# srvk/eesen

Hardware: AMD Instinct MI355X
Metric: CTC training frames/sec (whole node), 4x512 BiLSTM (higher is better)
Workload: dtype f32

## Files before the change

eesen_amd/build.py:

```python
from __future__ import annotations

import os
import shutil
import subprocess
import sys
from concurrent.futures import ThreadPoolExecutor

_DIR = os.path.dirname(os.path.abspath(__file__))
CSRC = os.path.join(_DIR, "csrc")
LIBDIR = os.path.join(_DIR, "lib")
LIB = os.path.join(LIBDIR, "libeesen_hip.so")
SOURCES = ["gemm.hip", "lstm.hip", "lstm_persistent.hip", "rec_plan.cpp", "ctc.hip", "ctc_decode.hip", "ce.hip", "optim.hip", "feeder.hip", "net.cpp", "ctc_host.cpp", "ce_host.cpp", "nnet_format.cpp", "lm.cpp", "lex.cpp", "capi.cpp", "comm.cpp"]
HEADERS = ["common.h", "guard.h", "kernels.h", "rec_kernels.h", "net.h", "lm.h", "lex.h", "handles.h", "tuning.h", os.path.join("..", "..", "include", "eesen_hip.h")]
FLAGS = (os.environ.get("EESEN_BUILD_DEFS", "").split()) + ["--offload-arch=gfx950", "-O3", "-std=c++17", "-fPIC", "-fno-gpu-rdc", "-Wall", "-Wno-unused-function"]


BINDIR = os.path.join(os.path.dirname(os.path.abspath(__file__)), "bin")
TOOLS = {"train-ctc-parallel": "train_ctc_parallel.cc", "train-ce-parallel": "train_ce_parallel.cc", "net-output-extract": "net_output_extract.cc", "ctc-align": "ctc_align.cc", "ctc-decode": "ctc_decode.cc"}


def csrc_digest() -> str:
    import hashlib
    h = hashlib.sha1()
    files = []
    for d in (CSRC, os.path.join(CSRC, "tools"), os.path.join(_DIR, "..", "include")):
        files += [os.path.join(d, f) for f in sorted(os.listdir(d)) if f.endswith((".hip", ".cpp", ".h", ".cc", ".map"))]
    for f in files:
        h.update(os.path.basename(f).encode() + b"\0")
        h.update(open(f, "rb").read())
    return h.hexdigest()[:16]


def hipcc() -> str:
    for c in (os.environ.get("HIPCC"), shutil.which("hipcc"), "/opt/rocm/bin/hipcc"):
        if c and os.path.exists(c):
            return c
    raise RuntimeError("hipcc not found")


def _stale(target: str, deps) -> bool:
    if not os.path.exists(target):
        return True
    t = os.path.getmtime(target)
    return any(os.path.getmtime(d) > t for d in deps)


def build(force: bool = False, verbose: bool = False) -> str:
    os.makedirs(LIBDIR, exist_ok=True)
    cc = hipcc()
    hdrs = [os.path.join(CSRC, h) for h in HEADERS] + [os.path.abspath(__file__)]
    jobs = []
    objs = []
    for s in SOURCES:
        src = os.path.join(CSRC, s)
        obj = os.path.join(LIBDIR, s.replace(".", "_") + ".o")
        objs.append(obj)
        if force or _stale(obj, [src] + hdrs):
            cmd = [cc] + FLAGS + (["-x", "hip"] if s.endswith(".cpp") else []) + ["-c", src, "-o", obj]
            jobs.append(cmd)

    def run(cmd):
        if verbose:
            print(" ".join(cmd), file=sys.stderr)
        r = subprocess.run(cmd, capture_output=True, text=True)
        if r.returncode != 0:
            raise RuntimeError("hipcc failed:\n" + " ".join(cmd) + "\n" + r.stdout + r.stderr)
        return r.stderr

    with ThreadPoolExecutor(max_workers=8) as ex:
        for warn in ex.map(run, jobs):
            if verbose and warn:
                print(warn, file=sys.stderr)
    if jobs or force or _stale(LIB, objs + [os.path.join(CSRC, "exports.map")]):
        run([cc, "--offload-arch=gfx950", "-shared", "-fPIC", "-o", LIB] + objs +
            ["-ldl", "-Wl,-Bsymbolic", "-Wl,--version-script=" + os.path.join(CSRC, "exports.map")])
    os.makedirs(BINDIR, exist_ok=True)
    cxx = shutil.which("g++") or "g++"
    for name, src in TOOLS.items():
        exe = os.path.join(BINDIR, name)
        srcp = os.path.join(CSRC, "tools", src)
        if force or _stale(exe, [srcp, LIB, os.path.join(CSRC, "tools", "kaldi_tables.h"), os.path.join(CSRC, "tools", "feat_pipeline.h"), os.path.join(CSRC, "tools", "parse_options.h"), os.path.join(CSRC, "tools", "class_prior.h"),
                                 os.path.join(CSRC, "..", "..", "include", "eesen_hip.h"), os.path.join(CSRC, "..", "..", "include", "eesen_hip_info.h")]):
            run([cxx, "-O2", "-std=c++17", "-Wall", srcp, "-o", exe, "-L" + LIBDIR, "-leesen_hip", "-Wl,-rpath," + LIBDIR,
                 "-Wl,-rpath,$ORIGIN/../lib", "-Wl,--allow-shlib-undefined"])
    return LIB


if __name__ == "__main__":
    print(build(force="--force" in sys.argv, verbose=True))
```

eesen_amd/csrc/kernels.h:

```cpp
#pragma once
#include "common.h"

namespace eesen {

struct GemmBound {
  const float* p = nullptr;
  int per_index = 0;
};
void gemm_f32(hipStream_t st, bool a_kc, bool b_kc, int M, int N, int K, float alpha, const float* A, int lda,
              const float* B, int ldb, float beta, float* C, int ldc, const float* bias, float* ws,
              size_t ws_floats, int extra_lds_bytes = 0,
              bool bf16_operands = false,
              GemmBound bound_a = {}, GemmBound bound_b = {});

constexpr int kDefaultGemmMode = 2;
int gemm_mode();
void set_gemm_mode(int mode);
void amax_abs(hipStream_t st, const float* P, long rows, int cols, int ld, float* out);
void amax_abs_accumulate(hipStream_t st, const float* P, long rows, int cols, int ld, float* out);
constexpr int kAmaxBlocks = 512;
void amax_rows_cols(hipStream_t st, const float* P, long rows, int cols, int ld, float* out_rows, float* out_cols, float* ws);

#ifndef EESEN_SHARDS
#define EESEN_SHARDS 8
#endif
constexpr int kShards = EESEN_SHARDS, kShardStride = 32;
constexpr int kCtlHalf = 2048 * kShards;

struct GemmGate {
  const unsigned* cnt;
  unsigned* err;
  int ndir, nz, nblk;
  int T, S;
  int spin_limit;
};
void gemm_f32_nt_gated(hipStream_t st, int M, int N, int K, const float* A, int lda, const float* B, int ldb, float* C,
                       int ldc, const float* bias, const GemmGate& gate, GemmBound bound_a = {}, GemmBound bound_b = {});

struct LstmLayerDev {
  int T, S, H, ndir;
  float* G;
  float* C;
  float* Y;
  float* X = nullptr;
  const float* Wm;
  const float* WmT;
  const float* peep;
  const int* lens;
  const float* rmask = nullptr;
  int drop_mode = 0;
  int s_begin = 0, s_count = 0;
  float* PX = nullptr;
  size_t px_floats = 0;
  int poll_delay = 0;
  int poll_raw = 0;
  unsigned* milestone = nullptr;
  int milestone_step = 0;
  int xcd_map = 1, fwd_mux = 1, bwd_q4 = 1, bwd_ksplit = 1, bwd_mux = 1;
  int fwd_t16_small = 1;
  int fwd_narrow2 = 1;
  int bwd_q4_st8 = 1;
  int fwd_bf16 = 0;
  int fwd_split = 0;
  int fwd_f16 = 0;
  const float* wm_amax = nullptr;
  int bwd_f16 = 0;
  unsigned char* DGH = nullptr;
  float* EX = nullptr;
};
float handoff_flight_ns();
void set_gpu_share(int n);
int gpu_share_value();
void wait_for_word(hipStream_t st, const unsigned* word, unsigned target, unsigned* err, double limit_s = 2.0);
void lstm_fwd_step(hipStream_t st, const LstmLayerDev& L, int step);
void lstm_bwd_step(hipStream_t st, const LstmLayerDev& L, int step, const float* dY, int lddy, float* DG, float* DCF);
void dropout_mask(hipStream_t st, float* out, long rows, int cols, int ld, float p, unsigned long long seed, bool per_column);
void activation_rows(hipStream_t st, bool tanh_, const float* x, int ldx, float* y, int ldy, long rows, int cols);
void activation_diff_rows(hipStream_t st, bool tanh_, const float* y, int ldy, float* d, int ldd, long rows, int cols);
void mul_elements(hipStream_t st, const float* a, int lda, const float* m, int ldm, float* out, int ldo, long rows, int cols);
enum { kRecNone = 0, kRecFwdBf = 1, kRecFwdMux = 2, kRecFwdF32 = 3, kRecBwdQ4 = 4, kRecBwdKsplit = 5, kRecBwdKsplitMux = 6, kRecBwdGeneric = 7 };
struct RecPlan {
  int kind = kRecNone;
  const char* kernel = "";
  int seq_tile = 0;
  int units = 0;
  int windows = 0;
  int grid[3] = {0, 0, 0};
  int wgs = 0;
  int wgs_per_cu = 0;
  int vgprs = 0, lds = 0;
  int free_vgprs = -1;
  int seq_tiles = 1;
  bool one_window = false;
  bool leaves_room = false;
  bool bf16 = false;
  bool light = false;
  size_t need_px = 0, need_ex = 0;
  bool need_dgh = false;
  size_t ctl_words = 0;
  int chunk = 0;
  const void* fn = nullptr;
};
RecPlan lstm_fwd_plan(const LstmLayerDev& L);
RecPlan lstm_bwd_plan(const LstmLayerDev& L);
void lstm_fwd_launch(hipStream_t st, const RecPlan& plan, const LstmLayerDev& L, unsigned* cnt, unsigned* err, int spin_limit,
                     unsigned long long* trace = nullptr, hipEvent_t after_reset = nullptr);
void lstm_bwd_launch(hipStream_t st, const RecPlan& plan, const LstmLayerDev& L, const float* dY, int lddy, float* DG, unsigned* cnt,
                     unsigned* err, int spin_limit, unsigned long long* trace = nullptr);
void lstm_bias_peep_grads(hipStream_t st, const LstmLayerDev& L, const float* DG, float* bias_grad, float* peep_grad,
                          float* ws, size_t ws_floats);
size_t lstm_bias_peep_ws_floats(int T, int S, int H, int ndir);

void col_sums(hipStream_t st, const float* M, int rows, int cols, int ld, float* out, float* ws, size_t ws_floats);
size_t col_sums_ws_floats(int rows, int cols);

void softmax_rows(hipStream_t st, const float* x, int ldx, float* y, int ldy, int rows, int K);
void log_rows(hipStream_t st, const float* in, int ldi, float* out, int ldo, int rows, int K);
void ctc_alpha_beta(hipStream_t st, const float* logp, int ld, int T, int S, int Lpad, const int* labx, const int* lens,
                    const int* lablens, float* alpha, float* beta, float* pzx, int waves = 0);
int ctc_sweep_waves(int Lpad, int waves = 0);
void ctc_best_path(hipStream_t st, const float* scores, int ld, int T, int S, int Lpad, const int* labx, const int* lens,
                   const int* lablens, float* delta, int waves = 0, int lattices = 0, int lat0 = 0, int lpu = 1);
void ctc_traceback(hipStream_t st, const float* delta, int T, int S, int Lpad, const int* labx, const int* lens, const int* lablens,
                   int* ali, int* pos, float* score);
void ctc_stamp(hipStream_t st, const int* pos, int T, int NL, int G, const int* lens, int* lstart, int* lend);
void ctc_hyp_lattices(hipStream_t st, const int* hyp, const int* hyp_len, const int* lens, int T, int NL, int N, int Lpad, int* labx,
                      int* lablens, int* lat_lens);
void ctc_row_topc(hipStream_t st, const float* scores, int ld, int rows, int K, int S, const int* lens, int Cc, int* cid, float* csc,
                  float* sblank);
struct LmTables;
struct LexTables;
void ctc_prefix_beam(hipStream_t st, const float* scores, int ld, int T, int S, const int* lens, int B, int Cc, const int* cid,
                     const float* csc, const float* sblank, const LmTables* lm, const LexTables* lex, float alpha, float beta, bool use_eos,
                     int* tparent, int* tlabel, int* fnode, int* flen, float* fscore, float* flm, int* count);
void ctc_hyp(hipStream_t st, const int* tparent, const int* tlabel, const int* fnode, const int* flen, const float* fscore, const float* flm,
             const int* count, int T, int S, int B, int N, int* hyp, int* hyp_len, float* score, float* lm_out);
struct WordLexTables;
void ctc_word_beam(hipStream_t st, const float* scores, int ld, int T, int S, const int* lens, int B, int Cc, const int* cid,
                   const float* csc, const float* sblank, const LmTables* lm, const WordLexTables& lex, float alpha, float beta, bool use_eos,
                   int* tparent, int* tlabel, int* tword, int* fnode, int* flen, float* fscore, float* flm, int* fword, int* fnw, int* count);
void ctc_word_hyp(hipStream_t st, const int* tparent, const int* tlabel, const int* tword, const int* fnode, const int* flen, const float* fscore,
                  const float* flm, const int* fword, const int* fnw, const int* count, int T, int S, int B, int N, int* hyp, int* hyp_len,
                  float* score, float* lm_out, int* words, int* ends, int* word_len);
void ctc_error_diff(hipStream_t st, const float* probs, int ld, int T, int S, int K, int Lpad, int Lmax, const int* lens,
                    const int* lablens, const int* labx, const float* alpha, const float* beta,
                    const float* pzx, float* diff, int ldd);
void log_sub_prior(hipStream_t st, float* m, int ld, int rows, int K, bool apply_log, const float* log_prior, float prior_scale);
void row_argmax(hipStream_t st, const float* m, int ld, int rows, int K, int* ids);

struct CeSums {
  double obj;
  long long correct;
};
int ce_eval_blocks(int rows);
void ce_eval(hipStream_t st, const float* y, int ld, int rows, int K, int S, const int* lens, const int* tgt, float* diff,
             int ldd, CeSums* part, CeSums* out);

void sgd_update(hipStream_t st, float* param, float* corr, const float* fresh, long n, float mmt, float lr_coef,
                float max_grad, const unsigned* skip = nullptr, const float* live = nullptr);
void zero_if_set(hipStream_t st, float* p, long n, const unsigned* word);
void adaptive_update(hipStream_t st, float* param, float* corr, const float* fresh, float* accu, long n, float mmt, float lr,
                     float max_grad, float eps, float rho, float one_minus_rho, bool rmsprop, const unsigned* skip = nullptr,
                     const float* live = nullptr);
void tensor_moments(hipStream_t st, const float* base, long rows, int cols, long ld, double* out6, double* ws,
                    int nb = 0, int hf = 0, int hi = 0);
void transpose2d(hipStream_t st, const float* src, int rows, int cols, float* dst);
void copy2d(hipStream_t st, const float* src, int lds, float* dst, int ldd, int rows, int cols);

}
```

eesen_amd/csrc/lstm_persistent.hip:

```cpp
#include "rec_kernels.h"

namespace eesen {
namespace {

typedef float f32x4 __attribute__((ext_vector_type(4)));
constexpr int NW = 8;
constexpr int kSc1 = 16;

#define EESEN_RCP(x) __builtin_amdgcn_rcpf(x)
__device__ __forceinline__ float sigmoidf_(float x) { return EESEN_RCP(1.f + __expf(-x)); }
__device__ __forceinline__ float tanhf_(float x) { return 1.f - 2.f * EESEN_RCP(1.f + __expf(2.f * x)); }

__device__ __forceinline__ __amdgpu_buffer_rsrc_t make_rsrc(const float* base) {
  return __builtin_amdgcn_make_buffer_rsrc(const_cast<float*>(base), 0, 0x7fffffff, 0x00020000);
}
__device__ __forceinline__ float ld1(__amdgpu_buffer_rsrc_t r, unsigned byte_off) {
  return __builtin_bit_cast(float, __builtin_amdgcn_raw_buffer_load_b32(r, byte_off, 0, 0));
}
constexpr int EESEN_POLL_WAVE = 7;
constexpr int EESEN_POLL_SLEEP = 1;
__device__ __forceinline__ void ld8_sc1(__amdgpu_buffer_rsrc_t r, unsigned byte_off, int k, int kmax, bool ok, float (&v)[8]) {
  constexpr int pol = 0;
  constexpr unsigned kOob = 0x80000000u;
  const unsigned oa = (ok && k < kmax) ? byte_off : kOob;
  const unsigned ob = (ok && k + 4 < kmax) ? byte_off + 16 : kOob;
  const f32x4 a = __builtin_amdgcn_raw_buffer_load_b128(r, oa, 0, pol);
  const f32x4 b = __builtin_amdgcn_raw_buffer_load_b128(r, ob, 0, pol);
  v[0] = a[0]; v[1] = a[1]; v[2] = a[2]; v[3] = a[3];
  v[4] = b[0]; v[5] = b[1]; v[6] = b[2]; v[7] = b[3];
}
__device__ __forceinline__ float ror8(float x) {
  return __builtin_bit_cast(float, __builtin_amdgcn_mov_dpp(__builtin_bit_cast(int, x), 0x128, 0xf, 0xf, true));
}
__device__ __forceinline__ void ld8_plain(const float* __restrict__ row, int k, int kmax, bool ok, float (&v)[8]) {
  float4 a = make_float4(0.f, 0.f, 0.f, 0.f), b = a;
  if (ok && k < kmax) a = *reinterpret_cast<const float4*>(row + k);
  if (ok && k + 4 < kmax) b = *reinterpret_cast<const float4*>(row + k + 4);
  v[0] = a.x; v[1] = a.y; v[2] = a.z; v[3] = a.w;
  v[4] = b.x; v[5] = b.y; v[6] = b.z; v[7] = b.w;
}

struct Role {
  int nblk, ndir, nz, xcd;
  __device__ __forceinline__ int combo(int b) const { return xcd ? b % (ndir * nz) : b / nblk; }
  __device__ __forceinline__ int unit_group(int b) const { return xcd ? b / (ndir * nz) : b % nblk; }
  __device__ __forceinline__ int dir(int b) const { return combo(b) % ndir; }
  __device__ __forceinline__ int seq_group(int b) const { return combo(b) / ndir; }
};

__device__ __forceinline__ void sleep_ticks(int ticks) {
  if (ticks <= 0) return;
  const unsigned long long t0 = wall_clock64();
  while ((long long)(wall_clock64() - t0) < (long long)ticks) __builtin_amdgcn_s_sleep(1);
}
__device__ __forceinline__ bool wait_counters(unsigned* cnt, unsigned nblk, unsigned step, unsigned* err, int spin_limit, int lane, int delay) {
  const unsigned mine = lane < kShards ? ((nblk - lane + kShards - 1) / kShards) * step : 0u;
  sleep_ticks(delay);
  for (int spins = 0; spins < spin_limit; ++spins) {
    bool ok = true;
    if (lane < kShards) ok = __hip_atomic_load(cnt + lane * kShardStride, __ATOMIC_RELAXED, __HIP_MEMORY_SCOPE_AGENT) >= mine;
    if (__all(ok)) return true;
    if ((spins & 1023) == 1023 && __hip_atomic_load(err, __ATOMIC_RELAXED, __HIP_MEMORY_SCOPE_AGENT) != 0) return false;
    __builtin_amdgcn_s_sleep(EESEN_POLL_SLEEP);
  }
  if (lane == 0) __hip_atomic_store(err, 1u, __ATOMIC_RELAXED, __HIP_MEMORY_SCOPE_AGENT);
  return false;
}

__global__ __launch_bounds__(64) void handoff_pingpong_kernel(unsigned* flags, unsigned long long* out, int rounds) {
  if (threadIdx.x != 0) return;
  unsigned* mine = flags + (blockIdx.x == 0 ? 0 : 32);
  unsigned* theirs = flags + (blockIdx.x == 0 ? 32 : 0);
  unsigned* dead = flags + 16;
  const unsigned long long t0 = wall_clock64();
  bool ok = true;
  for (int i = 1; i <= rounds && ok; ++i) {
    if (blockIdx.x == 0) __hip_atomic_store(mine, (unsigned)i, __ATOMIC_RELAXED, __HIP_MEMORY_SCOPE_AGENT);
    ok = false;
    for (int spins = 0; spins < (1 << 20); ++spins) {
      if (__hip_atomic_load(theirs, __ATOMIC_RELAXED, __HIP_MEMORY_SCOPE_AGENT) >= (unsigned)i) { ok = true; break; }
      if ((spins & 255) == 255 && __hip_atomic_load(dead, __ATOMIC_RELAXED, __HIP_MEMORY_SCOPE_AGENT) != 0) break;
    }
    if (!ok) { __hip_atomic_store(dead, 1u, __ATOMIC_RELAXED, __HIP_MEMORY_SCOPE_AGENT); break; }
    if (blockIdx.x != 0) __hip_atomic_store(mine, (unsigned)i, __ATOMIC_RELAXED, __HIP_MEMORY_SCOPE_AGENT);
  }
  if (blockIdx.x == 0) out[0] = ok ? wall_clock64() - t0 : 0ull;
}

__global__ __launch_bounds__(64) void wait_for_word_kernel(const unsigned* word, unsigned target, unsigned* err, unsigned long long limit_ticks) {
  if (threadIdx.x != 0) return;
  const unsigned long long t0 = wall_clock64();
  for (unsigned spins = 0;; ++spins) {
    if (__hip_atomic_load(word, __ATOMIC_RELAXED, __HIP_MEMORY_SCOPE_AGENT) >= target) return;
    if ((spins & 7) == 7) {
      if (__hip_atomic_load(err, __ATOMIC_RELAXED, __HIP_MEMORY_SCOPE_AGENT) != 0) return;
      if (wall_clock64() - t0 > limit_ticks) break;
    }
    __builtin_amdgcn_s_sleep(127);
    __builtin_amdgcn_s_sleep(127);
  }
  __hip_atomic_store(err, 2u, __ATOMIC_RELAXED, __HIP_MEMORY_SCOPE_AGENT);
}

__device__ __forceinline__ void report_milestone(unsigned* ms, unsigned ngroups) {
  if (__hip_atomic_fetch_add(ms, 1u, __ATOMIC_RELAXED, __HIP_MEMORY_SCOPE_AGENT) + 1u == ngroups)
    __hip_atomic_store(ms + 1, 1u, __ATOMIC_RELAXED, __HIP_MEMORY_SCOPE_AGENT);
}

#define EESEN_STAMP(i) do { if (trace && tid == 0 && blockIdx.x == 0 && step < 127) \
    trace[step * 5 + (i)] = __builtin_amdgcn_s_memtime(); } while (0)

template <int CPW, int MT, int NT, bool DROP, bool XCHG = false>
__global__ __launch_bounds__(NW * 64) void lstm_fwd_persistent_kernel(LstmLayerDev L, unsigned* cnt, unsigned* err,
                                                                      int spin_limit, unsigned long long* trace, Role R) {
  constexpr int ST = 16 * MT, UB = 4 * NT, RW = 16 * NT + 4;
  __shared__ __attribute__((aligned(16))) float red[NW][ST][RW];
  __shared__ int s_go;
  __builtin_amdgcn_s_setprio(3);
  const int tid = threadIdx.x, lane = tid & 63, wave = tid >> 6;
  const int H = L.H, S = L.S, T = L.T;
  const int ldY = L.ndir * H, ldG = L.ndir * 4 * H;
  const int bx = R.unit_group(blockIdx.x), dir = R.dir(blockIdx.x), bz = R.seq_group(blockIdx.x);
  const int u0 = bx * UB, s0 = L.s_begin + bz * ST;
  const int s_end = L.s_begin + (L.s_count ? L.s_count : S);
  unsigned* my_cnt = cnt + (size_t)(dir * R.nz + bz) * kShards * kShardStride;
  const unsigned nblk = R.nblk;

  const int li = lane & 15, kq = lane >> 4;
  float b[NT][CPW][8];
#pragma unroll
  for (int n = 0; n < NT; ++n) {
    const float* Wr = L.Wm + ((size_t)dir * 4 * H + (size_t)u0 * 4 + n * 16 + li) * H;
#pragma unroll
    for (int c = 0; c < CPW; ++c) ld8_plain(Wr, (wave + c * NW) * 32 + kq * 8, H, true, b[n][c]);
  }
  const int es = tid / UB, eu = tid % UB;
  const int s_e = s0 + es;
  const bool e_ok = tid < ST * UB && s_e < s_end;
  float p_i = 0.f, p_f = 0.f, p_o = 0.f, cprev = 0.f;
  int len = 0;
  if (e_ok) {
    const float* pp = L.peep + (size_t)dir * 3 * H + u0 + eu;
    p_i = pp[0]; p_f = pp[H]; p_o = pp[2 * H];
    len = L.lens[s_e];
  }
  const size_t gcol = (size_t)dir * 4 * H + (u0 + eu) * 4;
  float4 gx = make_float4(0.f, 0.f, 0.f, 0.f);
  if (e_ok) gx = *reinterpret_cast<const float4*>(L.G + (size_t)((dir == 0 ? 0 : T - 1) * S + s_e) * ldG + gcol);

  const __amdgpu_buffer_rsrc_t rY = make_rsrc(XCHG ? L.X : L.Y);
  const int nch = (H + 31) / 32;
  const unsigned xblk = (unsigned)nch * 512u * 4u;
  const int zt = (L.s_begin / ST) + bz;
  const int nzall = (S + ST - 1) / ST;
  for (int step = 0; step < T; ++step) {
    const int t = dir == 0 ? step : T - 1 - step;
    const int tp = dir == 0 ? t - 1 : t + 1;
    f32x4 acc[MT][NT];
#pragma unroll
    for (int m = 0; m < MT; ++m)
#pragma unroll
      for (int n = 0; n < NT; ++n) acc[m][n] = f32x4{0.f, 0.f, 0.f, 0.f};
    EESEN_STAMP(0);
    if (step > 0) {
      if (wave == EESEN_POLL_WAVE) {
        const bool go = wait_counters(my_cnt, nblk, (unsigned)step, err, spin_limit, lane, L.poll_delay);
        if (lane == 0) s_go = go ? 1 : 0;
      }
      __syncthreads();
      if (!s_go) return;
      EESEN_STAMP(1);
      if (L.milestone && step == L.milestone_step + 1 && bx == 0 && tid == 0)
        report_milestone(L.milestone, (unsigned)(R.ndir * R.nz));
      const unsigned ybase = (unsigned)(((size_t)(tp + 1) * S * ldY + dir * H) * 4);
      float a[MT][CPW][8];
      if constexpr (XCHG) {
        const unsigned xb = ((unsigned)(tp * L.ndir + dir) * (unsigned)nzall + (unsigned)zt) * xblk;
        constexpr unsigned kOob = 0x80000000u;
        const bool rok = s0 + li < s_end;
#pragma unroll
        for (int c = 0; c < CPW; ++c) {
          const int ch = wave + c * NW;
          const unsigned o0 = xb + (unsigned)((ch * 2 * 4 + kq) * 64 + li * 4) * 4u;
          const bool ok = rok && ch < nch;
          const f32x4 lo = __builtin_amdgcn_raw_buffer_load_b128(rY, ok ? o0 : kOob, 0, 0);
          const f32x4 hi = __builtin_amdgcn_raw_buffer_load_b128(rY, ok ? o0 + 4u * 64u * 4u : kOob, 0, 0);
          a[0][c][0] = lo[0]; a[0][c][1] = lo[1]; a[0][c][2] = lo[2]; a[0][c][3] = lo[3];
          a[0][c][4] = hi[0]; a[0][c][5] = hi[1]; a[0][c][6] = hi[2]; a[0][c][7] = hi[3];
        }
      } else {
#pragma unroll
      for (int c = 0; c < CPW; ++c) {
        const int k = (wave + c * NW) * 32 + kq * 8;
#pragma unroll
        for (int m = 0; m < MT; ++m) {
          const int sa = s0 + m * 16 + li;
          ld8_sc1(rY, ybase + (unsigned)(((size_t)sa * ldY + k) * 4), k, H, sa < s_end, a[m][c]);
        }
      }
      }
      __builtin_amdgcn_sched_barrier(0);
#pragma unroll
      for (int c = 0; c < CPW; ++c)
#pragma unroll
        for (int j = 0; j < 8; ++j)
#pragma unroll
          for (int m = 0; m < MT; ++m)
#pragma unroll
            for (int n = 0; n < NT; ++n) acc[m][n] = __builtin_amdgcn_mfma_f32_16x16x4f32(a[m][c][j], b[n][c][j], acc[m][n], 0, 0, 0);
    }
#pragma unroll
    for (int m = 0; m < MT; ++m)
#pragma unroll
      for (int n = 0; n < NT; ++n)
#pragma unroll
        for (int r = 0; r < 4; ++r) red[wave][m * 16 + 4 * kq + r][n * 16 + li] = acc[m][n][r];
    __syncthreads();
    EESEN_STAMP(2);
    if (e_ok) {
      float4 pre = gx;
#pragma unroll
      for (int w = 0; w < NW; ++w) {
        const float4 v = *reinterpret_cast<const float4*>(&red[w][es][eu * 4]);
        pre.x += v.x; pre.y += v.y; pre.z += v.z; pre.w += v.w;
      }
      float g = tanhf_(pre.x);
      float i = sigmoidf_(pre.y + p_i * cprev);
      float f = sigmoidf_(pre.z + p_f * cprev);
      float c = g * i + cprev * f;
      if (DROP) {
        const float mk = L.rmask[(size_t)((t + 1) * S + s_e) * ldY + dir * H + u0 + eu];
        c = L.drop_mode == 1 ? mk * (g * i) + cprev * f : mk * (g * i + cprev * f);
      }
      float h = tanhf_(c);
      float o = sigmoidf_(pre.w + p_o * c);
      float m = h * o;
      if (t >= len) { g = i = f = o = c = m = 0.f; }
      *reinterpret_cast<float4*>(L.G + (size_t)(t * S + s_e) * ldG + gcol) = make_float4(g, i, f, o);
      const size_t o1 = (size_t)((t + 1) * S + s_e) * ldY + dir * H + u0 + eu;
      L.C[o1] = c;
      __hip_atomic_store(L.Y + o1, m, __ATOMIC_RELAXED, __HIP_MEMORY_SCOPE_AGENT);
      if constexpr (XCHG) {
        const int k = u0 + eu;
        const size_t xo = ((size_t)(t * L.ndir + dir) * nzall + zt) * ((size_t)nch * 512) +
                          (size_t)(((k >> 5) * 2 + ((k & 7) >> 2)) * 4 + ((k & 31) >> 3)) * 64 + es * 4 + (k & 3);
        __hip_atomic_store(L.X + xo, m, __ATOMIC_RELAXED, __HIP_MEMORY_SCOPE_AGENT);
      }
      cprev = c;
    }
    EESEN_STAMP(3);
    {
      if (tid < ST * UB) asm volatile("s_waitcnt vmcnt(0)" ::: "memory");
      __syncthreads();
      EESEN_STAMP(4);
      if (tid == 0) __hip_atomic_fetch_add(my_cnt + (bx & (kShards - 1)) * kShardStride, 1u, __ATOMIC_RELAXED, __HIP_MEMORY_SCOPE_AGENT);
      if (e_ok && step + 1 < T)
        gx = *reinterpret_cast<const float4*>(L.G + (size_t)((dir == 0 ? t + 1 : t - 1) * S + s_e) * ldG + gcol);
    }
  }
}

typedef __bf16 bf16x8_t __attribute__((ext_vector_type(8)));
typedef _Float16 f16x8_t __attribute__((ext_vector_type(8)));
typedef _Float16 f16x2_t __attribute__((ext_vector_type(2)));
typedef float f32x2_t __attribute__((ext_vector_type(2)));
__device__ __forceinline__ void half_scale(const float* amax, float& scale, float& inv) {
  const int e = (int)((__float_as_uint(*amax) >> 23) & 0xffu);
  const int s = min(max(127 + 14 + 127 - e, 1), 253);
  scale = __uint_as_float((unsigned)s << 23);
  inv = __uint_as_float((unsigned)(254 - s) << 23);
}
__device__ __forceinline__ void half_scale(float amax, float& scale, float& inv) { half_scale(&amax, scale, inv); }
__device__ __forceinline__ unsigned rne_f16(float x) { return (unsigned)__builtin_bit_cast(unsigned short, (_Float16)x); }
__device__ __forceinline__ float f16_bits_to_f32(unsigned h) { return (float)__builtin_bit_cast(_Float16, (unsigned short)h); }
__device__ __forceinline__ unsigned rne_bf16(float x) {
  const unsigned b = __float_as_uint(x);
  return (b + 0x7fffu + ((b >> 16) & 1u)) >> 16;
}
__device__ __forceinline__ unsigned quad_xor1(unsigned v) { return (unsigned)__builtin_amdgcn_mov_dpp((int)v, 0xB1, 0xf, 0xf, true); }
__device__ __forceinline__ unsigned quad_xor2(unsigned v) { return (unsigned)__builtin_amdgcn_mov_dpp((int)v, 0x4E, 0xf, 0xf, true); }
template <int CPW, int NT, int AP, int WP, bool F16 = false>
__global__ __launch_bounds__(NW * 64) void lstm_fwd_persistent_bf_kernel(LstmLayerDev L, unsigned* cnt, unsigned* err,
                                                                         int spin_limit, unsigned long long* trace, Role R) {
  constexpr int ST = 16, UB = 4 * NT, RW = 16 * NT + 4, SMAX = (AP > WP ? AP : WP) - 1;
  constexpr float kMScale = 16384.f;
  __shared__ __attribute__((aligned(16))) float red[NW][ST][RW];
  __shared__ int s_go;
  __builtin_amdgcn_s_setprio(3);
  const int tid = threadIdx.x, lane = tid & 63, wave = tid >> 6;
  const int H = L.H, S = L.S, T = L.T;
  if (T < 0) {
    if (tid == 0) {
      __hip_atomic_fetch_add(cnt, 1u, __ATOMIC_RELAXED, __HIP_MEMORY_SCOPE_AGENT);
      const unsigned long long t0 = wall_clock64();
      bool all = false;
      while (!(all = __hip_atomic_load(cnt, __ATOMIC_RELAXED, __HIP_MEMORY_SCOPE_AGENT) >= gridDim.x) && wall_clock64() - t0 < 500000ull)
        __builtin_amdgcn_s_sleep(8);
      if (!all) __hip_atomic_store(err, 1u, __ATOMIC_RELAXED, __HIP_MEMORY_SCOPE_AGENT);
    }
    return;
  }
  const int ldY = L.ndir * H, ldG = L.ndir * 4 * H;
  const int bx = R.unit_group(blockIdx.x), dir = R.dir(blockIdx.x), bz = R.seq_group(blockIdx.x);
  const int u0 = bx * UB, s0 = L.s_begin + bz * ST;
  const int s_end = L.s_begin + (L.s_count ? L.s_count : S);
  unsigned* my_cnt = cnt + (size_t)(dir * R.nz + bz) * kShards * kShardStride;
  const unsigned nblk = R.nblk;
  const int li = lane & 15, kq = lane >> 4;
  const int nch = H / 32;
  float wscale = 1.f, unscale = 1.f;
  if constexpr (F16) { half_scale(L.wm_amax, wscale, unscale); unscale *= 1.f / kMScale; }
  f32x4 b[WP][NT][CPW];
#pragma unroll
  for (int n = 0; n < NT; ++n) {
    const float* Wr = L.Wm + ((size_t)dir * 4 * H + (size_t)u0 * 4 + n * 16 + li) * H;
#pragma unroll
    for (int c = 0; c < CPW; ++c) {
      float w[8];
      ld8_plain(Wr, (wave + c * NW) * 32 + kq * 8, H, true, w);
      if constexpr (F16) {
#pragma unroll
        for (int j = 0; j < 8; ++j) w[j] *= wscale;
      }
#pragma unroll
      for (int pl = 0; pl < WP; ++pl) {
        f32x4 pk;
#pragma unroll
        for (int j = 0; j < 4; ++j) {
          if constexpr (F16) {
            const unsigned h0 = rne_f16(w[2 * j]), h1 = rne_f16(w[2 * j + 1]);
            pk[j] = __uint_as_float(h0 | (h1 << 16));
            w[2 * j] -= f16_bits_to_f32(h0);
            w[2 * j + 1] -= f16_bits_to_f32(h1);
          } else {
            const unsigned h0 = rne_bf16(w[2 * j]), h1 = rne_bf16(w[2 * j + 1]);
            pk[j] = __uint_as_float(h0 | (h1 << 16));
            w[2 * j] -= __uint_as_float(h0 << 16);
            w[2 * j + 1] -= __uint_as_float(h1 << 16);
          }
        }
        b[pl][n][c] = pk;
      }
    }
  }
  const int es = tid / UB, eu = tid % UB;
  const int s_e = s0 + es;
  const bool e_act = tid < ST * UB;
  const bool e_ok = e_act && s_e < s_end;
  float p_i = 0.f, p_f = 0.f, p_o = 0.f, cprev = 0.f;
  int len = 0;
  if (e_ok) {
    const float* pp = L.peep + (size_t)dir * 3 * H + u0 + eu;
    p_i = pp[0]; p_f = pp[H]; p_o = pp[2 * H];
    len = L.lens[s_e];
  }
  const size_t gcol = (size_t)dir * 4 * H + (u0 + eu) * 4;
  float4 gx = make_float4(0.f, 0.f, 0.f, 0.f);
  if (e_ok) gx = *reinterpret_cast<const float4*>(L.G + (size_t)((dir == 0 ? 0 : T - 1) * S + s_e) * ldG + gcol);
  const __amdgpu_buffer_rsrc_t rX = make_rsrc(L.X);
  const unsigned xpl = (unsigned)nch * 1024u;
  const unsigned xblk = xpl * AP;
  const int zt = (L.s_begin / ST) + bz;
  const int nzall = (S + ST - 1) / ST;
  unsigned char* const xbytes = reinterpret_cast<unsigned char*>(L.X);
  for (int step = 0; step < T; ++step) {
    const int t = dir == 0 ? step : T - 1 - step;
    const int tp = dir == 0 ? t - 1 : t + 1;
    f32x4 acc[NT];
#pragma unroll
    for (int n = 0; n < NT; ++n) acc[n] = f32x4{0.f, 0.f, 0.f, 0.f};
    EESEN_STAMP(0);
    if (step > 0) {
      if (wave == EESEN_POLL_WAVE) {
        const bool go = wait_counters(my_cnt, nblk, (unsigned)step, err, spin_limit, lane, L.poll_delay);
        if (lane == 0) s_go = go ? 1 : 0;
      }
      __syncthreads();
      if (!s_go) return;
      EESEN_STAMP(1);
      if (L.milestone && step == L.milestone_step + 1 && bx == 0 && tid == 0)
        report_milestone(L.milestone, (unsigned)(R.ndir * R.nz));
      const unsigned xb = ((unsigned)(tp * L.ndir + dir) * (unsigned)nzall + (unsigned)zt) * xblk;
      constexpr unsigned kOob = 0x80000000u;
      const bool rok = s0 + li < s_end;
      f32x4 a[AP][CPW];
#pragma unroll
      for (int pl = 0; pl < AP; ++pl)
#pragma unroll
        for (int c = 0; c < CPW; ++c) {
          const int ch = wave + c * NW;
          a[pl][c] = __builtin_amdgcn_raw_buffer_load_b128(rX, (rok && ch < nch) ? xb + (unsigned)pl * xpl + (unsigned)(((ch * 4 + kq) * 16 + li) * 16) : kOob, 0, 0);
        }
      __builtin_amdgcn_sched_barrier(0);
#pragma unroll
      for (int sum = SMAX; sum >= 0; --sum)
#pragma unroll
        for (int i = 0; i < AP; ++i) {
          const int j = sum - i;
          if (j < 0 || j >= WP) continue;
#pragma unroll
          for (int c = 0; c < CPW; ++c)
#pragma unroll
            for (int n = 0; n < NT; ++n) {
              const f32x4& bb = b[j < WP && j >= 0 ? j : 0][n][c];
              if constexpr (F16) acc[n] = __builtin_amdgcn_mfma_f32_16x16x32_f16(__builtin_bit_cast(f16x8_t, a[i][c]), __builtin_bit_cast(f16x8_t, bb), acc[n], 0, 0, 0);
              else acc[n] = __builtin_amdgcn_mfma_f32_16x16x32_bf16(__builtin_bit_cast(bf16x8_t, a[i][c]), __builtin_bit_cast(bf16x8_t, bb), acc[n], 0, 0, 0);
            }
        }
    }
#pragma unroll
    for (int n = 0; n < NT; ++n)
#pragma unroll
      for (int r = 0; r < 4; ++r) red[wave][4 * kq + r][n * 16 + li] = F16 ? acc[n][r] * unscale : acc[n][r];
    __syncthreads();
    EESEN_STAMP(2);
    if (e_act) {
      float4 pv[NW];
#pragma unroll
      for (int w = 0; w < NW; ++w) pv[w] = *reinterpret_cast<const float4*>(&red[w][es][eu * 4]);
      __builtin_amdgcn_sched_barrier(0);
      float4 pre = gx;
#pragma unroll
      for (int w = 0; w < NW; ++w) { pre.x += pv[w].x; pre.y += pv[w].y; pre.z += pv[w].z; pre.w += pv[w].w; }
      float g = tanhf_(pre.x);
      float i = sigmoidf_(pre.y + p_i * cprev);
      float f = sigmoidf_(pre.z + p_f * cprev);
      float c = g * i + cprev * f;
      float h = tanhf_(c);
      float o = sigmoidf_(pre.w + p_o * c);
      float m = h * o;
      if (t >= len || !e_ok) { g = i = f = o = c = m = 0.f; }
      if (e_ok) {
        *reinterpret_cast<float4*>(L.G + (size_t)(t * S + s_e) * ldG + gcol) = make_float4(g, i, f, o);
        const size_t o1 = (size_t)((t + 1) * S + s_e) * ldY + dir * H + u0 + eu;
        L.C[o1] = c;
        __hip_atomic_store(L.Y + o1, m, __ATOMIC_RELAXED, __HIP_MEMORY_SCOPE_AGENT);
        cprev = c;
      }
      const int k = u0 + eu;
      const size_t xo = ((size_t)(t * L.ndir + dir) * nzall + zt) * (size_t)xblk +
                        (size_t)((((k >> 5) * 4 + ((k & 31) >> 3)) * 16 + es) * 16 + (k & 7) * 2);
      float rem = F16 ? m * kMScale : m;
#pragma unroll
      for (int pl = 0; pl < AP; ++pl) {
        const unsigned hb = F16 ? rne_f16(rem) : rne_bf16(rem);
        rem -= F16 ? f16_bits_to_f32(hb) : __uint_as_float(hb << 16);
        const unsigned pk = hb | (quad_xor1(hb) << 16);
        const unsigned pk2 = quad_xor2(pk);
        if (e_ok && (eu & 3) == 0)
          __hip_atomic_store(reinterpret_cast<unsigned long long*>(xbytes + xo + (size_t)pl * xpl), (unsigned long long)pk | ((unsigned long long)pk2 << 32),
                             __ATOMIC_RELAXED, __HIP_MEMORY_SCOPE_AGENT);
      }
    }
    EESEN_STAMP(3);
    {
      if (e_act) asm volatile("s_waitcnt vmcnt(0)" ::: "memory");
      __syncthreads();
      EESEN_STAMP(4);
      if (tid == 0) __hip_atomic_fetch_add(my_cnt + (bx & (kShards - 1)) * kShardStride, 1u, __ATOMIC_RELAXED, __HIP_MEMORY_SCOPE_AGENT);
      if (e_ok && step + 1 < T)
        gx = *reinterpret_cast<const float4*>(L.G + (size_t)((dir == 0 ? t + 1 : t - 1) * S + s_e) * ldG + gcol);
    }
  }
}

template <int CPW, int NT, bool XCHG>
__global__ __launch_bounds__(NW * 64) void lstm_fwd_persistent_mux_kernel(LstmLayerDev L, unsigned* cnt, unsigned* err,
                                                                          int spin_limit, Role R) {
  constexpr int ST = 16, UB = 4 * NT, RW = 16 * NT + 4, Q = 2;
  __shared__ __attribute__((aligned(16))) float red[NW][ST][RW];
  __shared__ int s_go;
  __builtin_amdgcn_s_setprio(3);
  const int tid = threadIdx.x, lane = tid & 63, wave = tid >> 6;
  const int H = L.H, S = L.S, T = L.T;
  const int ldY = L.ndir * H, ldG = L.ndir * 4 * H;
  const int bx = R.unit_group(blockIdx.x), dir = R.dir(blockIdx.x), bg = R.seq_group(blockIdx.x);
  const int u0 = bx * UB;
  const int nzall = (S + ST - 1) / ST;
  const unsigned nblk = R.nblk;
  const int li = lane & 15, kq = lane >> 4;
  float b[NT][CPW][8];
#pragma unroll
  for (int n = 0; n < NT; ++n) {
    const float* Wr = L.Wm + ((size_t)dir * 4 * H + (size_t)u0 * 4 + n * 16 + li) * H;
#pragma unroll
    for (int c = 0; c < CPW; ++c) ld8_plain(Wr, (wave + c * NW) * 32 + kq * 8, H, true, b[n][c]);
  }
  const int es = tid / UB, eu = tid % UB;
  float p_i = 0.f, p_f = 0.f, p_o = 0.f;
  if (tid < ST * UB) {
    const float* pp = L.peep + (size_t)dir * 3 * H + u0 + eu;
    p_i = pp[0]; p_f = pp[H]; p_o = pp[2 * H];
  }
  const size_t gcol = (size_t)dir * 4 * H + (u0 + eu) * 4;
  int zt[Q], s_e[Q], len[Q];
  bool e_ok[Q];
  float cprev[Q];
  float4 gx[Q];
  unsigned* my_cnt[Q];
#pragma unroll
  for (int q = 0; q < Q; ++q) {
    zt[q] = bg * Q + q;
    s_e[q] = zt[q] * ST + es;
    e_ok[q] = tid < ST * UB && zt[q] < nzall && s_e[q] < S;
    len[q] = e_ok[q] ? L.lens[s_e[q]] : 0;
    cprev[q] = 0.f;
    gx[q] = make_float4(0.f, 0.f, 0.f, 0.f);
    if (e_ok[q]) gx[q] = *reinterpret_cast<const float4*>(L.G + (size_t)((dir == 0 ? 0 : T - 1) * S + s_e[q]) * ldG + gcol);
    my_cnt[q] = cnt + (size_t)(dir * nzall + zt[q]) * kShards * kShardStride;
  }
  const __amdgpu_buffer_rsrc_t rY = make_rsrc(XCHG ? L.X : L.Y);
  const int nch = (H + 31) / 32;
  const unsigned xblk = (unsigned)nch * 512u * 4u;
  bool polled = false;
  for (int step = 0; step < T; ++step) {
    const int t = dir == 0 ? step : T - 1 - step;
    const int tp = dir == 0 ? t - 1 : t + 1;
#pragma unroll
    for (int q = 0; q < Q; ++q) {
      if (zt[q] >= nzall) continue;
      f32x4 acc[NT];
#pragma unroll
      for (int n = 0; n < NT; ++n) acc[n] = f32x4{0.f, 0.f, 0.f, 0.f};
      if (step > 0) {
        if (!polled) {
          if (wave == EESEN_POLL_WAVE) {
            const bool go = wait_counters(my_cnt[q], nblk, (unsigned)step, err, spin_limit, lane, 0);
            if (lane == 0) s_go = go ? 1 : 0;
          }
          __syncthreads();
          if (!s_go) return;
        }
        if (L.milestone && step == L.milestone_step + 1 && bx == 0 && tid == 0)
          report_milestone(L.milestone, (unsigned)(L.ndir * nzall));
        float a[CPW][8];
        const int s0 = zt[q] * ST;
        if constexpr (XCHG) {
          const unsigned xb = ((unsigned)(tp * L.ndir + dir) * (unsigned)nzall + (unsigned)zt[q]) * xblk;
          constexpr unsigned kOob = 0x80000000u;
          const bool rok = s0 + li < S;
#pragma unroll
          for (int c = 0; c < CPW; ++c) {
            const int ch = wave + c * NW;
            const unsigned o0 = xb + (unsigned)((ch * 2 * 4 + kq) * 64 + li * 4) * 4u;
            const bool ok = rok && ch < nch;
            const f32x4 lo = __builtin_amdgcn_raw_buffer_load_b128(rY, ok ? o0 : kOob, 0, 0);
            const f32x4 hi = __builtin_amdgcn_raw_buffer_load_b128(rY, ok ? o0 + 4u * 64u * 4u : kOob, 0, 0);
            a[c][0] = lo[0]; a[c][1] = lo[1]; a[c][2] = lo[2]; a[c][3] = lo[3];
            a[c][4] = hi[0]; a[c][5] = hi[1]; a[c][6] = hi[2]; a[c][7] = hi[3];
          }
        } else {
          const unsigned ybase = (unsigned)(((size_t)(tp + 1) * S * ldY + dir * H) * 4);
#pragma unroll
          for (int c = 0; c < CPW; ++c) {
            const int k = (wave + c * NW) * 32 + kq * 8;
            const int sa = s0 + li;
            ld8_sc1(rY, ybase + (unsigned)(((size_t)sa * ldY + k) * 4), k, H, sa < S, a[c]);
          }
        }
        __builtin_amdgcn_sched_barrier(0);
#pragma unroll
        for (int c = 0; c < CPW; ++c)
#pragma unroll
          for (int j = 0; j < 8; ++j)
#pragma unroll
            for (int n = 0; n < NT; ++n) acc[n] = __builtin_amdgcn_mfma_f32_16x16x4f32(a[c][j], b[n][c][j], acc[n], 0, 0, 0);
      }
#pragma unroll
      for (int n = 0; n < NT; ++n)
#pragma unroll
        for (int r = 0; r < 4; ++r) red[wave][4 * kq + r][n * 16 + li] = acc[n][r];
      __syncthreads();
      if (e_ok[q]) {
        float4 pre = gx[q];
#pragma unroll
        for (int w = 0; w < NW; ++w) {
          const float4 v = *reinterpret_cast<const float4*>(&red[w][es][eu * 4]);
          pre.x += v.x; pre.y += v.y; pre.z += v.z; pre.w += v.w;
        }
        float g = tanhf_(pre.x);
        float i = sigmoidf_(pre.y + p_i * cprev[q]);
        float f = sigmoidf_(pre.z + p_f * cprev[q]);
        float c = g * i + cprev[q] * f;
        float h = tanhf_(c);
        float o = sigmoidf_(pre.w + p_o * c);
        float m = h * o;
        if (t >= len[q]) { g = i = f = o = c = m = 0.f; }
        *reinterpret_cast<float4*>(L.G + (size_t)(t * S + s_e[q]) * ldG + gcol) = make_float4(g, i, f, o);
        const size_t o1 = (size_t)((t + 1) * S + s_e[q]) * ldY + dir * H + u0 + eu;
        L.C[o1] = c;
        __hip_atomic_store(L.Y + o1, m, __ATOMIC_RELAXED, __HIP_MEMORY_SCOPE_AGENT);
        if constexpr (XCHG) {
          const int k = u0 + eu;
          const size_t xo = ((size_t)(t * L.ndir + dir) * nzall + zt[q]) * ((size_t)nch * 512) +
                            (size_t)(((k >> 5) * 2 + ((k & 7) >> 2)) * 4 + ((k & 31) >> 3)) * 64 + es * 4 + (k & 3);
          __hip_atomic_store(L.X + xo, m, __ATOMIC_RELAXED, __HIP_MEMORY_SCOPE_AGENT);
        }
        cprev[q] = c;
      }
      polled = false;
      {
        const int nq = q + 1 < Q && zt[Q - 1] < nzall ? q + 1 : 0;
        const int nstep = nq > q ? step : step + 1;
        if (nstep > 0 && nstep < T && !(nq == q)) {
          if (wave == EESEN_POLL_WAVE) {
            const bool go = wait_counters(my_cnt[nq], nblk, (unsigned)nstep, err, spin_limit, lane, 0);
            if (lane == 0) s_go = go ? 1 : 0;
          }
          polled = true;
        }
      }
      if (tid < ST * UB) asm volatile("s_waitcnt vmcnt(0)" ::: "memory");
      __syncthreads();
      if (polled && !s_go) return;
      if (tid == 0) __hip_atomic_fetch_add(my_cnt[q] + (bx & (kShards - 1)) * kShardStride, 1u, __ATOMIC_RELAXED, __HIP_MEMORY_SCOPE_AGENT);
      if (e_ok[q] && step + 1 < T)
        gx[q] = *reinterpret_cast<const float4*>(L.G + (size_t)((dir == 0 ? t + 1 : t - 1) * S + s_e[q]) * ldG + gcol);
    }
  }
}

template <int CPW, int ST, bool DROP>
__global__ __launch_bounds__(NW * 64) void lstm_bwd_persistent_kernel(LstmLayerDev L, const float* __restrict__ dY,
                                                                      int lddy, float* __restrict__ DG, unsigned* cnt,
                                                                      unsigned* err, int spin_limit, unsigned long long* trace,
                                                                      Role R, int chunk) {
  constexpr bool X44 = ST == 8 && CPW <= 8;
  constexpr int LDSB = X44 && CPW == 8 ? 2 : 0, REGB = X44 ? CPW - LDSB : 1;
  __shared__ __attribute__((aligned(16))) float4 bl[LDSB ? LDSB : 1][4][LDSB ? NW * 64 : 1];
  __shared__ float red[NW][16][17];
  __shared__ int s_go;
  __builtin_amdgcn_s_setprio(3);
  const int tid = threadIdx.x, lane = tid & 63, wave = tid >> 6;
  const int H = L.H, S = L.S, T = L.T;
  const int ldY = L.ndir * H, ldG = L.ndir * 4 * H, K4 = 4 * H;
  const int bx = R.unit_group(blockIdx.x), dir = R.dir(blockIdx.x), bz = R.seq_group(blockIdx.x);
  const int u0 = bx * 16, s0 = L.s_begin + bz * ST;
  const int s_end = L.s_begin + (L.s_count ? L.s_count : S);
  unsigned* my_cnt = cnt + (size_t)(dir * R.nz + bz) * kShards * kShardStride;
  const unsigned nblk = R.nblk;

  const int li = lane & 15, kq = lane >> 4;
  const int sa = s0 + li, ub = u0 + li;
  const int g4 = lane >> 4, rb4 = g4 >> 1, ks4 = g4 & 1, cb4 = (lane >> 2) & 3, x4 = lane & 3;
  float bw[REGB][4][4];
  if constexpr (X44) {
    const int ub4 = u0 + cb4 * 4 + x4;
    const float* Br = L.WmT + ((size_t)dir * H + min(ub4, H - 1)) * K4;
#pragma unroll
    for (int c = 0; c < CPW; ++c) {
      const int k0 = (wave + c * NW) * 32 + ks4 * 16;
#pragma unroll
      for (int q = 0; q < 4; ++q) {
        float4 v = make_float4(0.f, 0.f, 0.f, 0.f);
        if (ub4 < H && k0 + q * 4 < K4) v = *reinterpret_cast<const float4*>(Br + k0 + q * 4);
        if (c < REGB) { bw[c][0][q] = v.x; bw[c][1][q] = v.y; bw[c][2][q] = v.z; bw[c][3][q] = v.w; }
        else bl[c - REGB][q][tid] = v;
      }
    }
  }
  float b[X44 ? 1 : CPW][8];
  if constexpr (!X44) {
    const float* Br = L.WmT + ((size_t)dir * H + ub) * K4;
#pragma unroll
    for (int c = 0; c < CPW; ++c) {
      const int k0 = (wave + c * NW) * 32;
      if constexpr (ST == 8) {
        float lo[8], hi[8];
        ld8_plain(Br, k0 + kq * 4, K4, ub < H, lo);
        ld8_plain(Br, k0 + 16 + kq * 4, K4, ub < H, hi);
#pragma unroll
        for (int j = 0; j < 4; ++j) { b[c][j] = lo[j]; b[c][4 + j] = hi[j]; }
      } else {
        ld8_plain(Br, k0 + kq * 8, K4, ub < H, b[c]);
      }
    }
  }
  const int es = tid >> 4, eu = tid & 15;
  const int s_e = s0 + es, u_e = u0 + eu;
  const bool e_ok = tid < ST * 16 && s_e < s_end && u_e < H;
  float p_i = 0.f, p_f = 0.f, p_o = 0.f;
  int len = 0;
  if (e_ok) {
    const float* pp = L.peep + (size_t)dir * 3 * H + u_e;
    p_i = pp[0]; p_f = pp[H]; p_o = pp[2 * H];
    len = L.lens[s_e];
  }
  float dcf = 0.f, dn_i = 0.f, dn_f = 0.f;
  const size_t gcol = (size_t)dir * K4 + u_e * 4;
  const size_t ycol = (size_t)dir * H + u_e;
  float4 gt = make_float4(0.f, 0.f, 0.f, 0.f);
  float dy = 0.f, c_t = 0.f, c_p = 0.f;
  {
    const int t0 = dir == 0 ? T - 1 : 0, tp0 = dir == 0 ? t0 - 1 : t0 + 1;
    if (e_ok) {
      gt = *reinterpret_cast<const float4*>(L.G + (size_t)(t0 * S + s_e) * ldG + gcol);
      dy = dY[(size_t)(t0 * S + s_e) * lddy + ycol];
      c_t = L.C[(size_t)((t0 + 1) * S + s_e) * ldY + ycol];
      c_p = L.C[(size_t)((tp0 + 1) * S + s_e) * ldY + ycol];
    }
  }
  __amdgpu_buffer_rsrc_t rDG = make_rsrc(DG);
  int tbS = 0;

  for (int step = 0; step < T; ++step) {
    const int t = dir == 0 ? T - 1 - step : step;
    const int tn = dir == 0 ? t + 1 : t - 1;
    if (chunk < T && step % chunk == 0) {
      const int tb = dir == 0 ? max(0, T - step - chunk) : max(0, step - 1);
      tbS = tb * S;
      rDG = make_rsrc(DG + (size_t)tbS * ldG);
    }
    f32x4 acc0 = {0.f, 0.f, 0.f, 0.f}, acc1 = {0.f, 0.f, 0.f, 0.f};
    EESEN_STAMP(0);
    if (step > 0) {
      if (wave == EESEN_POLL_WAVE) {
        const bool go = wait_counters(my_cnt, nblk, (unsigned)step, err, spin_limit, lane, L.poll_delay);
        if (lane == 0) s_go = go ? 1 : 0;
      }
      __syncthreads();
      if (!s_go) return;
      EESEN_STAMP(1);
      const int tnb = tn * S - tbS;
      const size_t arow = ((size_t)(tnb + sa) * ldG + (size_t)dir * K4) * 4;
      if constexpr (X44) {
        const unsigned arow4 = (unsigned)(((size_t)(tnb + s0 + rb4 * 4 + x4) * ldG + (size_t)dir * K4) * 4);
        const bool rok = s0 + rb4 * 4 + x4 < s_end;
        constexpr int INF = CPW < 4 ? CPW : 4;
        auto fetch = [&](int c) {
          const int k = (wave + c * NW) * 32 + (ks4 * 4 + cb4) * 4;
          return __builtin_amdgcn_raw_buffer_load_b128(rDG, (rok && k < K4) ? arow4 + (unsigned)k * 4u : 0x80000000u, 0,
                                                       0);
        };
        f32x4 a4[INF];
#pragma unroll
        for (int c = 0; c < INF; ++c) a4[c] = fetch(c);
        __builtin_amdgcn_sched_barrier(0);
        f32x4 ac[2] = {{0.f, 0.f, 0.f, 0.f}, {0.f, 0.f, 0.f, 0.f}};
#pragma unroll
        for (int c = 0; c < CPW; ++c) {
          const f32x4 cur = a4[c % INF];
#pragma unroll
          for (int h = 0; h < 2; ++h) {
            float w0[4], w1[4];
            if (c < REGB) {
#pragma unroll
              for (int r = 0; r < 4; ++r) { w0[r] = bw[c < REGB ? c : 0][r][2 * h]; w1[r] = bw[c < REGB ? c : 0][r][2 * h + 1]; }
            } else {
              int lt = tid;
              asm volatile("" : "+v"(lt));
              const float4 v0 = bl[c < REGB ? 0 : c - REGB][2 * h][lt], v1 = bl[c < REGB ? 0 : c - REGB][2 * h + 1][lt];
              w0[0] = v0.x; w0[1] = v0.y; w0[2] = v0.z; w0[3] = v0.w;
              w1[0] = v1.x; w1[1] = v1.y; w1[2] = v1.z; w1[3] = v1.w;
            }
#pragma unroll
            for (int r = 0; r < 4; ++r) {
              if (h == 0) {
                ac[0] = __builtin_amdgcn_mfma_f32_4x4x1f32(cur[r], w0[r], ac[0], 2, 0, 0);
                ac[1] = __builtin_amdgcn_mfma_f32_4x4x1f32(cur[r], w1[r], ac[1], 2, 1, 0);
              } else {
                ac[0] = __builtin_amdgcn_mfma_f32_4x4x1f32(cur[r], w0[r], ac[0], 2, 2, 0);
                ac[1] = __builtin_amdgcn_mfma_f32_4x4x1f32(cur[r], w1[r], ac[1], 2, 3, 0);
              }
            }
          }
          if (c + INF < CPW) {
// ... 677 lines not shown
#pragma unroll
        for (int d = 0; d < 2; ++d) tmp[d] = __builtin_amdgcn_mfma_f32_16x16x32_f16(__builtin_bit_cast(f16x8_t, ah2[d]), __builtin_bit_cast(f16x8_t, bl[3][c + d]), tmp[d], 0, 0, 0);
#pragma unroll
        for (int d = 0; d < 2; ++d) tmp[d] = __builtin_amdgcn_mfma_f32_16x16x32_f16(__builtin_bit_cast(f16x8_t, ah2[d]), __builtin_bit_cast(f16x8_t, bh[3][c + d]), tmp[d], 0, 0, 0);
#pragma unroll
        for (int d = 0; d < 2; ++d) {
#pragma unroll
          for (int r = 0; r < 4; ++r) acc[3][r] = fmaf(tmp[d][r], ex_inv(iv[c + d], r), acc[3][r]);
        }
        if (c == 0) {
          __builtin_amdgcn_sched_barrier(0);
          if (e_ok) px_load<KU>(px, ku, es * 16 + eu, sw);
          __builtin_amdgcn_sched_barrier(0);
        }
      }
#pragma unroll
      for (int r = 0; r < 4; ++r) red2[wave][4 * kq + r][li] = acc[3][r] * winv;
      EESEN_STAMP(2);
      __syncthreads();
      if (e_ok) {
        float rv[NW];
#pragma unroll
        for (int w = 0; w < NW; ++w) rv[w] = red2[w][es][eu];
#pragma unroll
        for (int w = 0; w < NW; ++w) dm_in += rv[w];
        if (!px_take<KU>(px, ku, es * 16 + eu, (unsigned)step, err, spin_limit, sw, dm_in)) {
          __hip_atomic_store(err, 1u, __ATOMIC_RELAXED, __HIP_MEMORY_SCOPE_AGENT);
          s_fail = 1;
        }
      }
      EESEN_STAMP(3);
    }
    if (e_act) {
      const float dm = dy + dm_in;
      const float g_ = gt.x, i = gt.y, f = gt.z, o = gt.w;
      const float h = tanhf_(c_t);
      const float dh = (1.f - h * h) * (dm * o);
      float dob = o * (1.f - o) * (dm * h);
      const float dc = dh + park[3][tid] + park[4][tid] * park[0][tid] + park[5][tid] * park[1][tid] + dob * park[2][tid];
      float df = f * (1.f - f) * (dc * c_p);
      float di = i * (1.f - i) * (dc * g_);
      float dg = (1.f - g_ * g_) * (dc * i);
      float carry = dc * f;
      if (t >= len || !e_ok) { dg = di = df = dob = 0.f; carry = 0.f; }
      float sc, inv;
      unsigned ex4;
      {
        const float rm = dpp_row_max16(fmaxf(fmaxf(fabsf(dg), fabsf(di)), fmaxf(fabsf(df), fabsf(dob))));
        half_scale(rm, sc, inv);
        const int ei = (int)(__float_as_uint(inv) >> 23);
        ex4 = (unsigned)__builtin_amdgcn_readlane(ei, 0) | ((unsigned)__builtin_amdgcn_readlane(ei, 16) << 8) |
              ((unsigned)__builtin_amdgcn_readlane(ei, 32) << 16) | ((unsigned)__builtin_amdgcn_readlane(ei, 48) << 24);
      }
#if !defined(EESEN_PROBE_KH) || !(EESEN_PROBE_KH & 4)
      if (lane == 0 && s0 + 4 * wave < s_end) {
        const f32x4 iv4 = {__uint_as_float(ex4), __uint_as_float(ex4), __uint_as_float(ex4), __uint_as_float(ex4)};
        __builtin_amdgcn_raw_buffer_store_b128(iv4, rEX, (unsigned)((((size_t)(t * L.ndir + dir) * NZ + zt) * NP + uc0 / 16) * 64 + wave * 16), 0, kSc1);
      }
#endif
      if (e_ok) {
        const f32x4 out = {dg, di, df, dob};
        const unsigned o32 = (unsigned)(((size_t)(t * S - tbS + s_e) * ldG + gcol) * 4);
        const f32x2_t x01 = {dg * sc, di * sc}, x23 = {df * sc, dob * sc};
        const f16x2_t h01 = __builtin_convertvector(x01, f16x2_t), h23 = __builtin_convertvector(x23, f16x2_t);
        const f32x2_t r01 = {x01[0] - (float)h01[0], x01[1] - (float)h01[1]}, r23 = {x23[0] - (float)h23[0], x23[1] - (float)h23[1]};
        const f16x2_t l01 = __builtin_convertvector(r01, f16x2_t), l23 = __builtin_convertvector(r23, f16x2_t);
        const f32x4 pp = {__builtin_bit_cast(float, h01), __builtin_bit_cast(float, h23), __builtin_bit_cast(float, l01), __builtin_bit_cast(float, l23)};
#if !defined(EESEN_PROBE_KH) || !(EESEN_PROBE_KH & 1)
        __builtin_amdgcn_raw_buffer_store_b128(pp, rDH, o32, 0, kSc1);
#endif
        __builtin_amdgcn_raw_buffer_store_b128(out, rDG, o32, 0, kSc1);
        park[3][tid] = carry; park[4][tid] = di; park[5][tid] = df;
      }
    }
    if (step + 1 < T) {
      if (tid < ST * 16) asm volatile("s_waitcnt vmcnt(1)" ::: "memory");
      __syncthreads();
      if (s_fail) return;
      EESEN_STAMP(4);
      if (tid == 0) __hip_atomic_fetch_add(pub_cnt, 1u, __ATOMIC_RELAXED, __HIP_MEMORY_SCOPE_AGENT);
      if (e_ok) {
        const int t2 = dir == 0 ? t - 1 : t + 1, tp2 = dir == 0 ? t2 - 1 : t2 + 1;
        gt = *reinterpret_cast<const float4*>(L.G + (size_t)(t2 * S + s_e) * ldG + gcol);
        dy = dY[(size_t)(t2 * S + s_e) * lddy + ycol];
        c_t = c_p;
        c_p = L.C[(size_t)((tp2 + 1) * S + s_e) * ldY + ycol];
      }
    }
  }
}

template <int CPW>
__global__ __launch_bounds__(NW * 64) void lstm_bwd_persistent_ksplit_mux_kernel(LstmLayerDev L, const float* __restrict__ dY, int lddy,
                                                                                 float* __restrict__ DG, unsigned long long* __restrict__ PX, unsigned* cnt,
                                                                                 unsigned* err, int spin_limit, Role R, int chunk) {
  constexpr int KU = 4, ST = 16, UW = 64, NT = 4, Q = 2;
  __shared__ float red[NW][ST][UW + 1];
  __shared__ float own[Q][ST][17];
  __shared__ int s_go, s_fail;
  __builtin_amdgcn_s_setprio(3);
  const int tid = threadIdx.x, lane = tid & 63, wave = tid >> 6;
  const int H = L.H, S = L.S, T = L.T;
  const int ldY = L.ndir * H, ldG = L.ndir * 4 * H, K4 = 4 * H, KQ = K4 / KU;
  const int bx = R.unit_group(blockIdx.x), dir = R.dir(blockIdx.x), bg = R.seq_group(blockIdx.x);
  const int uu = bx / KU, ku = bx % KU;
  const int um0 = uu * UW, uc0 = um0 + ku * 16;
  const int nzall = (S + ST - 1) / ST, ngroups = L.ndir * nzall, nub = H / UW;
  const unsigned nprod = (unsigned)(H / KU / 16);
  const int li = lane & 15, kq = lane >> 4;
  float b[NT][CPW][8];
#pragma unroll
  for (int n = 0; n < NT; ++n) {
    const float* Br = L.WmT + ((size_t)dir * H + um0 + n * 16 + li) * K4 + (size_t)ku * KQ;
#pragma unroll
    for (int c = 0; c < CPW; ++c) ld8_plain(Br, (wave + c * NW) * 32 + kq * 8, KQ, true, b[n][c]);
  }
  const int es = tid >> 4, eu = tid & 15;
  const int u_e = uc0 + eu;
  float p_i = 0.f, p_f = 0.f, p_o = 0.f;
  if (tid < ST * 16) {
    const float* pp = L.peep + (size_t)dir * 3 * H + u_e;
    p_i = pp[0]; p_f = pp[H]; p_o = pp[2 * H];
  }
  const size_t gcol = (size_t)dir * K4 + u_e * 4;
  const size_t ycol = (size_t)dir * H + u_e;
  int zt[Q], s0[Q], s_e[Q], len[Q], g[Q];
  bool live[Q], e_ok[Q];
  float dcf[Q], dn_i[Q], dn_f[Q], dy[Q], c_t[Q], c_p[Q], dm_in[Q];
  float4 gt[Q];
  unsigned *wait_cnt[Q], *pub_cnt[Q];
#pragma unroll
  for (int q = 0; q < Q; ++q) {
    zt[q] = bg * Q + q;
    live[q] = zt[q] < nzall;
    s0[q] = zt[q] * ST;
    s_e[q] = s0[q] + es;
    e_ok[q] = live[q] && tid < ST * 16 && s_e[q] < S;
    g[q] = dir * nzall + (live[q] ? zt[q] : 0);
    wait_cnt[q] = cnt + (size_t)(g[q] * KU + ku) * kShards * kShardStride;
    pub_cnt[q] = cnt + (size_t)(g[q] * KU + uc0 / (H / KU)) * kShards * kShardStride + (size_t)(((uc0 / 16) % (int)nprod) & (kShards - 1)) * kShardStride;
    len[q] = e_ok[q] ? L.lens[s_e[q]] : 0;
    dcf[q] = dn_i[q] = dn_f[q] = dy[q] = c_t[q] = c_p[q] = dm_in[q] = 0.f;
    gt[q] = make_float4(0.f, 0.f, 0.f, 0.f);
    const int t0 = dir == 0 ? T - 1 : 0, tp0 = dir == 0 ? t0 - 1 : t0 + 1;
    if (e_ok[q]) {
      gt[q] = *reinterpret_cast<const float4*>(L.G + (size_t)(t0 * S + s_e[q]) * ldG + gcol);
      dy[q] = dY[(size_t)(t0 * S + s_e[q]) * lddy + ycol];
      c_t[q] = L.C[(size_t)((t0 + 1) * S + s_e[q]) * ldY + ycol];
      c_p[q] = L.C[(size_t)((tp0 + 1) * S + s_e[q]) * ldY + ycol];
    }
  }
  if (tid == 0) s_fail = 0;
  __amdgpu_buffer_rsrc_t rDG = make_rsrc(DG);
  int tbS = 0;

  for (int step = 0; step < T; ++step) {
    const int t = dir == 0 ? T - 1 - step : step;
    const int tn = dir == 0 ? t + 1 : t - 1;
    if (chunk < T && step % chunk == 0) {
      const int tb = dir == 0 ? max(0, T - step - chunk) : max(0, step - 1);
      tbS = tb * S;
      rDG = make_rsrc(DG + (size_t)tbS * ldG);
    }
    unsigned long long sw[Q][KU] = {};
    if (step > 0) {
#pragma unroll
      for (int q = 0; q < Q; ++q) {
        if (!live[q]) continue;
        if (wave == EESEN_POLL_WAVE) {
          const bool go = wait_counters(wait_cnt[q], nprod, (unsigned)step, err, spin_limit, lane, 0);
          if (lane == 0) s_go = go ? 1 : 0;
        }
        __syncthreads();
        if (!s_go) return;
        f32x4 acc[NT];
#pragma unroll
        for (int n = 0; n < NT; ++n) acc[n] = f32x4{0.f, 0.f, 0.f, 0.f};
        const int sa = s0[q] + li;
        const size_t arow = ((size_t)(tn * S - tbS + sa) * ldG + (size_t)dir * K4 + (size_t)ku * KQ) * 4;
        float a[CPW][8];
#pragma unroll
        for (int c = 0; c < CPW; ++c) {
          const int k = (wave + c * NW) * 32 + kq * 8;
          ld8_sc1(rDG, (unsigned)(arow + (size_t)k * 4), k, KQ, sa < S, a[c]);
        }
        __builtin_amdgcn_sched_barrier(0);
#pragma unroll
        for (int c = 0; c < CPW / 2; ++c)
#pragma unroll
          for (int j = 0; j < 8; ++j)
#pragma unroll
            for (int n = 0; n < NT; ++n) acc[n] = __builtin_amdgcn_mfma_f32_16x16x4f32(a[c][j], b[n][c][j], acc[n], 0, 0, 0);
        __builtin_amdgcn_sched_barrier(0);
        if (q == 1 && e_ok[0])
          px_load<KU>(PX + ((size_t)((size_t)(step & 1) * ngroups + g[0]) * nub + uu) * (KU * KU * 256), ku, es * 16 + eu, sw[0]);
        __builtin_amdgcn_sched_barrier(0);
#pragma unroll
        for (int c = CPW / 2; c < CPW; ++c)
#pragma unroll
          for (int j = 0; j < 8; ++j)
#pragma unroll
            for (int n = 0; n < NT; ++n) acc[n] = __builtin_amdgcn_mfma_f32_16x16x4f32(a[c][j], b[n][c][j], acc[n], 0, 0, 0);
#pragma unroll
        for (int n = 0; n < NT; ++n)
#pragma unroll
          for (int r = 0; r < 4; ++r) red[wave][4 * kq + r][n * 16 + li] = acc[n][r];
        __syncthreads();
        unsigned long long* px = PX + ((size_t)((size_t)(step & 1) * ngroups + g[q]) * nub + uu) * (KU * KU * 256);
#pragma unroll
        for (int h = 0; h < 2; ++h) {
          const int o = tid + h * (NW * 64), sq = o >> 6, uc = o & 63, dst = uc >> 4;
          float v = 0.f;
#pragma unroll
          for (int w = 0; w < NW; ++w) v += red[w][sq][uc];
          if (dst == ku) own[q][sq][uc & 15] = v;
          else px_put(px + (size_t)(dst * KU + ku) * 256 + sq * 16 + (uc & 15), v, (unsigned)step);
        }
        __syncthreads();
      }
    }
    if (step > 0) {
      if (live[1] && e_ok[1]) px_load<KU>(PX + ((size_t)((size_t)(step & 1) * ngroups + g[1]) * nub + uu) * (KU * KU * 256), ku, es * 16 + eu, sw[1]);
      if (!live[1] && e_ok[0]) px_load<KU>(PX + ((size_t)((size_t)(step & 1) * ngroups + g[0]) * nub + uu) * (KU * KU * 256), ku, es * 16 + eu, sw[0]);
    }
#pragma unroll
    for (int q = 0; q < Q; ++q) {
      if (!live[q]) continue;
      float dm = dy[q];
      if (step > 0) {
        if (e_ok[q]) {
          const unsigned long long* px = PX + ((size_t)((size_t)(step & 1) * ngroups + g[q]) * nub + uu) * (KU * KU * 256);
          dm += own[q][es][eu];
          if (!px_take<KU>(px, ku, es * 16 + eu, (unsigned)step, err, spin_limit, sw[q], dm)) {
            __hip_atomic_store(err, 1u, __ATOMIC_RELAXED, __HIP_MEMORY_SCOPE_AGENT);
            s_fail = 1;
          }
        }
      }
      if (e_ok[q]) {
        const float g_ = gt[q].x, i = gt[q].y, f = gt[q].z, o = gt[q].w;
        const float h = tanhf_(c_t[q]);
        const float dh = (1.f - h * h) * (dm * o);
        float dob = o * (1.f - o) * (dm * h);
        const float dc = dh + dcf[q] + dn_i[q] * p_i + dn_f[q] * p_f + dob * p_o;
        float df = f * (1.f - f) * (dc * c_p[q]);
        float di = i * (1.f - i) * (dc * g_);
        float dg = (1.f - g_ * g_) * (dc * i);
        float carry = dc * f;
        if (t >= len[q]) { dg = di = df = dob = 0.f; carry = 0.f; }
        const f32x4 out = {dg, di, df, dob};
        __builtin_amdgcn_raw_buffer_store_b128(out, rDG, (unsigned)(((size_t)(t * S - tbS + s_e[q]) * ldG + gcol) * 4), 0, kSc1);
        dcf[q] = carry; dn_i[q] = di; dn_f[q] = df;
      }
      if (step + 1 < T) {
        if (tid < ST * 16) asm volatile("s_waitcnt vmcnt(0)" ::: "memory");
        __syncthreads();
        if (s_fail) return;
        if (tid == 0) __hip_atomic_fetch_add(pub_cnt[q], 1u, __ATOMIC_RELAXED, __HIP_MEMORY_SCOPE_AGENT);
        if (e_ok[q]) {
          const int t2 = dir == 0 ? t - 1 : t + 1, tp2 = dir == 0 ? t2 - 1 : t2 + 1;
          gt[q] = *reinterpret_cast<const float4*>(L.G + (size_t)(t2 * S + s_e[q]) * ldG + gcol);
          dy[q] = dY[(size_t)(t2 * S + s_e[q]) * lddy + ycol];
          c_t[q] = c_p[q];
          c_p[q] = L.C[(size_t)((tp2 + 1) * S + s_e[q]) * ldY + ycol];
        }
      }
    }
  }
}

static_assert(NW == kRecWaves && sizeof(Role) == sizeof(RecRole), "rec_kernels.h states the workgroup size and the role argument");

#define EESEN_ROW(family, kind, kernel, ...) {family, kind, {__VA_ARGS__}, reinterpret_cast<const void*>(&kernel<__VA_ARGS__>), #kernel "<" #__VA_ARGS__ ">"}
#define EESEN_FWD_F32(...) EESEN_ROW(kFwdF32, kRecFwdF32, lstm_fwd_persistent_kernel, __VA_ARGS__)
#define EESEN_FWD_BF(...) EESEN_ROW(kFwdBf, kRecFwdBf, lstm_fwd_persistent_bf_kernel, __VA_ARGS__)
#define EESEN_BWD_GEN(...) EESEN_ROW(kBwdGeneric, kRecBwdGeneric, lstm_bwd_persistent_kernel, __VA_ARGS__)
#define EESEN_BWD_Q4(...) EESEN_ROW(kBwdQ4, kRecBwdQ4, lstm_bwd_persistent_q4_kernel, __VA_ARGS__)
const RecKernel kRecKernels[] = {
    EESEN_FWD_F32(1,1,4,true,false), EESEN_FWD_F32(1,1,4,false,false), EESEN_FWD_F32(1,1,4,false,true),
    EESEN_FWD_F32(2,1,4,true,false), EESEN_FWD_F32(2,1,4,false,false), EESEN_FWD_F32(2,1,4,false,true),
    EESEN_FWD_F32(4,1,4,true,false), EESEN_FWD_F32(4,1,4,false,false), EESEN_FWD_F32(4,1,4,false,true),
    EESEN_FWD_F32(1,1,2,true,false), EESEN_FWD_F32(1,1,2,false,false), EESEN_FWD_F32(1,1,2,false,true),
    EESEN_FWD_F32(2,1,2,true,false), EESEN_FWD_F32(2,1,2,false,false), EESEN_FWD_F32(2,1,2,false,true),
    EESEN_FWD_F32(1,2,1,true,false), EESEN_FWD_F32(1,2,1,false,false),
    EESEN_FWD_F32(2,2,1,true,false), EESEN_FWD_F32(2,2,1,false,false),
    EESEN_FWD_F32(4,2,1,true,false), EESEN_FWD_F32(4,2,1,false,false),
    EESEN_FWD_BF(1,2,2,2,true), EESEN_FWD_BF(2,2,2,2,true),
    EESEN_FWD_BF(1,4,2,2,true), EESEN_FWD_BF(2,4,2,2,true), EESEN_FWD_BF(3,4,2,2,true), EESEN_FWD_BF(4,4,2,2,true),
    EESEN_FWD_BF(1,2,3,3,false), EESEN_FWD_BF(2,2,3,3,false),
    EESEN_FWD_BF(1,4,1,2,false), EESEN_FWD_BF(2,4,1,2,false), EESEN_FWD_BF(3,4,1,2,false), EESEN_FWD_BF(4,4,1,2,false),
    EESEN_ROW(kFwdMux, kRecFwdMux, lstm_fwd_persistent_mux_kernel, 4,4,true), EESEN_ROW(kFwdMux, kRecFwdMux, lstm_fwd_persistent_mux_kernel, 4,4,false),
    EESEN_BWD_GEN(1,8,true), EESEN_BWD_GEN(1,8,false), EESEN_BWD_GEN(1,16,true), EESEN_BWD_GEN(1,16,false),
    EESEN_BWD_GEN(2,8,true), EESEN_BWD_GEN(2,8,false), EESEN_BWD_GEN(2,16,true), EESEN_BWD_GEN(2,16,false),
    EESEN_BWD_GEN(4,8,true), EESEN_BWD_GEN(4,8,false), EESEN_BWD_GEN(4,16,true), EESEN_BWD_GEN(4,16,false),
    EESEN_BWD_GEN(8,8,true), EESEN_BWD_GEN(8,8,false), EESEN_BWD_GEN(8,16,true), EESEN_BWD_GEN(8,16,false),
    EESEN_BWD_GEN(16,8,true), EESEN_BWD_GEN(16,8,false), EESEN_BWD_GEN(16,16,true), EESEN_BWD_GEN(16,16,false),
    EESEN_BWD_Q4(2,4), EESEN_BWD_Q4(2,8), EESEN_BWD_Q4(4,4), EESEN_BWD_Q4(4,8), EESEN_BWD_Q4(6,4), EESEN_BWD_Q4(6,8), EESEN_BWD_Q4(8,4), EESEN_BWD_Q4(8,8),
    EESEN_ROW(kBwdKsplit, kRecBwdKsplit, lstm_bwd_persistent_ksplit_kernel, 2), EESEN_ROW(kBwdKsplit, kRecBwdKsplit, lstm_bwd_persistent_ksplit_kernel, 3),
    EESEN_ROW(kBwdKsplit, kRecBwdKsplit, lstm_bwd_persistent_ksplit_kernel, 4),
    EESEN_ROW(kBwdKsplitH, kRecBwdKsplit, lstm_bwd_persistent_ksplit_h_kernel, 2), EESEN_ROW(kBwdKsplitH, kRecBwdKsplit, lstm_bwd_persistent_ksplit_h_kernel, 4),
    EESEN_ROW(kBwdKsplitMux, kRecBwdKsplitMux, lstm_bwd_persistent_ksplit_mux_kernel, 2), EESEN_ROW(kBwdKsplitMux, kRecBwdKsplitMux, lstm_bwd_persistent_ksplit_mux_kernel, 3),
    EESEN_ROW(kBwdKsplitMux, kRecBwdKsplitMux, lstm_bwd_persistent_ksplit_mux_kernel, 4),
};
#undef EESEN_BWD_Q4
#undef EESEN_BWD_GEN
#undef EESEN_FWD_BF
#undef EESEN_FWD_F32
#undef EESEN_ROW

}

const RecKernel* rec_kernel(int family, int a0, int a1, int a2, int a3, int a4) {
  const int want[5] = {a0, a1, a2, a3, a4};
  for (const RecKernel& k : kRecKernels)
    if (k.family == family && std::equal(want, want + 5, k.arg)) return &k;
  return nullptr;
}
const void* handoff_pingpong_fn() { return reinterpret_cast<const void*>(&handoff_pingpong_kernel); }
const void* wait_for_word_fn() { return reinterpret_cast<const void*>(&wait_for_word_kernel); }

}
```

eesen_amd/csrc/net.cpp:

```cpp
#include "net.h"

#include <algorithm>
#include <cmath>
#include <cstdio>
#include <cstring>

namespace eesen {


int PhaseTimer::begin(hipStream_t st, int phase) {
  if (!on_) return -1;
  if (used_ == spans_.size()) spans_.emplace_back();
  spans_[used_].phase = phase;
  spans_[used_].a.record(st);
  return (int)used_++;
}
void PhaseTimer::end(hipStream_t st, int idx) {
  if (!on_ || idx < 0) return;
  spans_[idx].b.record(st);
}
void PhaseTimer::collect(float* out, int nphase) {
  for (int i = 0; i < nphase; ++i) out[i] = 0.f;
  for (size_t i = 0; i < used_; ++i) {
    spans_[i].b.wait();
    float ms = 0.f;
    EESEN_HIP_CHECK(hipEventElapsedTime(&ms, spans_[i].a, spans_[i].b));
    if (spans_[i].phase >= 0 && spans_[i].phase < nphase) out[spans_[i].phase] += ms * 1e-3f;
  }
  if (accumulate_) used_ = 0;
}

int PhaseTimer::spans(int* phases, float* secs, int cap) {
  for (size_t i = 0; i < used_ && (int)i < cap; ++i) {
    spans_[i].b.wait();
    float ms = 0.f;
    EESEN_HIP_CHECK(hipEventElapsedTime(&ms, spans_[i].a, spans_[i].b));
    if (phases) phases[i] = spans_[i].phase;
    if (secs) secs[i] = ms * 1e-3f;
  }
  return (int)used_;
}

long Layer::file_params() const {
  if (is_lstm()) return (long)ndir * ((long)4 * Hf * din_f + (long)4 * Hf * Hf + 4 * Hf + 3 * Hf);
  if (kind == EESEN_LAYER_AFFINE) return (long)dout_f * din_f + dout_f;
  return 0;
}

const char* Layer::marker() const {
  switch (kind) {
    case EESEN_LAYER_BILSTM_PARALLEL: return nonparallel ? "<BiLstm>" : "<BiLstmParallel>";
    case EESEN_LAYER_LSTM_PARALLEL: return nonparallel ? "<Lstm>" : "<LstmParallel>";
    case EESEN_LAYER_AFFINE: return "<AffineTransform>";
    case EESEN_LAYER_SOFTMAX: return "<Softmax>";
    case EESEN_LAYER_SIGMOID: return "<Sigmoid>";
    case EESEN_LAYER_TANH: return "<Tanh>";
  }
  return "<Unknown>";
}

template <class F>
static void for_each_param(const Layer& L, F f) {
  long fi = 0;
  if (L.is_lstm()) {
    const int H = L.H, Hf = L.Hf, D = L.din_f, D4 = pad4(L.din);
    for (int dir = 0; dir < L.ndir; ++dir) {
      for (int r = 0; r < 4 * Hf; ++r) {
        const int q = r / Hf, u = r % Hf;
        for (int d = 0; d < D; ++d) f(fi++, L.off_wx + ((size_t)dir * 4 * H + u * 4 + q) * D4 + L.in_col(d));
      }
      for (int r = 0; r < 4 * Hf; ++r) {
        const int q = r / Hf, u = r % Hf;
        for (int k = 0; k < Hf; ++k) f(fi++, L.off_wm + ((size_t)dir * 4 * H + u * 4 + q) * H + k);
      }
      for (int r = 0; r < 4 * Hf; ++r) f(fi++, L.off_bias + (size_t)dir * 4 * H + (r % Hf) * 4 + r / Hf);
      for (int g = 0; g < 3; ++g)
        for (int u = 0; u < Hf; ++u) f(fi++, L.off_peep + ((size_t)dir * 3 + g) * H + u);
    }
  } else if (L.kind == EESEN_LAYER_AFFINE) {
    const int D4 = pad4(L.din);
    for (int r = 0; r < L.dout; ++r)
      for (int d = 0; d < L.din_f; ++d) f(fi++, L.off_w + (size_t)r * D4 + L.in_col(d));
    for (int r = 0; r < L.dout; ++r) f(fi++, L.off_b + r);
  }
}

Net::Net(int dev, void* stream) : device(dev) {
  require_device(dev);
  st = reinterpret_cast<hipStream_t>(stream);
  int lo = 0, hi = 0;
  EESEN_HIP_CHECK(hipDeviceGetStreamPriorityRange(&lo, &hi));
  EESEN_HIP_CHECK(hipStreamCreateWithPriority(&st2.s, hipStreamNonBlocking, lo));
  tn = Tuning::from_env();
  persistent = tn.persistent;
  gate_fwd = tn.gate_fwd >= 0 ? tn.gate_fwd != 0 : gemm_mode() == 0;
  overlap = tn.overlap >= 0 ? tn.overlap != 0 : persistent != 0;
  spin_limit = tn.spin_limit;
  if (tn.trace) {
    trace.reserve(1280);
    EESEN_HIP_CHECK(hipMemset(trace.p, 0, 1280 * sizeof(unsigned long long)));
  }
  ctl.reserve(kCtlWords);
  EESEN_HIP_CHECK(hipMemset(ctl.p, 0, kCtlWords * sizeof(unsigned)));
  {
    constexpr float kFwdNs = 400.f, kBwdNs = 280.f, kBwdSideNs = 420.f, kRefFlightNs = 400.f;
    flight_ns = handoff_flight_ns();
    const float fscale = flight_ns >= 300.f && flight_ns <= 700.f ? 1.f : flight_ns / kRefFlightNs;
    auto ticks = [&](float ns) { return std::min(300, std::max(0, (int)std::lround(fscale * ns / 10.f))); };
    delay_fwd = ticks(kFwdNs); delay_bwd = ticks(kBwdNs); delay_bwd_side = ticks(kBwdSideNs);
    if (const char* e = tn.poll_ns) {
      int a = -1, b2 = -1;
      if (sscanf(e, "%d,%d", &a, &b2) == 2) { delay_fwd = a / 10; delay_bwd = delay_bwd_side = b2 / 10; poll_raw = 1; }
    }
    if (tn.print_flight)
      fprintf(stderr, "eesen_hip: increment flight %.0f ns; first-poll delays forward %d0, backward %d0 (beside side-stream GEMMs %d0) ns\n", flight_ns, delay_fwd, delay_bwd, delay_bwd_side);
  }
}

Net::~Net() {
  (void)hipSetDevice(device);
  (void)hipStreamSynchronize(st);
  for (StatGuard* g : guards) {
    (void)hipStreamSynchronize(g->st);
    g->word = nullptr;
    g->net = nullptr;
  }
  if (trace.p) {
    std::vector<unsigned long long> h(1280);
    if (hipMemcpy(h.data(), trace.p, h.size() * 8, hipMemcpyDeviceToHost) == hipSuccess)
      for (int pass = 0; pass < 2; ++pass) {
        double seg[5] = {0, 0, 0, 0, 0};
        int n = 0;
        for (int s = 8; s < 120; ++s) {
          const unsigned long long* a = h.data() + pass * 640 + s * 5;
          if (!a[0] || !a[5]) continue;
          seg[0] += (double)(a[1] - a[0]); seg[1] += (double)(a[2] - a[1]); seg[2] += (double)(a[3] - a[2]);
          seg[3] += (double)(a[4] - a[3]); seg[4] += (double)(a[5] - a[4]);
          ++n;
        }
        if (n) fprintf(stderr, "EESEN_TRACE %s: wait %.0f | A-load+MFMA+reduce %.0f | epilogue %.0f | drain+barrier %.0f | publish->next %.0f ticks/step (%d steps)\n",
                       pass ? "bwd" : "fwd", seg[0] / n, seg[1] / n, seg[2] / n, seg[3] / n, seg[4] / n, n);
      }
  }
  if (st2) (void)hipStreamSynchronize(st2);
}

void StatGuard::hook(Net* n, int device, hipStream_t stream, const char* entry_point) {
  if (n && !(n->device == device && n->st == stream))
    throw Error(EESEN_ERR_INVALID, std::string(entry_point) + ": the loss object and the Net must live on the same device and stream");
  unhook();
  if (!n || !n->ctl.p) return;
  word = n->ctl.p + kCtlWords - 1;
  net = n;
  st = stream;
  n->guards.push_back(this);
}

void StatGuard::unhook() {
  if (net) net->guards.erase(std::remove(net->guards.begin(), net->guards.end(), this), net->guards.end());
  word = nullptr;
  net = nullptr;
}

void StatGuard::note_dropped(const char* what) {
  if (dropped++ == 0 || dropped % 100 == 0)
    fprintf(stderr, "WARNING (eesen_hip) %s statistics of a minibatch computed from a timed-out forward pass were dropped (%ld so far)\n", what, dropped);
}

void Net::sync() {
  EESEN_HIP_CHECK(hipSetDevice(device));
  EESEN_HIP_CHECK(hipStreamSynchronize(st));
  wait_buckets_host();
  comm_check_alive(comm);
  check_device_error(true);
}

void Net::check_device_error(bool consumer) {
  if (!ctl.p) return;
  unsigned e = 0;
  EESEN_HIP_CHECK(hipMemcpy(&e, ctl.p + kCtlWords - 1, sizeof(unsigned), hipMemcpyDeviceToHost));
  if (!e) { steps_since_clean = 0; return; }
  EESEN_HIP_CHECK(hipStreamSynchronize(st));
  EESEN_HIP_CHECK(hipMemset(ctl.p + kCtlWords - 1, 0, sizeof(unsigned)));
  const bool only_waiter = e == 2 && tn.fwd_mid;
  if (only_waiter) tn.fwd_mid = 0;
  else { persistent = 0; gate_fwd = false; overlap = false; }
  ++recoveries;
  const int lost = std::max(1, steps_since_clean);
  steps_since_clean = 0;
  const bool rerun = consumer && propagated && input.p && rows > 0;
  const char* what = comm ? "contributed a ZERO gradient to the data-parallel sum (the ranks' models stay identical)" : "were NOT applied";
  if (only_waiter)
    fprintf(stderr, "WARNING (eesen_hip) the side stream's wait for a forward-recurrence milestone gave up (kernels serialised by a tool?): "
                    "%d minibatch(es) in flight %s%s; continuing without the early input GEMM (EESEN_FWD_MID=0)\n", lost, what,
            rerun ? " and the last forward pass is re-run" : "");
  else
    fprintf(stderr, "WARNING (eesen_hip) a persistent recurrence kernel gave up waiting for a peer workgroup (GPU shared or preempted?): "
                    "%d minibatch(es) in flight %s%s; continuing with the one-launch-per-step kernels\n", lost, what,
            rerun ? " and the last forward pass is re-run" : "");
  if (rerun) {
    forward_pass();
    EESEN_HIP_CHECK(hipStreamSynchronize(st));
  }
}

void Net::arm_device_error_poll() {
  if (!ctl.p) return;
  if (!err_pin.p) *static_cast<unsigned*>(err_pin.reserve(sizeof(unsigned))) = 0;
  EESEN_HIP_CHECK(hipMemcpyAsync(err_pin.p, ctl.p + kCtlWords - 1, sizeof(unsigned), hipMemcpyDeviceToHost, st));
  err_pin.used(st);
  err_armed = true;
}

void Net::poll_device_error() {
  if (!err_armed || !err_pin.ev.query()) return;
  err_armed = false;
  if (*err_pin.as<unsigned>()) check_device_error(false);
  else steps_since_clean = 0;
}

void Net::add_layer(int kind, int din, int dout, float coef, float max_grad) {
  EESEN_REQUIRE(!finalized, EESEN_ERR_STATE, "net already finalized");
  EESEN_REQUIRE(din > 0 && dout > 0, EESEN_ERR_INVALID, "layer dimensions must be positive");
  const Layer* prev = layers.empty() ? nullptr : &layers.back();
  if (prev)
    EESEN_REQUIRE(prev->dout_f == din, EESEN_ERR_INVALID, "Dimensionality mismatch between consecutive layers");
  Layer L;
  L.kind = kind; L.coef = coef; L.max_grad = max_grad;
  L.din_f = din; L.dout_f = dout;
  L.din = prev ? prev->dout : din;
  if (prev) { L.in_nb = prev->out_nb; L.in_hf = prev->out_hf; L.in_hi = prev->out_hi; }
  L.dout = dout;
  const char* sees_pad = "directly on an LSTM layer whose cell count per direction is not a multiple of 4 is not supported: it would see the "
                         "zero cells the library pads such a layer with";
  switch (kind) {
    case EESEN_LAYER_BILSTM_PARALLEL:
      EESEN_REQUIRE(dout % 2 == 0, EESEN_ERR_INVALID, "<CellDim> of a BiLstm layer must be even");
      L.ndir = 2; L.Hf = dout / 2;
      break;
    case EESEN_LAYER_LSTM_PARALLEL:
      L.ndir = 1; L.Hf = dout;
      break;
    case EESEN_LAYER_AFFINE:
      break;
    case EESEN_LAYER_SOFTMAX:
      EESEN_REQUIRE(din == dout, EESEN_ERR_INVALID, "Softmax needs InputDim == OutputDim");
      if (L.in_nb) throw Error(EESEN_ERR_INVALID, std::string("a <Softmax> ") + sees_pad);
      break;
    case EESEN_LAYER_SIGMOID:
    case EESEN_LAYER_TANH:
      EESEN_REQUIRE(din == dout, EESEN_ERR_INVALID, "an activation layer needs InputDim == OutputDim");
      if (L.in_nb && kind == EESEN_LAYER_SIGMOID) throw Error(EESEN_ERR_INVALID, std::string("a <Sigmoid> ") + sees_pad + " (sigmoid(0) = 1/2)");
      L.dout = L.din;
      L.out_nb = L.in_nb; L.out_hf = L.in_hf; L.out_hi = L.in_hi;
      break;
    default:
      throw Error(EESEN_ERR_INVALID, "unsupported layer kind " + std::to_string(kind));
  }
  if (L.is_lstm()) {
    L.H = pad4(L.Hf);
    L.dout = L.ndir * L.H;
    if (L.H != L.Hf) { L.out_nb = L.ndir; L.out_hf = L.Hf; L.out_hi = L.H; }
  }
  layers.push_back(std::move(L));
}

void Net::finalize() {
  EESEN_REQUIRE(!finalized, EESEN_ERR_STATE, "net already finalized");
  EESEN_REQUIRE(!layers.empty(), EESEN_ERR_INVALID, "empty net");
  EESEN_HIP_CHECK(hipSetDevice(device));
  size_t off = 0;
  for (Layer& L : layers) {
    L.p_off = off;
    size_t n = 0;
    if (L.is_lstm()) {
      const size_t H = L.H, D4 = pad4(L.din), nd = L.ndir;
      L.off_wx = n;   n += nd * 4 * H * D4;
      L.off_bias = n; n += nd * 4 * H;
      L.off_wm = n;   n += nd * 4 * H * H;
      L.off_peep = n; n += nd * 3 * H;
      L.WmT.reserve(nd * H * 4 * H);
    } else if (L.kind == EESEN_LAYER_AFFINE) {
      L.off_w = n; n += (size_t)L.dout * pad4(L.din);
      L.off_b = n; n += pad4(L.dout);
    }
    L.p_n = (n + 3) & ~(size_t)3;
    off += L.p_n;
  }
  P = off;
  if (P) {
    params.reserve(P); corr.reserve(P); fresh.reserve(P + kLiveWords);
    EESEN_HIP_CHECK(hipMemsetAsync(params.p, 0, P * sizeof(float), st));
    EESEN_HIP_CHECK(hipMemsetAsync(corr.p, 0, P * sizeof(float), st));
    EESEN_HIP_CHECK(hipMemsetAsync(fresh.p, 0, (P + kLiveWords) * sizeof(float), st));
  }
  if (tn.overlap < 0)
    for (const Layer& L : layers)
      if (L.is_lstm() && L.H > 512) overlap = false;
  amax.reserve(1 + layers.size());
  EESEN_HIP_CHECK(hipMemsetAsync(amax.p, 0, amax.cap * sizeof(float), st));
  EESEN_HIP_CHECK(hipMemsetD32Async(reinterpret_cast<hipDeviceptr_t>(amax.p), 0x3f800000, 1, st));
  finalized = true;
  refresh_derived();
  sync();
}

void Net::measure(const float* Pm, long nrows, int cols, int ld, DevBuf<float>& out_rows, DevBuf<float>& out_cols) {
  out_rows.reserve((size_t)nrows);
  out_cols.reserve((size_t)cols);
  amax_ws.reserve((size_t)kAmaxBlocks * std::min(16384, (cols + 3) & ~3));
  amax_rows_cols(st, Pm, nrows, cols, ld, out_rows.p, out_cols.p, amax_ws.p);
}
bool Net::x_is_bounded(int li) const {
  if (li == 0) return false;
  const Layer& Pv = layers[li - 1];
  return (Pv.is_lstm() && !Pv.cur_fwd_drop) || Pv.is_activation() || Pv.kind == EESEN_LAYER_SOFTMAX;
}
void Net::ensure_weight_amax() {
  const bool mode2 = gemm_mode() == 2;
  const bool need_w = mode2 && !wamax_valid;
  if (wm_valid && !need_w) return;
  if (!wm_valid) EESEN_HIP_CHECK(hipMemsetAsync(am_wm(0), 0, layers.size() * sizeof(float), st));
  for (size_t li = 0; li < layers.size(); ++li) {
    Layer& L = layers[li];
    if (L.is_lstm()) {
      if (need_w) measure(params.p + L.p_off + L.off_wx, (long)L.ndir * 4 * L.H, pad4(L.din), pad4(L.din), L.bw.rows, L.bw.cols);
      if (!wm_valid) amax_abs_accumulate(st, params.p + L.p_off + L.off_wm, (long)L.ndir * 4 * L.H, L.H, L.H, am_wm((int)li));
    } else if (L.kind == EESEN_LAYER_AFFINE && need_w) measure(params.p + L.p_off + L.off_w, L.dout, pad4(L.din), pad4(L.din), L.bw.rows, L.bw.cols);
  }
  wm_valid = true;
  if (mode2) wamax_valid = true;
}

long Net::num_params() const {
  long n = 0;
  for (const Layer& L : layers) n += L.file_params();
  return n;
}

void Net::init_accu() {
  if (accu_init) return;
  accu.reserve(P);
  EESEN_HIP_CHECK(hipMemsetAsync(accu.p, 0, P * sizeof(float), st));
  accu_init = true;
}

void Net::refresh_derived() {
  wamax_valid = wm_valid = false;
  for (Layer& L : layers)
    if (L.is_lstm())
      for (int dir = 0; dir < L.ndir; ++dir)
        transpose2d(st, params.p + L.p_off + L.off_wm + (size_t)dir * 4 * L.H * L.H, 4 * L.H, L.H,
                    L.WmT.p + (size_t)dir * L.H * 4 * L.H);
}

int Net::tensor_moments(int which, int layer, double* out6_host, int cap_tensors) {
  EESEN_REQUIRE(finalized, EESEN_ERR_STATE, "net not finalized");
  EESEN_REQUIRE(layer >= 0 && layer < (int)layers.size(), EESEN_ERR_INVALID, "layer index out of range");
  EESEN_REQUIRE(which >= 0 && which <= 2, EESEN_ERR_INVALID, "which: 0 parameters, 1 momentum buffers, 2 accumulators");
  const Layer& L = layers[layer];
  struct Region { size_t off; long rows; int cols; long ld; int nb, hf, hi; };
  std::vector<Region> reg;
  if (L.is_lstm()) {
    const int H = L.H, Hf = L.Hf, D4 = pad4(L.din);
    for (int dir = 0; dir < L.ndir; ++dir) {
      reg.push_back({L.off_wx + (size_t)dir * 4 * H * D4, 4L * Hf, L.din_f, D4, L.in_nb, L.in_hf, L.in_hi});
      reg.push_back({L.off_wm + (size_t)dir * 4 * H * H, 4L * Hf, Hf, H, 0, 0, 0});
      reg.push_back({L.off_bias + (size_t)dir * 4 * H, 1, 4 * Hf, 4L * H, 0, 0, 0});
      for (int g = 0; g < 3; ++g) reg.push_back({L.off_peep + ((size_t)dir * 3 + g) * H, 1, Hf, H, 0, 0, 0});
    }
  } else if (L.kind == EESEN_LAYER_AFFINE) {
    reg.push_back({L.off_w, L.dout, L.din_f, pad4(L.din), L.in_nb, L.in_hf, L.in_hi});
    reg.push_back({L.off_b, 1, L.dout, L.dout, 0, 0, 0});
  }
  const int n = (int)reg.size();
  if (!out6_host || n == 0) return n;
  EESEN_REQUIRE(cap_tensors >= n, EESEN_ERR_INVALID, "moments buffer too small");
  EESEN_HIP_CHECK(hipSetDevice(device));
  if (which == 2) init_accu();
  sync();
  const float* base = (which == 0 ? params.p : which == 1 ? corr.p : accu.p) + L.p_off;
  DevBuf<double> d;
  d.reserve((size_t)n * 6 + 8);
  for (int i = 0; i < n; ++i)
    eesen::tensor_moments(st, base + reg[i].off, reg[i].rows, reg[i].cols, reg[i].ld, d.p + (size_t)i * 6, d.p + (size_t)n * 6, reg[i].nb, reg[i].hf, reg[i].hi);
  EESEN_HIP_CHECK(hipStreamSynchronize(st));
  EESEN_HIP_CHECK(hipMemcpy(out6_host, d.p, (size_t)n * 6 * sizeof(double), hipMemcpyDeviceToHost));
  return n;
}

static void upload_flat(Net& net, DevBuf<float>& dst, const float* host, long n) {
  EESEN_REQUIRE(net.finalized, EESEN_ERR_STATE, "net not finalized");
  EESEN_REQUIRE(n == net.num_params(), EESEN_ERR_INVALID, "parameter count mismatch");
  EESEN_HIP_CHECK(hipSetDevice(net.device));
  std::vector<float> h(net.P, 0.f);
  long base = 0;
  for (const Layer& L : net.layers) {
    for_each_param(L, [&](long fi, size_t io) { h[L.p_off + io] = host[base + fi]; });
    base += L.file_params();
  }
  net.sync();
  if (net.P) EESEN_HIP_CHECK(hipMemcpy(dst.p, h.data(), net.P * sizeof(float), hipMemcpyHostToDevice));
}

void Net::set_params(const float* host, long n) {
  upload_flat(*this, params, host, n);
  refresh_derived();
  sync();
}

void Net::set_accu(const float* host, long n) {
  init_accu();
  upload_flat(*this, accu, host, n);
}

void Net::get_flat(const DevBuf<float>& buf, float* host, long n) {
  EESEN_REQUIRE(finalized, EESEN_ERR_STATE, "net not finalized");
  EESEN_REQUIRE(n == num_params(), EESEN_ERR_INVALID, "parameter count mismatch");
  sync();
  std::vector<float> h(P);
  if (P) EESEN_HIP_CHECK(hipMemcpy(h.data(), buf.p, P * sizeof(float), hipMemcpyDeviceToHost));
  long base = 0;
  for (const Layer& L : layers) {
    for_each_param(L, [&](long fi, size_t io) { host[base + fi] = h[L.p_off + io]; });
    base += L.file_params();
  }
}

void Net::set_seq_lengths(const int* l, int s) {
  EESEN_REQUIRE(s > 0, EESEN_ERR_INVALID, "need at least one sequence");
  EESEN_HIP_CHECK(hipSetDevice(device));
  lens.assign(l, l + s);
  for (int v : lens) EESEN_REQUIRE(v >= 0, EESEN_ERR_INVALID, "negative sequence length");
  poll_device_error();
  lens_d.reserve(s);
  int* pinned = static_cast<int*>(lens_pin.reserve(s * sizeof(int), std::max<size_t>(64, (size_t)s * 2) * sizeof(int)));
  std::copy(lens.begin(), lens.end(), pinned);
  EESEN_HIP_CHECK(hipMemcpyAsync(lens_d.p, pinned, s * sizeof(int), hipMemcpyHostToDevice, st));
  lens_pin.used(st);
  S = s;
  propagated = false;
}

static LstmLayerDev lstm_view(const Net& net, const Layer& L, int T) {
  LstmLayerDev d;
  d.T = T; d.S = net.S; d.H = L.H; d.ndir = L.ndir;
  d.G = L.G.p; d.C = L.C.p; d.Y = L.Y.p;
  d.X = L.X.p;
  d.Wm = net.params.p + L.p_off + L.off_wm;
  d.WmT = L.WmT.p;
  d.peep = net.params.p + L.p_off + L.off_peep;
  d.lens = net.lens_d.p;
  d.rmask = L.cur_drop_mode ? L.rmask.p : nullptr;
  d.drop_mode = L.cur_drop_mode;
  d.fwd_bf16 = net.fwd_bf16_rec ? 1 : 0;
  d.fwd_split = net.tn.fwd_split;
  d.fwd_f16 = net.tn.fwd_f16 && net.tn.fwd_split;
  d.bwd_f16 = net.tn.bwd_f16 && net.tn.fwd_split;
  d.wm_amax = net.amax.p ? const_cast<Net&>(net).am_wm((int)(&L - net.layers.data())) : nullptr;
  d.xcd_map = net.tn.xcd_map; d.fwd_mux = net.tn.fwd_mux; d.bwd_q4 = net.tn.bwd_q4; d.bwd_q4_st8 = net.tn.bwd_q4_st8; d.fwd_narrow2 = net.tn.fwd_narrow2; d.fwd_t16_small = net.tn.fwd_t16_small; d.bwd_ksplit = net.tn.bwd_ksplit; d.bwd_mux = net.tn.bwd_mux;
  return d;
}

void Net::set_layer_dropout(int layer, const float* nine) {
  EESEN_REQUIRE(layer >= 0 && layer < (int)layers.size(), EESEN_ERR_INVALID, "layer index out of range");
  Layer& L = layers[layer];
  bool any = false;
  for (int k = 0; k < 9; ++k) any |= nine[k] != 0.f;
  EESEN_REQUIRE(!any || L.kind == EESEN_LAYER_BILSTM_PARALLEL, EESEN_ERR_INVALID, "dropout options exist on BiLstm layers only");
  EESEN_REQUIRE(nine[0] >= 0.f && nine[0] < 1.f && nine[7] >= 0.f && nine[7] < 1.f, EESEN_ERR_INVALID, "dropout factor outside [0, 1)");
  for (int k = 0; k < 9; ++k) L.drop[k] = (k == 0 || k == 7) ? nine[k] : (nine[k] != 0.f ? 1.f : 0.f);
}

void Net::get_layer_dropout(int layer, float* nine) const {
  EESEN_REQUIRE(layer >= 0 && layer < (int)layers.size(), EESEN_ERR_INVALID, "layer index out of range");
  for (int k = 0; k < 9; ++k) nine[k] = layers[layer].drop[k];
}

static void widen_mask(const Layer& L, const float* src, long n, std::vector<float>& dst, const char* what) {
  dst.clear();
  if (!src) return;
  const long wf = (long)L.ndir * L.Hf, wi = (long)L.ndir * L.H;
  EESEN_REQUIRE(n > 0 && n % wf == 0, EESEN_ERR_INVALID, std::string(what) + ": the float count is not a multiple of the layer's ndir * H columns");
  if (wf == wi) { dst.assign(src, src + n); return; }
  const long rows = n / wf;
  dst.assign((size_t)rows * wi, 0.f);
  for (long r = 0; r < rows; ++r)
    for (int d = 0; d < L.ndir; ++d)
      std::copy(src + r * wf + (long)d * L.Hf, src + r * wf + (long)(d + 1) * L.Hf, dst.begin() + r * wi + (long)d * L.H);
}

void Net::set_dropout_masks(int layer, const float* fwd, long fwd_n, const float* rec, int rec_rows, long rec_n, int coin) {
  EESEN_REQUIRE(layer >= 0 && layer < (int)layers.size() && layers[layer].is_lstm(), EESEN_ERR_INVALID, "not an LSTM layer");
  Layer& L = layers[layer];
  if (rec) EESEN_REQUIRE(rec_rows > 0 && rec_n == (long)rec_rows * L.ndir * L.Hf, EESEN_ERR_INVALID, "recurrent mask: rec_floats must be rec_rows x ndir * H");
  widen_mask(L, fwd, fwd ? fwd_n : 0, L.inj_fmask, "forward mask");
  widen_mask(L, rec, rec ? rec_n : 0, L.inj_rmask, "recurrent mask");
  L.inj_rmask_rows = rec ? rec_rows : 0;
  L.inj_coin = coin;
}

void Net::get_dropout_masks(int layer, float* fwd_host, float* rec_host, int* info4) {
  EESEN_REQUIRE(layer >= 0 && layer < (int)layers.size() && layers[layer].is_lstm(), EESEN_ERR_INVALID, "not an LSTM layer");
  EESEN_REQUIRE(propagated, EESEN_ERR_STATE, "no Propagate yet");
  Layer& L = layers[layer];
  EESEN_HIP_CHECK(hipSetDevice(device));
  sync();
  const size_t ldY = (size_t)L.ndir * L.H, wf = (size_t)L.ndir * L.Hf;
  auto fetch = [&](float* host, const float* dev, size_t nrows) {
    if (wf == ldY) { EESEN_HIP_CHECK(hipMemcpy(host, dev, nrows * ldY * sizeof(float), hipMemcpyDeviceToHost)); return; }
    std::vector<float> tmp(nrows * ldY);
    EESEN_HIP_CHECK(hipMemcpy(tmp.data(), dev, tmp.size() * sizeof(float), hipMemcpyDeviceToHost));
    for (size_t r = 0; r < nrows; ++r)
      for (int d = 0; d < L.ndir; ++d)
        std::copy(tmp.begin() + r * ldY + (size_t)d * L.H, tmp.begin() + r * ldY + (size_t)d * L.H + L.Hf, host + r * wf + (size_t)d * L.Hf);
  };
  if (fwd_host && L.cur_fwd_drop) fetch(fwd_host, L.fmask.p, (size_t)rows);
  if (rec_host && L.cur_drop_mode) fetch(rec_host, L.rmask.p, (size_t)(T + 2) * S);
  if (info4) { info4[0] = L.cur_fwd_drop; info4[1] = L.cur_drop_mode; info4[2] = L.cur_twiddle_coin; info4[3] = (int)wf; }
}

static void prepare_dropout(Net& net, Layer& L) {
  L.cur_fwd_drop = false; L.cur_drop_mode = 0; L.cur_twiddle_coin = false;
  const bool want = net.in_train && L.has_dropout();
  if (!want) { L.inj_fmask.clear(); L.inj_rmask.clear(); L.inj_rmask_rows = 0; L.inj_coin = -1; return; }
  const float fwd_p = L.drop[0], rec_p = L.drop[7];
  const bool fw_seq = L.drop[2] != 0.f, rec_step = L.drop[3] != 0.f, rec_seq = L.drop[4] != 0.f;
  const bool rnndrop = L.drop[5] != 0.f, nml = L.drop[6] != 0.f, twiddle = L.drop[8] != 0.f;
  const int T = net.T, S = net.S, ldY = L.ndir * L.H;
  bool coin = false;
  if (twiddle) {
    if (L.inj_coin >= 0) coin = L.inj_coin != 0;
    else {
      unsigned long long z = net.drop_seed + (++net.drop_counter) * 0x9E3779B97F4A7C15ull;
      z = (z ^ (z >> 30)) * 0xBF58476D1CE4E5B9ull; z = (z ^ (z >> 27)) * 0x94D049BB133111EBull; z ^= z >> 31;
      coin = (z >> 63) != 0;
    }
  }
  L.cur_twiddle_coin = coin;
  const bool rec = (rnndrop || nml) && (!twiddle || !coin);
  const bool fwd = fwd_p > 0.f && (!twiddle || coin);
  if (rec) {
    EESEN_REQUIRE(rec_step != rec_seq, EESEN_ERR_INVALID,
                  "recurrent dropout needs exactly one of RecurrentTimeStepDropout / RecurrentSequenceDropout (bilstm-layer.h:102-113)");
    EESEN_REQUIRE(!(rnndrop && nml), EESEN_ERR_INVALID, "RNNDrop and NoMemLossDropout are mutually exclusive");
    const long mrows = (long)(T + 2) * S;
    L.rmask.reserve((size_t)mrows * ldY);
    if (!L.inj_rmask.empty()) {
      EESEN_REQUIRE((L.inj_rmask_rows == mrows || L.inj_rmask_rows == S) && (long)L.inj_rmask.size() == (long)L.inj_rmask_rows * ldY,
                    EESEN_ERR_INVALID, "injected recurrent mask has the wrong shape");
      const size_t chunk = (size_t)L.inj_rmask_rows * ldY;
      for (long r0 = 0; r0 < mrows; r0 += L.inj_rmask_rows)
        EESEN_HIP_CHECK(hipMemcpyAsync(L.rmask.p + (size_t)r0 * ldY, L.inj_rmask.data(), chunk * sizeof(float), hipMemcpyHostToDevice, net.st));
      EESEN_HIP_CHECK(hipStreamSynchronize(net.st));
    } else {
      dropout_mask(net.st, L.rmask.p, mrows, ldY, ldY, rec_p, net.drop_seed + (++net.drop_counter) * 0x632BE59BD9B4E019ull, rec_seq);
    }
    L.cur_drop_mode = rnndrop ? 2 : 1;
  }
  if (fwd) {
    L.fmask.reserve((size_t)net.rows * ldY);
    L.Yd.reserve((size_t)net.rows * ldY);
    if (!L.inj_fmask.empty()) {
      EESEN_REQUIRE((long)L.inj_fmask.size() == (long)net.rows * ldY, EESEN_ERR_INVALID, "injected forward mask has the wrong shape");
      EESEN_HIP_CHECK(hipMemcpyAsync(L.fmask.p, L.inj_fmask.data(), L.inj_fmask.size() * sizeof(float), hipMemcpyHostToDevice, net.st));
      EESEN_HIP_CHECK(hipStreamSynchronize(net.st));
    } else {
      dropout_mask(net.st, L.fmask.p, net.rows, ldY, ldY, fwd_p, net.drop_seed + (++net.drop_counter) * 0x632BE59BD9B4E019ull, fw_seq);
    }
    L.cur_fwd_drop = true;
  }
  L.inj_fmask.clear(); L.inj_rmask.clear(); L.inj_rmask_rows = 0; L.inj_coin = -1;
}

void Net::propagate(const float* in, int nrows, int ld, bool is_device) {
  EESEN_REQUIRE(finalized, EESEN_ERR_STATE, "net not finalized");
  EESEN_REQUIRE(S > 0, EESEN_ERR_STATE, "SetSeqLengths must precede Propagate");
  EESEN_REQUIRE(nrows > 0 && nrows % S == 0, EESEN_ERR_INVALID, "row count must be a positive multiple of the sequence count");
  const int D = layers[0].din, D4 = pad4(D);
  EESEN_REQUIRE(ld >= D, EESEN_ERR_INVALID, "input leading dimension smaller than InputDim");
  EESEN_HIP_CHECK(hipSetDevice(device));
  rows = nrows;
  T = rows / S;
  for (int v : lens) EESEN_REQUIRE(v <= T, EESEN_ERR_INVALID, "sequence length exceeds the number of frames");
  timer.reset();

  if (input.reserve((size_t)rows * D4) || D4 != D) EESEN_HIP_CHECK(hipMemsetAsync(input.p, 0, (size_t)rows * D4 * sizeof(float), st));
  if (is_device) {
    EESEN_HIP_CHECK(hipMemcpy2DAsync(input.p, (size_t)D4 * sizeof(float), in, (size_t)ld * sizeof(float), (size_t)D * sizeof(float), rows,
                                     hipMemcpyDeviceToDevice, st));
  } else {
    PinBuf& hs = in_stage[in_stage_idx++ & 1];
    const size_t bytes = (size_t)rows * D * sizeof(float);
    float* staged = static_cast<float*>(hs.reserve(bytes, bytes + bytes / 4));
    for (int r = 0; r < rows; ++r) std::memcpy(staged + (size_t)r * D, in + (size_t)r * ld, (size_t)D * sizeof(float));
    EESEN_HIP_CHECK(hipMemcpy2DAsync(input.p, (size_t)D4 * sizeof(float), staged, (size_t)D * sizeof(float), (size_t)D * sizeof(float), rows,
                                     hipMemcpyHostToDevice, st));
    hs.used(st);
  }
  forward_pass();
}

void Net::forward_pass() {
  const float* x = input.p;
  int ldx = pad4(layers[0].din);
  ++steps_since_clean;
  info_fwd_persistent = info_lstm_layers = info_fwd_bf16 = 0;
  bool g_gated = false;
  int gated_rows = 0;
  int mid_r0 = 0, mid_r1 = 0;
  const bool half = gemm_mode() == 2;
  ensure_weight_amax();
  amx_valid = half;
  for (Layer& L : layers) {
    const int li_ = (int)(&L - layers.data());
    GemmBound x_amax, w_amax;
    if (half && L.trainable()) {
      if (x_is_bounded(li_)) x_amax = bound_one();
      else { measure(x, rows, L.din, ldx, L.bx.rows, L.bx.cols); x_amax = GemmBound{L.bx.rows.p, 1}; }
      w_amax = GemmBound{L.bw.rows.p, 1};
    }
    if (L.is_lstm()) {
      const int H = L.H, nd = L.ndir, ldY = nd * H, ldG = nd * 4 * H;
      L.G.reserve((size_t)rows * ldG);
      const size_t state = (size_t)(T + 2) * S * ldY;
      L.C.reserve(state);
      L.Y.reserve(state);
      if (persistent && H % 32 == 0) L.X.reserve((size_t)T * nd * ((S + 15) / 16) * (size_t)(H / 32) * 768);
      const size_t blk = (size_t)S * ldY * sizeof(float);
      EESEN_HIP_CHECK(hipMemsetAsync(L.C.p, 0, blk, st));
      EESEN_HIP_CHECK(hipMemsetAsync(L.Y.p, 0, blk, st));
      EESEN_HIP_CHECK(hipMemsetAsync(L.C.p + (size_t)(T + 1) * S * ldY, 0, blk, st));
      EESEN_HIP_CHECK(hipMemsetAsync(L.Y.p + (size_t)(T + 1) * S * ldY, 0, blk, st));
      prepare_dropout(*this, L);
      if (g_gated) {
        if (gated_rows < rows) {
          const int ti_ = timer.begin(st, 0);
          gemm_f32(st, true, true, rows - gated_rows, ldG, L.din, 1.f, x + (size_t)gated_rows * ldx, ldx, params.p + L.p_off + L.off_wx,
                   pad4(L.din), 0.f, L.G.p + (size_t)gated_rows * ldG, ldG, params.p + L.p_off + L.off_bias, nullptr, 0, 0, fwd_bf16, x_amax, w_amax);
          timer.end(st, ti_);
        }
        EESEN_HIP_CHECK(hipStreamWaitEvent(st, ev_gate_done, 0));
        g_gated = false;
      } else if (mid_r1 > mid_r0) {
        const int ti_ = timer.begin(st, 0);
        const int parts[2][2] = {{0, mid_r0}, {mid_r1, rows}};
        for (const auto& pr : parts)
          if (pr[1] > pr[0])
            gemm_f32(st, true, true, pr[1] - pr[0], ldG, L.din, 1.f, x + (size_t)pr[0] * ldx, ldx, params.p + L.p_off + L.off_wx, pad4(L.din),
                     0.f, L.G.p + (size_t)pr[0] * ldG, ldG, params.p + L.p_off + L.off_bias, nullptr, 0, 0, fwd_bf16, x_amax, w_amax);
        timer.end(st, ti_);
        EESEN_HIP_CHECK(hipStreamWaitEvent(st, ev_gate_done, 0));
        mid_r0 = mid_r1 = 0;
      } else {
        const int ti_ = timer.begin(st, 0);
        gemm_f32(st, true, true, rows, ldG, L.din, 1.f, x, ldx, params.p + L.p_off + L.off_wx, pad4(L.din), 0.f, L.G.p, ldG,
                 params.p + L.p_off + L.off_bias, nullptr, 0, 0, fwd_bf16, x_amax, w_amax);
        timer.end(st, ti_);
      }
      Layer* nxt = (&L - layers.data()) + 1 < (long)layers.size() ? &layers[(&L - layers.data()) + 1] : nullptr;
      LstmLayerDev v = lstm_view(*this, L, T);
      const RecPlan fp = persistent ? lstm_fwd_plan(v) : RecPlan{};
      const bool pers = fp.kind != kRecNone;
      const bool plan_gate = pers && overlap && gate_fwd && !fwd_bf16 && !L.cur_fwd_drop && fp.units <= 8 && nxt && nxt->is_lstm() && T >= 2 && rows >= 128 &&
                             fp.one_window &&
                             (nxt->ndir * 4 * nxt->H) % 128 == 0 && ldY % 16 == 0 && nd * fp.seq_tiles * kShards <= 64;
      const int mile_step = (3 * T) / 4;
      const bool plan_mid = pers && overlap && tn.fwd_mid && !plan_gate && !L.cur_fwd_drop && fp.leaves_room && nd == 2 && nxt && nxt->is_lstm() &&
                            T >= 32 && mile_step + 1 < T && fp.one_window;
      { const int ti_ = timer.begin(st, 1);
      v.poll_delay = delay_fwd;
      v.poll_raw = poll_raw;
      if (plan_mid) {
        mile.reserve(32);
        EESEN_HIP_CHECK(hipMemsetAsync(mile.p, 0, 2 * sizeof(unsigned), st));
        EESEN_HIP_CHECK(hipEventRecord(ev_gate_reset, st));
        v.milestone = mile.p;
        v.milestone_step = mile_step;
      }
      if (pers) lstm_fwd_launch(st, fp, v, ctl.p, ctl.p + kCtlWords - 1, spin_limit, trace.p, plan_gate ? ev_gate_reset.get() : nullptr);
      else
        for (int step = 0; step < T; ++step) lstm_fwd_step(st, v, step);
      info_fwd_persistent += pers ? 1 : 0;
      info_fwd_bf16 += fp.bf16 ? 1 : 0;
      ++info_lstm_layers;
      check_launch("lstm_fwd");
      timer.end(st, ti_);
      if (pers && plan_gate) {
        const int ldG2 = nxt->ndir * 4 * nxt->H;
        nxt->G.reserve((size_t)rows * ldG2);
        EESEN_HIP_CHECK(hipStreamWaitEvent(st2, ev_gate_reset, 0));
        const int tj_ = timer.begin(st2, 0);
        GemmGate gate{ctl.p, ctl.p + kCtlWords - 1, nd, fp.seq_tiles, fp.grid[0], T, S, spin_limit};
        gated_rows = rows / 128 * 128;
        gemm_f32_nt_gated(st2, gated_rows, ldG2, ldY, L.Y.p + (size_t)S * ldY, ldY, params.p + nxt->p_off + nxt->off_wx, pad4(nxt->din),
                          nxt->G.p, ldG2, params.p + nxt->p_off + nxt->off_bias, gate, half ? bound_one() : GemmBound{}, half ? GemmBound{nxt->bw.rows.p, 1} : GemmBound{});
        timer.end(st2, tj_);
        EESEN_HIP_CHECK(hipEventRecord(ev_gate_done, st2));
        g_gated = true;
      }
      if (plan_mid) {
        EESEN_HIP_CHECK(hipMemsetD32Async(reinterpret_cast<hipDeviceptr_t>(mile.p + 1), 1, 1, st));
        const int ldG2 = nxt->ndir * 4 * nxt->H;
        nxt->G.reserve((size_t)rows * ldG2);
        mid_r0 = ((T - 1 - mile_step) * S + 255) / 256 * 256;
        mid_r1 = (mile_step + 1) * S / 256 * 256;
        if (mid_r1 <= mid_r0) mid_r0 = mid_r1 = 0;
      }
      if (plan_mid && mid_r1 > mid_r0) {
        const int ldG2 = nxt->ndir * 4 * nxt->H;
        EESEN_HIP_CHECK(hipStreamWaitEvent(st2, ev_gate_reset, 0));
        wait_for_word(st2, mile.p + 1, 1u, ctl.p + kCtlWords - 1, 2.0 * std::max(1.0, T / 1000.0) * std::max(1.0, spin_limit / 400000.0));
        const int tj_ = timer.begin(st2, 0);
        gemm_f32(st2, true, true, mid_r1 - mid_r0, ldG2, nxt->din, 1.f, L.Y.p + (size_t)S * ldY + (size_t)mid_r0 * ldY, ldY,
                 params.p + nxt->p_off + nxt->off_wx, pad4(nxt->din), 0.f, nxt->G.p + (size_t)mid_r0 * ldG2, ldG2,
                 params.p + nxt->p_off + nxt->off_bias, nullptr, 0,  64, fwd_bf16,
                 half ? bound_one() : GemmBound{}, half ? GemmBound{nxt->bw.rows.p, 1} : GemmBound{});
        timer.end(st2, tj_);
        EESEN_HIP_CHECK(hipEventRecord(ev_gate_done, st2));
      } }
      if (L.cur_fwd_drop)
        mul_elements(st, L.Y.p + (size_t)S * ldY, ldY, L.fmask.p, ldY, L.Yd.p, ldY, rows, ldY);
      x = L.output(S);
      ldx = ldY;
    } else if (L.kind == EESEN_LAYER_AFFINE) {
      const int ldo = pad4(L.dout);
      if (L.out.reserve((size_t)rows * ldo)) EESEN_HIP_CHECK(hipMemsetAsync(L.out.p, 0, L.out.cap * sizeof(float), st));
      { const int ti_ = timer.begin(st, 2);
      gemm_f32(st, true, true, rows, L.dout, L.din, 1.f, x, ldx, params.p + L.p_off + L.off_w, pad4(L.din), 0.f, L.out.p, ldo,
               params.p + L.p_off + L.off_b, nullptr, 0, 0, fwd_bf16, x_amax, w_amax);
      timer.end(st, ti_); }
      x = L.out.p;
      ldx = ldo;
    } else if (L.is_activation()) {
      const int ldo = pad4(L.dout);
      if (L.out.reserve((size_t)rows * ldo)) EESEN_HIP_CHECK(hipMemsetAsync(L.out.p, 0, L.out.cap * sizeof(float), st));
      { const int ti_ = timer.begin(st, 2);
      activation_rows(st, L.kind == EESEN_LAYER_TANH, x, ldx, L.out.p, ldo, rows, L.dout);
      timer.end(st, ti_); }
      x = L.out.p;
      ldx = ldo;
    } else {
      const int ldo = pad4(L.dout);
      if (L.out.reserve((size_t)rows * ldo)) EESEN_HIP_CHECK(hipMemsetAsync(L.out.p, 0, L.out.cap * sizeof(float), st));
      { const int ti_ = timer.begin(st, 2);
      softmax_rows(st, x, ldx, L.out.p, ldo, rows, L.dout);
      timer.end(st, ti_); }
      x = L.out.p;
      ldx = ldo;
    }
  }
  out_ptr = x;
  out_cols = layers.back().dout;
  out_ld = ldx;
  if (const Layer& Lb = layers.back(); Lb.out_nb) {
    const int ldo = pad4(Lb.dout_f);
    if (out_f.reserve((size_t)rows * ldo) && ldo != Lb.dout_f) EESEN_HIP_CHECK(hipMemsetAsync(out_f.p, 0, out_f.cap * sizeof(float), st));
    for (int b = 0; b < Lb.out_nb; ++b) copy2d(st, x + (size_t)b * Lb.out_hi, ldx, out_f.p + (size_t)b * Lb.out_hf, ldo, rows, Lb.out_hf);
    out_ptr = out_f.p; out_cols = Lb.dout_f; out_ld = ldo;
  }
  propagated = true;
  if (persistent) arm_device_error_poll();
}

void Net::backpropagate(const float* out_diff, int ldd, float* in_diff, int ldi) {
  bucket_log.clear();
  deferred_buckets.clear();
  try {
    backpropagate_impl(out_diff, ldd, in_diff, ldi);
  } catch (...) {
    fail_step_buckets();
    throw;
  }
}

void Net::backpropagate_impl(const float* out_diff, int ldd, float* in_diff, int ldi) {
  EESEN_REQUIRE(propagated, EESEN_ERR_STATE, "Backpropagate needs a preceding Propagate");
  EESEN_HIP_CHECK(hipSetDevice(device));
  int maxdim = 0, max_g = 0, max_y = 0;
  size_t need_ws = 0;
  for (const Layer& L : layers) {
    maxdim = std::max(maxdim, std::max(pad4(L.din), pad4(L.dout)));
    if (L.is_lstm()) {
      max_g = std::max(max_g, L.ndir * 4 * L.H);
      max_y = std::max(max_y, L.ndir * L.H);
      need_ws = std::max(need_ws, lstm_bias_peep_ws_floats(T, S, L.H, L.ndir));
    }
    need_ws = std::max(need_ws, col_sums_ws_floats(rows, L.dout));
  }
  need_ws = std::max(need_ws, (size_t)16 << 20);
  ws.reserve(need_ws);
  ws_floats = need_ws;
  dA.reserve((size_t)rows * maxdim);
  dB.reserve((size_t)rows * maxdim);
  if (max_g) {
    DGb[0].reserve((size_t)rows * max_g);
    DGb[1].reserve((size_t)rows * max_g);
  }
  if (max_y) DCF.reserve((size_t)S * max_y);
  ws2.reserve(need_ws);
  int dg_slot = 0;
  bool side_pending[2] = {false, false};
  deferred_buckets.clear();
  const std::vector<RecPlan> bwd = bwd_plans(T);
  const bool overlap = overlap_for_minibatch(bwd);
  exchange_deferred = comm && exchange_deferred_for_minibatch(bwd);
  bucket_log.clear();
  info_bwd_persistent = 0;
  live_valid = comm != nullptr;
  if (comm) {
    comm_check_alive(comm);
    EESEN_HIP_CHECK(hipMemsetD32Async(reinterpret_cast<hipDeviceptr_t>(fresh.p + P), 0x3f800000, 1, st));
  }

  const int Kout = layers.back().dout;
  float* d = dA.p;
  int ld_d = pad4(Kout);
  float* dn = dB.p;
  const bool half = gemm_mode() == 2;
  ensure_weight_amax();
  auto x_cols = [&](int li) -> GemmBound {
    if (!half || !amx_valid) return GemmBound{};
    return x_is_bounded(li) ? bound_one() : GemmBound{layers[li].bx.cols.p, 1};
  };
  if (const Layer& Lb = layers.back(); Lb.out_nb) {
    EESEN_HIP_CHECK(hipMemsetAsync(d, 0, (size_t)rows * ld_d * sizeof(float), st));
    for (int b = 0; b < Lb.out_nb; ++b) copy2d(st, out_diff + (size_t)b * Lb.out_hf, ldd, d + (size_t)b * Lb.out_hi, ld_d, rows, Lb.out_hf);
  } else {
    if (ld_d != Kout) EESEN_HIP_CHECK(hipMemsetAsync(d, 0, (size_t)rows * ld_d * sizeof(float), st));
    copy2d(st, out_diff, ldd, d, ld_d, rows, Kout);
  }

  for (int li = (int)layers.size() - 1; li >= 0; --li) {
    Layer& L = layers[li];
    const float* x;
    int ldx;
    if (li == 0) { x = input.p; ldx = pad4(L.din); }
    else {
      const Layer& Pv = layers[li - 1];
      if (Pv.is_lstm()) { ldx = Pv.ndir * Pv.H; x = Pv.output(S); }
      else { ldx = pad4(Pv.dout); x = Pv.out.p; }
    }
    const bool want_in = li > 0 || in_diff != nullptr;
    const int ld_n = pad4(L.din);
    float* fr = fresh.p + L.p_off;
    if (L.kind == EESEN_LAYER_SOFTMAX) {
      continue;
    } else if (L.is_activation()) {
      { const int ti_ = timer.begin(st, 4);
      activation_diff_rows(st, L.kind == EESEN_LAYER_TANH, L.out.p, pad4(L.dout), d, ld_d, rows, L.dout);
      timer.end(st, ti_); }
      continue;
    } else if (L.kind == EESEN_LAYER_AFFINE) {
      { const int ti_ = timer.begin(st, 4);
      if (half) measure(d, rows, L.dout, ld_d, L.bd.rows, L.bd.cols);
      if (want_in) {
        if (ld_n != L.din) EESEN_HIP_CHECK(hipMemsetAsync(dn, 0, (size_t)rows * ld_n * sizeof(float), st));
        gemm_f32(st, true, false, rows, L.din, L.dout, 1.f, d, ld_d, params.p + L.p_off + L.off_w, pad4(L.din), 0.f, dn, ld_n,
                 nullptr, nullptr, 0, 0, false, half ? GemmBound{L.bd.rows.p, 1} : GemmBound{}, half ? GemmBound{L.bw.cols.p, 1} : GemmBound{});
      }
      gemm_f32(st, false, false, L.dout, L.din, rows, 1.f, d, ld_d, x, ldx, 0.f, fr + L.off_w, pad4(L.din), nullptr, ws.p, ws_floats, 0, false,
               half ? GemmBound{L.bd.cols.p, 1} : GemmBound{}, x_cols(li));
      col_sums(st, d, rows, L.dout, ld_d, fr + L.off_b, ws.p, ws_floats);
      timer.end(st, ti_); }
      bucket_allreduce(li, st);
    } else {
      const int H = L.H, nd = L.ndir, ldG = nd * 4 * H, ldY = nd * H;
      LstmLayerDev v = lstm_view(*this, L, T);
      v.poll_delay = overlap ? delay_bwd_side : delay_bwd;
      v.poll_raw = poll_raw;
      const RecPlan& bp = bwd[li];
      if (bp.need_px) { bwd_px.reserve(bp.need_px); v.PX = bwd_px.p; v.px_floats = bwd_px.cap; }
      if (bp.need_dgh) {
        bwd_dgh.reserve((size_t)rows * ldG);
        bwd_ex.reserve(bp.need_ex);
        v.DGH = reinterpret_cast<unsigned char*>(bwd_dgh.p);
        v.EX = bwd_ex.p;
      }
      EESEN_REQUIRE(in_train || !L.has_dropout(), EESEN_ERR_STATE, "Can't backpropagate a dropout layer in test mode (bilstm-parallel-layer.h:425)");
      if (L.cur_fwd_drop) mul_elements(st, d, ld_d, L.fmask.p, ldY, d, ld_d, rows, ldY);
      float* DGl = DGb[dg_slot].p;
      if (side_pending[dg_slot]) {
        EESEN_HIP_CHECK(hipStreamWaitEvent(st, ev_grad[dg_slot], 0));
        side_pending[dg_slot] = false;
      }
      { const int ti_ = timer.begin(st, 3);
      if (bp.kind != kRecNone) {
        lstm_bwd_launch(st, bp, v, d, ld_d, DGl, ctl.p + kCtlHalf, ctl.p + kCtlWords - 1, spin_limit, trace.p ? trace.p + 640 : nullptr);
        ++info_bwd_persistent;
      } else
        for (int step = 0; step < T; ++step) lstm_bwd_step(st, v, step, d, ld_d, DGl, DCF.p);
      check_launch("lstm_bwd");
      timer.end(st, ti_); }
      if (half) { const int ti_ = timer.begin(st, 4); measure(DGl, rows, ldG, ldG, L.bd.rows, L.bd.cols); timer.end(st, ti_); }
      EESEN_HIP_CHECK(hipEventRecord(ev_rec, st));
      if (want_in) {
        const int ti_ = timer.begin(st, 4);
        if (ld_n != L.din) EESEN_HIP_CHECK(hipMemsetAsync(dn, 0, (size_t)rows * ld_n * sizeof(float), st));
        gemm_f32(st, true, false, rows, L.din, ldG, 1.f, DGl, ldG, params.p + L.p_off + L.off_wx, pad4(L.din), 0.f, dn, ld_n,
                 nullptr, nullptr, 0, 0, false, half ? GemmBound{L.bd.rows.p, 1} : GemmBound{}, half ? GemmBound{L.bw.cols.p, 1} : GemmBound{});
        timer.end(st, ti_);
        EESEN_HIP_CHECK(hipEventRecord(ev_rec, st));
      }
      hipStream_t sg = overlap ? st2 : st;
      const int side_lds_env = (tn.side_lds_kb >= 0 ? tn.side_lds_kb : (gemm_mode() >= 1 ? 48 : 32)) * 1024;
      bool lstm_below = false;
      for (int lj = 0; lj < li; ++lj) lstm_below |= layers[lj].is_lstm();
      const int side_lds = overlap && lstm_below ? side_lds_env : 0;
      if (overlap) EESEN_HIP_CHECK(hipStreamWaitEvent(st2, ev_rec, 0));
      { const int ti_ = timer.begin(sg, 4);
      gemm_f32(sg, false, false, ldG, L.din, rows, 1.f, DGl, ldG, x, ldx, 0.f, fr + L.off_wx, pad4(L.din), nullptr, ws2.p, need_ws, side_lds, false,
               half ? GemmBound{L.bd.cols.p, 1} : GemmBound{}, x_cols(li));
      for (int dir = 0; dir < nd; ++dir)
        gemm_f32(sg, false, false, 4 * H, H, rows, 1.f, DGl + (size_t)dir * 4 * H, ldG,
                 L.Y.p + (size_t)(dir == 0 ? 0 : 2 * S) * ldY + (size_t)dir * H, ldY, 0.f,
                 fr + L.off_wm + (size_t)dir * 4 * H * H, H, nullptr, ws2.p, need_ws, side_lds, false,
                 half ? GemmBound{L.bd.cols.p + (size_t)dir * 4 * H, 1} : GemmBound{}, half ? bound_one() : GemmBound{});
      lstm_bias_peep_grads(sg, v, DGl, fr + L.off_bias, fr + L.off_peep, ws2.p, need_ws);
      timer.end(sg, ti_); }
      bucket_allreduce(li, sg);
      if (overlap) {
        EESEN_HIP_CHECK(hipEventRecord(ev_grad[dg_slot], st2));
        side_pending[dg_slot] = true;
      }
      dg_slot ^= 1;
    }
    if (want_in) {
      std::swap(d, dn);
      ld_d = ld_n;
    }
  }
  if (in_diff) copy2d(st, d, ld_d, in_diff, ldi, rows, layers[0].din);
  flush_deferred_buckets();
  for (int k = 0; k < 2; ++k)
    if (side_pending[k]) EESEN_HIP_CHECK(hipStreamWaitEvent(st, ev_grad[k], 0));
}

std::vector<RecPlan> Net::bwd_plans(int T) const {
  std::vector<RecPlan> plans(layers.size());
  for (size_t li = 0; li < layers.size(); ++li)
    if (persistent && layers[li].is_lstm()) plans[li] = lstm_bwd_plan(lstm_view(*this, layers[li], T));
  return plans;
}
bool Net::overlap_for_minibatch(const std::vector<RecPlan>& bwd) const {
  bool ov = overlap;
  if (ov && tn.overlap < 0 && persistent)
    for (size_t li = 0; li < layers.size(); ++li)
      if (const Layer& L = layers[li]; L.is_lstm() && L.H > 320 && L.H <= 512 && S > 32 && !bwd[li].light) ov = false;
  return ov;
}
bool Net::exchange_deferred_for_minibatch(const std::vector<RecPlan>& bwd) const {
  if (tn.comm_defer >= 0) return tn.comm_defer != 0;
  if (!persistent) return false;
  for (const RecPlan& bp : bwd)
    if (bp.kind != kRecNone && bp.free_vgprs < kRcclVgprsPerSimdLane) return true;
  return false;
}

std::string Net::plan_string() const {
  EESEN_REQUIRE(finalized, EESEN_ERR_STATE, "net not finalized");
  EESEN_REQUIRE(S > 0, EESEN_ERR_STATE, "call eesen_net_set_seq_lengths first: the plan depends on the minibatch shape");
  EESEN_HIP_CHECK(hipSetDevice(device));
  int T = this->T;
  if (!propagated) { T = 0; for (int v : lens) T = std::max(T, v); }
  auto one = [](const RecPlan& P) {
    char b[512];
    if (P.kind == kRecNone) { snprintf(b, sizeof(b), "{\"kernel\": \"per-step kernels (lstm.hip)\", \"persistent\": false}"); return std::string(b); }
    snprintf(b, sizeof(b), "{\"kernel\": \"%s\", \"persistent\": true, \"sequences_per_workgroup\": %d, \"units_per_workgroup\": %d, \"grid\": [%d, %d, %d], "
             "\"workgroups\": %d, \"workgroups_per_cu\": %d, \"launches\": %d, \"vgprs\": %d, \"lds_bytes\": %d, \"free_vgprs_per_simd_lane\": %d}",
             P.kernel, P.seq_tile, P.units, P.grid[0], P.grid[1], P.grid[2], P.wgs, P.wgs_per_cu, P.windows, P.vgprs, P.lds, P.free_vgprs);
    return std::string(b);
  };
  const std::vector<RecPlan> bwd = bwd_plans(T);
  std::string o = "{\"T\": " + std::to_string(T) + ", \"S\": " + std::to_string(S) + ", \"persistent\": " + (persistent ? "true" : "false") + ", \"layers\": [";
  bool first = true;
  for (size_t li = 0; li < layers.size(); ++li) {
    const Layer& L = layers[li];
    if (!L.is_lstm()) continue;
    const RecPlan fp = persistent && T >= 1 ? lstm_fwd_plan(lstm_view(*this, L, T)) : RecPlan{}, &bp = bwd[li];
    o += std::string(first ? "" : ", ") + "{\"layer\": " + std::to_string(li) + ", \"cells\": " + std::to_string(L.H) + ", \"directions\": " + std::to_string(L.ndir) +
         ", \"forward\": " + one(fp) + ", \"backward\": " + one(bp) + "}";
    first = false;
  }
  const bool ov = overlap_for_minibatch(bwd);
  o += std::string("], \"weight_gradient_gemms\": \"") + (ov ? "side stream, under the next-lower recurrence" : "main stream, serial") + "\"";
  o += std::string(", \"gemm_arithmetic\": \"") + (gemm_mode() == 2 ? "two fp16 planes, three products (fp32-class)" : gemm_mode() == 1 ? "3-way bf16 split (fp32-class)" : "f32-input MFMA") + "\"";
  o += std::string(", \"exchange\": ") + (comm ? (exchange_deferred_for_minibatch(bwd) ? "\"deferred: every bucket behind the backward pass's last recurrence\""
                                                                                      : "\"overlapped: each bucket as soon as its layer's gradients are enqueued\"") : "null");
  o += std::string(", \"exchange_rule\": \"") + (tn.comm_defer >= 0 ? "EESEN_COMM_DEFER" : "auto: deferred when a persistent backward grid leaves < 256 registers per SIMD lane") + "\"";
  o += ", \"gpu_share\": " + std::to_string(gpu_share_value()) + "}";
  return o;
}

void Net::update() {
  EESEN_REQUIRE(finalized, EESEN_ERR_STATE, "net not finalized");
  EESEN_HIP_CHECK(hipSetDevice(device));
  const unsigned* skip = persistent && !grads_sanitized ? ctl.p + kCtlWords - 1 : nullptr;
  const float* live = comm && live_valid ? fresh.p + P : nullptr;
  comm_check_alive(comm);
  { const int ti_ = timer.begin(st, 5);
  for (int li = (int)layers.size() - 1; li >= 0; --li) {
    Layer& L = layers[li];
    if (L.p_n) {
      if (comm && li < (int)bucket_pending.size() && bucket_pending[li]) {
        const int tw_ = timer.begin(st, 7);
        EESEN_HIP_CHECK(hipStreamWaitEvent(st, ev_bucket[li], 0));
        timer.end(st, tw_);
        bucket_pending[li] = 0;
      }
      if (rule == 0) {
        sgd_update(st, params.p + L.p_off, corr.p + L.p_off, fresh.p + L.p_off, (long)L.p_n, mmt, lr * L.coef, L.max_grad, skip, live);
      } else {
        init_accu();
        adaptive_update(st, params.p + L.p_off, corr.p + L.p_off, fresh.p + L.p_off, accu.p + L.p_off, (long)L.p_n, mmt, lr,
                        L.max_grad, ada_eps, rms_rho, rms_one_minus_rho, rule == 2, skip, live);
      }
    }
  }
  refresh_derived();
  timer.end(st, ti_); }
  grads_sanitized = false;
  live_valid = false;
  if (persistent) arm_device_error_poll();
}

}
```

eesen_amd/csrc/net.h:

```cpp
#pragma once
#include <string>
#include <vector>

#include "kernels.h"
#include "lex.h"
#include "lm.h"
#include "tuning.h"

namespace eesen {

inline int pad4(int x) { return (x + 3) & ~3; }
constexpr size_t kCtlWords = 2 * kCtlHalf + 32;

struct Layer {
  int kind = 0, din = 0, dout = 0;
  float coef = 1.f, max_grad = 0.f;
  size_t p_off = 0, p_n = 0;
  int H = 0, ndir = 0;
  int din_f = 0, dout_f = 0, Hf = 0;
  int in_nb = 0, in_hf = 0, in_hi = 0, out_nb = 0, out_hf = 0, out_hi = 0;
  int in_col(int d) const { return in_nb ? (d / in_hf) * in_hi + d % in_hf : d; }
  size_t off_wx = 0, off_bias = 0, off_wm = 0, off_peep = 0;
  DevBuf<float> WmT;
  DevBuf<float> G, C, Y;
  DevBuf<float> X;
  size_t off_w = 0, off_b = 0;
  DevBuf<float> out;
  struct Bounds { DevBuf<float> rows, cols; } bw, bx, bd;
  float drop[9] = {0, 0, 0, 0, 0, 0, 0, 0, 0};
  bool has_dropout() const { return drop[0] > 0.f || drop[5] != 0.f || drop[6] != 0.f; }
  DevBuf<float> fmask;
  DevBuf<float> rmask;
  DevBuf<float> Yd;
  bool cur_fwd_drop = false;
  int cur_drop_mode = 0;
  bool cur_twiddle_coin = false;
  std::vector<float> inj_fmask, inj_rmask;
  int inj_rmask_rows = 0, inj_coin = -1;
  const float* output(int S) const { return cur_fwd_drop ? Yd.p : Y.p + (size_t)S * ndir * H; }
  bool is_lstm() const { return kind == EESEN_LAYER_LSTM_PARALLEL || kind == EESEN_LAYER_BILSTM_PARALLEL; }
  bool nonparallel = false;
  bool is_activation() const { return kind == EESEN_LAYER_SIGMOID || kind == EESEN_LAYER_TANH; }
  bool trainable() const { return is_lstm() || kind == EESEN_LAYER_AFFINE; }
  long file_params() const;
  const char* marker() const;
};

class PhaseTimer {
 public:
  void enable(bool on) { on_ = on; }
  bool enabled() const { return on_; }
  void set_accumulate(bool a) { accumulate_ = a; used_ = 0; }
  void reset() { if (!accumulate_) used_ = 0; }
  int begin(hipStream_t st, int phase);
  void end(hipStream_t st, int idx);
  void collect(float* out, int nphase);
  int spans(int* phases, float* secs, int cap);
 private:
  struct Span { DevEvent a{true}, b{true}; int phase = 0; };
  std::vector<Span> spans_;
  size_t used_ = 0;
  bool on_ = false, accumulate_ = false;
};

struct Comm;
void comm_check_alive(const Comm* c);
constexpr size_t kLiveWords = 4;
constexpr int kRcclVgprsPerSimdLane = 256;

struct StatGuard {
  const unsigned* word = nullptr;
  struct Net* net = nullptr;
  long dropped = 0;
  hipStream_t st = nullptr;
  StatGuard() = default;
  StatGuard(const StatGuard&) = delete;
  StatGuard& operator=(const StatGuard&) = delete;
  ~StatGuard() { unhook(); }
  void hook(struct Net* n, int device, hipStream_t stream, const char* entry_point);
  void unhook();
  void note_dropped(const char* what);
};

struct Net {
  int device = 0;
  hipStream_t st = nullptr;
  std::vector<Layer> layers;
  bool finalized = false;
  size_t P = 0;
  DevBuf<float> params, corr, fresh;
  float lr = 0.f, mmt = 0.f;
  int rule = 0;
  float ada_eps = 1e-6f, rms_rho = 0.9f, rms_one_minus_rho = 0.1f;
  DevBuf<float> accu;
  bool accu_init = false;
  void init_accu();
  void set_accu(const float* host, long n);
  std::vector<int> lens;
  DevBuf<int> lens_d;
  int T = 0, S = 0, rows = 0;
  bool propagated = false;
  DevBuf<float> input;
  PinBuf in_stage[2];
  unsigned in_stage_idx = 0;
  const float* out_ptr = nullptr;
  int out_cols = 0, out_ld = 0;
  DevBuf<float> out_f;
  DevBuf<float> DGb[2], DCF, dA, dB, ws, ws2;
  DevBuf<float> bwd_px;
  DevBuf<float> bwd_dgh, bwd_ex;
  DevStream st2;
  DevEvent ev_rec, ev_grad[2];
  bool overlap = true;
  DevEvent ev_gate_reset, ev_gate_done;
  DevBuf<unsigned> mile;
  bool gate_fwd = true;
  bool fwd_bf16 = false;
  bool fwd_bf16_rec = false;
  int info_fwd_bf16 = 0;
  DevBuf<unsigned> ctl;
  Tuning tn;
  int persistent = 1;
  int info_fwd_persistent = 0, info_bwd_persistent = 0, info_lstm_layers = 0;
  int spin_limit = 400000;
  float flight_ns = 0.f;
  int delay_fwd = 61, delay_bwd = 43, delay_bwd_side = 64, poll_raw = 0;
  int recoveries = 0;
  DevBuf<unsigned long long> trace;
  void check_device_error(bool consumer);
  int steps_since_clean = 0;
  PinBuf lens_pin, err_pin;
  bool err_armed = false;
  void poll_device_error();
  void arm_device_error_poll();
  bool in_train = true;
  unsigned long long drop_seed = 777, drop_counter = 0;
  void set_train_mode(bool train) { in_train = train; }
  void set_layer_dropout(int layer, const float* nine);
  void get_layer_dropout(int layer, float* nine) const;
  void set_dropout_masks(int layer, const float* fwd, long fwd_n, const float* rec, int rec_rows, long rec_n, int coin);
  void get_dropout_masks(int layer, float* fwd_host, float* rec_host, int* info4);
  size_t ws_floats = 0;
  DevBuf<float> amax, amax_ws;
  bool wamax_valid = false, wm_valid = false;
  bool amx_valid = false;
  float* am_wm(int li) { return amax.p + 1 + li; }
  GemmBound bound_one() const { return GemmBound{amax.p, 0}; }
  bool x_is_bounded(int li) const;
  void measure(const float* P, long rows, int cols, int ld, DevBuf<float>& out_rows, DevBuf<float>& out_cols);
  void ensure_weight_amax();
  PhaseTimer timer;
  Comm* comm = nullptr;
  std::vector<DevEvent> ev_ready, ev_bucket;
  std::vector<char> bucket_pending;
  std::vector<int> deferred_buckets;
  bool exchange_deferred = false;
  std::vector<RecPlan> bwd_plans(int T) const;
  bool overlap_for_minibatch(const std::vector<RecPlan>& bwd) const;
  bool exchange_deferred_for_minibatch(const std::vector<RecPlan>& bwd) const;
  std::string plan_string() const;
  DevEvent ev_bwd_done;
  void issue_bucket(int li);
  void fail_step_buckets() noexcept;
  void flush_deferred_buckets();
  std::vector<StatGuard*> guards;
  bool grads_sanitized = false;
  bool live_valid = false;
  std::vector<int> bucket_log;
  PinBuf live_pin;
  void set_comm(Comm* c);
  int top_trainable() const;
  int live_ranks();
  void bucket_allreduce(int li, hipStream_t producer);
  void wait_buckets_host();
  void backpropagate_zero();
  void allreduce_grads(Comm* c);

  Net(int device, void* stream);
  ~Net();
  void add_layer(int kind, int din, int dout, float coef, float max_grad);
  void finalize();
  long num_params() const;
  void set_params(const float* host, long n);
  void get_flat(const DevBuf<float>& buf, float* host, long n);
  void set_seq_lengths(const int* lens, int S);
  void propagate(const float* in, int rows, int ld, bool is_device);
  void forward_pass();
  void backpropagate(const float* out_diff, int ldd, float* in_diff, int ldi);
  void backpropagate_impl(const float* out_diff, int ldd, float* in_diff, int ldi);
  void update();
  void refresh_derived();
  int tensor_moments(int which, int layer, double* out6_host, int cap_tensors);
  void read(const std::string& path);
  void write(const std::string& path, bool binary);
  void sync();
};

inline void* loss_slot(PinBuf& pin, size_t bytes) { return pin.reserve(bytes, std::max<size_t>(bytes * 2, 4096)); }

struct Ctc {
  int device = 0;
  hipStream_t st = nullptr;
  DevBuf<float> logp, alpha, beta, pzx_d;
  DevBuf<int> labx, ids_d, ali_d;
  std::vector<int> last_lens;
  int last_T = 0, last_S = 0, last_Lpad = 0, last_Lprime = 0;
  int sweep_waves = 0;
  double obj_sum = 0;
  long sequences = 0, frames = 0, err_tokens = 0, ref_tokens = 0;
  DevEvent ev[4] = {DevEvent(true), DevEvent(true), DevEvent(true), DevEvent(true)};
  PhaseTimer timer;
  DevEvent aev[4] = {DevEvent(true), DevEvent(true), DevEvent(true), DevEvent(true)};
  PhaseTimer align_timer;
  PinBuf align_pin;
  DevBuf<float> dec_f;
  DevBuf<int> dec_i, dec_trie, dec_out;
  DevEvent dev[4] = {DevEvent(true), DevEvent(true), DevEvent(true), DevEvent(true)};
  PhaseTimer decode_timer;
  PinBuf decode_pin;
  int dec_rows = 0, dec_S = 0, dec_C = 0;
  std::vector<int> dec_lens;
  int dec_N = 0, dec_T = 0, dec_mode = 0, dec_space = -1;
  bool dec_fused = false;
  std::vector<int> dec_word, dec_word_len;
  DevBuf<int> stamp_i;
  DevEvent sev[4] = {DevEvent(true), DevEvent(true), DevEvent(true), DevEvent(true)};
  PhaseTimer stamp_timer;
  PinBuf stamp_pin;
  int stamp_group = 0;
  DevBuf<int> lm_i;
  DevBuf<float> lm_f;
  LmTables lm_tab{};
  unsigned long long lm_serial = 0;
  DevBuf<int> lex_i;
  LexTables lex_tab{};
  WordLexTables word_tab{};
  unsigned long long lex_serial = 0;
  PinBuf stage[2];
  unsigned stage_idx = 0;
  struct PendingPzx { PinBuf pin; int S = 0; long nframes = 0; bool active = false; } ppzx[2];
  struct PendingErr { PinBuf pin, probs; int S = 0, K = 0, rows = 0; bool active = false, with_probs = false, guarded = false; std::vector<int> frames, ids, off; } perr[2];
  StatGuard guard;
  std::string seq_out;
  unsigned ppzx_idx = 0, perr_idx = 0;
  void flush_pzx(PendingPzx& q);
  void flush_err(PendingErr& q, int* num_err, int* num_ref);
  void flush();

  Ctc(int device, void* stream);
  ~Ctc();
  void eval_parallel(const int* frame_num_utt, int S, const float* net_out, int rows, int K, int ld, const int* label_ids,
                     const int* label_off, float* diff, int ldd, float* pzx_host);
  void error_rate_mseq(const int* frame_num_utt, int S, const float* net_out, int rows, int K, int ld,
                       const int* label_ids, const int* label_off, int* num_err, int* num_ref);
  void get_alpha_beta(float* alpha_host, float* beta_host, int* Lprime);
  void phase_times(float* out3);
  void align_parallel(const int* frame_num_utt, int S, const float* scores, int rows, int K, int ld, bool is_log, const int* label_ids,
                      const int* label_off, int* ali_host, int* pos_host, float* score_host);
  void align_times(float* out3);
  void decode_parallel(const int* frame_num_utt, int S, const float* scores, int rows, int K, int ld, bool is_log, int beam, int max_classes,
                       int nbest, int* hyp_host, int* hyp_len_host, float* score_host);
  void decode_parallel_lm(const int* frame_num_utt, int S, const float* scores, int rows, int K, int ld, bool is_log, int beam, int max_classes,
                          int nbest, const TokenLm* lm, float lm_weight, float insertion_bonus, bool use_eos, int* hyp_host, int* hyp_len_host,
                          float* score_host, float* lm_score_host);
  void decode_parallel_lex(const int* frame_num_utt, int S, const float* scores, int rows, int K, int ld, bool is_log, int beam, int max_classes,
                           int nbest, const Lexicon* lex, const TokenLm* lm, float lm_weight, float word_bonus, bool use_eos, int* hyp_host,
                           int* hyp_len_host, float* score_host, float* lm_score_host, int* word_host, int* word_len_host);
  void decode_parallel_words(const int* frame_num_utt, int S, const float* scores, int rows, int K, int ld, bool is_log, int beam, int max_classes,
                             int nbest, const Lexicon* lex, const TokenLm* lm, float lm_weight, float word_bonus, bool use_eos, int* hyp_host,
                             int* hyp_len_host, float* score_host, float* lm_score_host, int* word_host, int* word_len_host, int* word_end_host);
  void decode_times(float* out3);
  void decode_stamps(const int* frame_num_utt, int S, const float* scores, int rows, int K, int ld, bool is_log, double conf_scale,
                     int* lstart_host, int* lend_host, int* wstart_host, int* wend_host, float* wconf_host, float* path_score_host);
  void stamp_times(float* out3);
  void get_decode_candidates(int* ids_host, float* scores_host, float* blank_host, int* Cc);
 private:
  struct Lattices { const int *labx, *lens, *lablens; int Lpad, Lprime; };
  Lattices upload_lattices(const int* frame_num_utt, int S, const int* label_ids, const int* label_off);
  void decode_batch(const int* frame_num_utt, int S, const float* scores, int rows, int K, int ld, bool is_log, int beam, int max_classes,
                    int nbest, const Lexicon* lex, const TokenLm* lm, float lm_weight, float insertion_bonus, bool use_eos, int* hyp_host,
                    int* hyp_len_host, float* score_host, float* lm_score_host);
  void upload_lm(const TokenLm& lm);
  void upload_lex(const Lexicon& lex);
};

void word_confidence(int n, const double* scores, const int* word_len, const int* word_ids, const int* wstart, const int* wend, int stride,
                     double conf_scale, double* conf_out);

int edit_distance(const int* ref, int nr, const int* hyp, int nh);

struct CeLoss {
  int device = 0;
  hipStream_t st = nullptr;
  DevBuf<int> tg;
  DevBuf<CeSums> part, res;
  PinBuf stage[2];
  unsigned stage_idx = 0;
  struct Pending { PinBuf pin; int S = 0; long rows = 0; bool active = false; } pend[2];
  unsigned pend_idx = 0;
  double obj = 0, obj_progress = 0;
  long correct = 0, frames = 0, sequences = 0, correct_progress = 0, frames_progress = 0, sequences_progress = 0;
  int report_step = 100;
  std::vector<std::string> progress;
  StatGuard guard;
  DevEvent ev[2] = {DevEvent(true), DevEvent(true)};
  PhaseTimer timer;

  CeLoss(int device, void* stream);
  ~CeLoss();
  void fold(Pending& q, double* obj_out);
  void flush();
  void eval_parallel(const int* frame_num_utt, int S, const float* net_out, int rows, int K, int ld, const int* targets,
                     float* diff, int ldd, double* obj_host);
  std::string report();
  void phase_times(float* out1);
};

}
```

eesen_amd/csrc/rec_kernels.h:

```cpp
#pragma once
#include "kernels.h"

namespace eesen {

constexpr int kRecWaves = 8;
struct RecRole { int nblk, ndir, nz, xcd; };

enum RecFamily { kFwdF32, kFwdBf, kFwdMux, kBwdGeneric, kBwdQ4, kBwdKsplit, kBwdKsplitH, kBwdKsplitMux };
struct RecKernel {
  int family;
  int kind;
  int arg[5];
  const void* fn;
  const char* name;
};
const RecKernel* rec_kernel(int family, int a0, int a1 = 0, int a2 = 0, int a3 = 0, int a4 = 0);
const void* handoff_pingpong_fn();
const void* wait_for_word_fn();

}
```

eesen_amd/csrc/rec_plan.cpp:

```cpp
#include "rec_kernels.h"

#include <atomic>
#include <map>
#include <mutex>
#include <tuple>

namespace eesen {
namespace {

constexpr int NW = kRecWaves;

std::atomic<int> g_share_override{0};
int gpu_share() {
  static const int env = [] { const char* e = getenv("EESEN_GPU_SHARE"); const int v = e && *e ? atoi(e) : 0; return v < 1 ? 0 : v; }();
  if (env) return env;
  const int o = g_share_override.load(std::memory_order_relaxed);
  return o > 0 ? o : 1;
}
int share_of_cus() {
  int ncu = 256, dev = 0;
  (void)hipGetDevice(&dev);
  (void)hipDeviceGetAttribute(&ncu, hipDeviceAttributeMultiprocessorCount, dev);
  return std::max(1, ncu / gpu_share());
}

template <class... Args>
void plan_launch(hipStream_t st, const void* fn, int wgs, Args... args) {
  void* argv[] = {static_cast<void*>(&args)...};
  EESEN_HIP_CHECK(hipLaunchKernel(fn, dim3(wgs), dim3(NW * 64), argv, 0, st));
}

bool bf_census(const RecKernel& k, int wgs) {
  static std::mutex mu;
  static std::map<std::tuple<int, const void*, int>, bool> seen;
  int dev = 0;
  if (hipGetDevice(&dev) != hipSuccess) return false;
  if (gpu_share() > 1) return false;
  std::lock_guard<std::mutex> lock(mu);
  const auto key = std::make_tuple(dev, k.fn, wgs);
  if (auto it = seen.find(key); it != seen.end()) return it->second;
  bool ok = false;
  unsigned* w = nullptr;
  if (hipDeviceSynchronize() == hipSuccess && hipMalloc(reinterpret_cast<void**>(&w), 2 * sizeof(unsigned)) == hipSuccess) {
    for (int take = 0; take < 3 && !ok; ++take) {
      if (hipMemset(w, 0, 2 * sizeof(unsigned)) != hipSuccess) break;
      LstmLayerDev L{};
      L.T = -1;
      unsigned* err = w + 1;
      int spin_limit = 0;
      unsigned long long* trace = nullptr;
      RecRole role{1, 1, 1, 0};
      void* argv[] = {&L, &w, &err, &spin_limit, &trace, &role};
      if (hipLaunchKernel(k.fn, dim3(wgs), dim3(NW * 64), argv, 0, nullptr) != hipSuccess) { (void)hipGetLastError(); break; }
      unsigned e = 1;
      ok = hipMemcpy(&e, w + 1, sizeof(unsigned), hipMemcpyDeviceToHost) == hipSuccess && e == 0;
    }
    (void)hipFree(w);
  }
  seen[key] = ok;
  if (getenv("EESEN_PRINT_PLAN")) fprintf(stderr, "LOG (eesen_hip) residency census: %d workgroups of %s on device %d: %s\n", wgs, k.name, dev, ok ? "seen co-resident" : "NOT seen");
  return ok;
}

bool fits(const RecKernel& k, dim3 grid, bool census = false) {
  int dev = 0, ncu = 0, nb = 0;
  if (hipGetDevice(&dev) != hipSuccess) return false;
  if (hipDeviceGetAttribute(&ncu, hipDeviceAttributeMultiprocessorCount, dev) != hipSuccess) return false;
  {
    static std::mutex mu;
    static std::map<std::pair<int, const void*>, int> cache;
    std::lock_guard<std::mutex> lock(mu);
    const auto key = std::make_pair(dev, k.fn);
    auto it = cache.find(key);
    if (it == cache.end()) {
      if (hipOccupancyMaxActiveBlocksPerMultiprocessor(&nb, k.fn, NW * 64, 0) != hipSuccess) return false;
      it = cache.emplace(key, nb).first;
    }
    nb = it->second;
  }
  const long wgs = (long)grid.x * grid.y * grid.z;
  if (wgs <= (long)ncu * std::max(1, nb - 1) / gpu_share()) return true;
  return census && wgs <= (long)ncu * nb / gpu_share() && bf_census(k, (int)wgs);
}


size_t ctl_words(size_t groups) { return groups * kShards * kShardStride; }

bool line_aligned(int seqs, int cols) { return ((size_t)seqs * cols * sizeof(float)) % 128 == 0; }

template <class F>
int pick_windows(int S, int seq_tile, F fits_with) {
  for (int nwin = 1; nwin <= 8; nwin *= 2) {
    if (S % nwin != 0 || (S / nwin) % seq_tile != 0) { if (nwin == 1 && fits_with(S)) return 1; continue; }
    if (fits_with(S / nwin)) return nwin;
  }
  return 0;
}

void take(RecPlan& P, const RecKernel& k, const dim3& grid, size_t words, int seq_tile, int units, int windows) {
  P.kind = k.kind; P.fn = k.fn; P.kernel = k.name;
  P.seq_tile = seq_tile; P.units = units; P.windows = windows; P.ctl_words = words;
  P.grid[0] = (int)grid.x; P.grid[1] = (int)grid.y; P.grid[2] = (int)grid.z;
  P.wgs = (int)(grid.x * grid.y * grid.z);
  P.wgs_per_cu = std::max(1, cdiv(P.wgs, share_of_cus()));
  static std::mutex mu;
  static std::map<const void*, std::pair<int, int>> cache;
  std::lock_guard<std::mutex> lock(mu);
  auto it = cache.find(P.fn);
  if (it == cache.end()) {
    hipFuncAttributes a{};
    if (hipFuncGetAttributes(&a, P.fn) != hipSuccess) { (void)hipGetLastError(); return; }
    it = cache.emplace(P.fn, std::make_pair((int)a.numRegs, (int)a.sharedSizeBytes)).first;
  }
  P.vgprs = it->second.first;
  P.lds = it->second.second;
  if (P.vgprs > 0) P.free_vgprs = 512 - P.wgs_per_cu * (NW / 4) * ((P.vgprs + 7) & ~7);
}

struct FwdTile { int mt, nt; };
struct BfPlan { bool on; int cpw, nt, ap, wp; bool f16; };

bool small_xchg(const LstmLayerDev& L, int bytes_per_unit_row) {
  return (size_t)L.T * L.ndir * cdiv(L.S, 16) * (size_t)(L.H / 32) * bytes_per_unit_row < ((size_t)1 << 31);
}
bool bf_fits(const LstmLayerDev& L, const BfPlan& P, int Sw) {
  const RecKernel* k = rec_kernel(kFwdBf, P.cpw, P.nt, P.ap, P.wp, P.f16);
  return k && fits(*k, dim3(L.H / (4 * P.nt), L.ndir, cdiv(Sw, 16)),  true);
}
bool narrow2_ok(const LstmLayerDev& L, int need) {
  const bool f16 = L.fwd_f16 && L.wm_amax != nullptr;
  if (!L.fwd_narrow2 || !(L.fwd_split || f16) || L.fwd_bf16 || L.X == nullptr || L.drop_mode || L.T < 2 || L.H % 32 != 0) return false;
  if (!small_xchg(L, 1024 * 3)) return false;
  return bf_fits(L, f16 ? BfPlan{true, need, 2, 2, 2, true} : BfPlan{true, need, 2, 3, 3, false}, L.S);
}
FwdTile fwd_tile(const LstmLayerDev& L) {
  const int need = ((L.H + 31) / 32 + NW - 1) / NW;
  const int ncu = share_of_cus();
  const bool t16_ok = L.H % 8 == 0 && (L.S > 16 || need > 2 || (L.fwd_t16_small && L.fwd_split && !L.drop_mode && L.X && L.H % 32 == 0));
  const long narrow_wgs = (long)(L.H / 8) * L.ndir * cdiv(L.S, 16);
  const bool narrow_full = narrow_wgs > ncu && !(narrow_wgs <= 2L * ncu && need <= 2 && narrow2_ok(L, need));
  if (t16_ok && L.H % 16 == 0 && need <= 4 && (need > 2 || narrow_full)) return {1, 4};
  if (t16_ok && need <= 2) return {1, 2};
  return {2, 1};
}

BfPlan bf_plan_shape(const LstmLayerDev& L, const FwdTile& ft) {
  const BfPlan off{false, 0, 0, 0, 0, false};
  if (L.X == nullptr || L.drop_mode || L.T < 2 || L.H % 32 != 0) return off;
  if (L.fwd_bf16) {
    if (L.H % 256 != 0 || L.H / 256 > 4 || !small_xchg(L, 1024)) return off;
    return {true, L.H / 256, 4, 1, 2, false};
  }
  const bool f16 = L.fwd_f16 && L.wm_amax != nullptr;
  if (L.fwd_split || f16) {
    const int need = (L.H / 32 + NW - 1) / NW;
    if (f16 && ft.mt == 1 && ft.nt == 4 && L.H % 256 == 0 && L.H / 256 <= 4 && small_xchg(L, 1024 * 2)) return {true, L.H / 256, 4, 2, 2, true};
    if (ft.mt != 1 || ft.nt != 2 || need > 2 || L.H % 8 != 0 || !small_xchg(L, 1024 * 3)) return off;
    if (f16) return {true, need, 2, 2, 2, true};
    if (L.fwd_split) return {true, need, 2, 3, 3, false};
  }
  return off;
}

bool bwd_ksplit_shape(const LstmLayerDev& L, int stile) {
  return L.bwd_ksplit && stile == 16 && !L.drop_mode && L.H % 256 == 0 && L.H >= 768 && L.H <= 1024 && L.T >= 2;
}
bool bwd_planes_shape(const LstmLayerDev& L, int stile) {
  const int cpw = L.H / (32 * NW);
  return L.bwd_f16 && L.wm_amax != nullptr && bwd_ksplit_shape(L, stile) && (cpw == 2 || cpw == 4) && L.H % (32 * NW) == 0;
}

}

void set_gpu_share(int n) { g_share_override.store(n < 1 ? 1 : n, std::memory_order_relaxed); }
int gpu_share_value() { return gpu_share(); }

float handoff_flight_ns() {
  static float cache[64] = {0};
  static std::mutex mu;
  std::lock_guard<std::mutex> lock(mu);
  int dev = 0;
  if (hipGetDevice(&dev) != hipSuccess || dev < 0 || dev >= 64) return 0.f;
  if (cache[dev] > 0.f) return cache[dev];
  unsigned* flags = nullptr;
  unsigned long long* out = nullptr;
  EESEN_HIP_CHECK(hipMalloc(reinterpret_cast<void**>(&flags), 64 * sizeof(unsigned)));
  EESEN_HIP_CHECK(hipMalloc(reinterpret_cast<void**>(&out), sizeof(unsigned long long)));
  int rounds = 2000;
  double ns[5];
  for (int rep = 0; rep < 5; ++rep) {
    EESEN_HIP_CHECK(hipMemset(flags, 0, 64 * sizeof(unsigned)));
    void* argv[] = {&flags, &out, &rounds};
    (void)hipLaunchKernel(handoff_pingpong_fn(), dim3(2), dim3(64), argv, 0, nullptr);
    unsigned long long ticks = 0;
    EESEN_HIP_CHECK(hipMemcpy(&ticks, out, sizeof(ticks), hipMemcpyDeviceToHost));
    ns[rep] = ticks ? 10.0 * (double)ticks / (2.0 * rounds) : 500.0;
  }
  std::sort(ns, ns + 5);
  (void)hipFree(flags);
  (void)hipFree(out);
  cache[dev] = (float)std::min(2000.0, std::max(100.0, ns[2]));
  return cache[dev];
}

void wait_for_word(hipStream_t st, const unsigned* word, unsigned target, unsigned* err, double limit_s) {
  unsigned long long ticks = (unsigned long long)(std::max(0.05, limit_s) * 1e8);
  void* argv[] = {&word, &target, &err, &ticks};
  (void)hipLaunchKernel(wait_for_word_fn(), dim3(1), dim3(64), argv, 0, st);
  check_launch("wait_for_word");
}

RecPlan lstm_fwd_plan(const LstmLayerDev& L) {
  RecPlan P;
  const int need = ((L.H + 31) / 32 + NW - 1) / NW;
  const FwdTile ft = fwd_tile(L);
  if (need > 4 || (ft.nt == 2 && need > 2) || L.H % (4 * ft.nt) != 0 || L.T < 2) return P;
  if (!line_aligned(L.S, L.ndir * L.H)) return P;
  if ((size_t)(L.T + 2) * L.S * L.ndir * L.H * sizeof(float) >= ((size_t)1 << 31)) return P;
  BfPlan B = bf_plan_shape(L, ft);
  const bool drop = L.drop_mode != 0;
  const int cpw32 = ft.nt == 2 ? std::min(need, 2) : need <= 2 ? need : 4;
  int nwin = B.on ? pick_windows(L.S, 16, [&](int Sw) { return bf_fits(L, B, Sw); }) : 0;
  if (nwin == 0) {
    B.on = false;
    const RecKernel* probe = rec_kernel(kFwdF32, cpw32, ft.mt, ft.nt, drop, false);
    nwin = pick_windows(L.S, 16 * ft.mt, [&](int Sw) { return probe && fits(*probe, dim3(L.H / (4 * ft.nt), L.ndir, cdiv(Sw, 16 * ft.mt))); });
  }
  if (nwin == 0) return P;
  if (nwin > 1 && !line_aligned(L.S / nwin, L.ndir * L.H)) return P;
  const int mt = B.on ? 1 : ft.mt, nt = B.on ? B.nt : ft.nt, nz = cdiv(L.S, 16 * mt);
  auto answer = [&](const RecKernel& k, const dim3& grid, size_t words, int seq_tile, int windows, bool one_window) {
    take(P, k, grid, words, seq_tile, 4 * nt, windows);
    P.seq_tiles = nz;
    P.one_window = one_window;
    P.leaves_room = nt <= 2 && (!B.on || (long)(L.H / (4 * nt)) * L.ndir * nz <= share_of_cus());
    P.bf16 = L.fwd_bf16 && k.kind == kRecFwdBf;
  };
  const dim3 grid(L.H / (4 * nt), L.ndir, cdiv(L.S / nwin, 16 * mt));
  const size_t words = ctl_words(grid.y * grid.z);
  if (B.on) {
    if (words <= (size_t)kCtlHalf) answer(*rec_kernel(kFwdBf, B.cpw, B.nt, B.ap, B.wp, B.f16), grid, words, 16, nwin, nwin == 1);
    return P;
  }
  const bool xchg = L.X != nullptr && ft.mt == 1 && L.H % 32 == 0 && !drop && small_xchg(L, 2048);
  if (L.fwd_mux && nwin == 2 && ft.mt == 1 && ft.nt == 4 && need > 2 && need <= 4 && !drop && L.H % 32 == 0) {
    const RecKernel& k = *rec_kernel(kFwdMux, 4, 4, xchg);
    const dim3 mgrid(L.H / 16, L.ndir, cdiv(nz, 2));
    if (fits(k, mgrid) && ctl_words((size_t)L.ndir * nz) <= (size_t)kCtlHalf) {
      answer(k, mgrid, ctl_words((size_t)L.ndir * nz), 32, 1, false);
      return P;
    }
  }
  if (words > (size_t)kCtlHalf) return P;
  const RecKernel* k = rec_kernel(kFwdF32, cpw32, ft.mt, ft.nt, drop, xchg);
  EESEN_REQUIRE(k != nullptr, EESEN_ERR_STATE, "no instantiation of the fp32 forward tile for this plan");
  answer(*k, grid, words, 16 * ft.mt, nwin, nwin == 1);
  return P;
}

void lstm_fwd_launch(hipStream_t st, const RecPlan& P, const LstmLayerDev& L0, unsigned* cnt, unsigned* err, int spin_limit,
                     unsigned long long* trace, hipEvent_t after_reset) {
  EESEN_REQUIRE(P.kind == kRecFwdBf || P.kind == kRecFwdMux || P.kind == kRecFwdF32, EESEN_ERR_STATE, "not a forward recurrence plan");
  const RecRole role{P.grid[0], P.grid[1], P.grid[2], L0.xcd_map};
  for (int w = 0; w < P.windows; ++w) {
    LstmLayerDev L = L0;
    if (P.kind == kRecFwdMux) { L.s_begin = 0; L.s_count = 0; }
    else { L.s_count = L0.S / P.windows; L.s_begin = w * L.s_count; }
    if (P.kind != kRecFwdMux && P.wgs_per_cu >= 2 && !L0.poll_raw) L.poll_delay = L0.poll_delay * 7 / 4;
    EESEN_HIP_CHECK(hipMemsetAsync(cnt, 0, sizeof(unsigned) * P.ctl_words, st));
    if (after_reset && P.one_window) EESEN_HIP_CHECK(hipEventRecord(after_reset, st));
    if (P.kind == kRecFwdMux) plan_launch(st, P.fn, P.wgs, L, cnt, err, spin_limit, role);
    else plan_launch(st, P.fn, P.wgs, L, cnt, err, spin_limit, trace, role);
  }
}

RecPlan lstm_bwd_plan(const LstmLayerDev& L) {
  RecPlan P;
  const int need = ((4 * L.H + 31) / 32 + NW - 1) / NW;
  const int ldG = L.ndir * 4 * L.H;
  const long blocks16 = (long)cdiv(L.H, 16) * L.ndir * cdiv(L.S, 16);
  const int stile = 2 * blocks16 <= share_of_cus() && L.S > 8 ? 8 : 16;
  P.light = stile == 8;
  if (need > 16 || L.T < 2) return P;
  if (!line_aligned(L.S, ldG)) return P;
  const size_t blk_bytes = (size_t)L.S * ldG * sizeof(float);
  const long max_blocks = (long)((((size_t)1 << 31) - 1) / blk_bytes);
  if (max_blocks < 3) return P;
  int chunk = (int)std::min<long>(L.T, max_blocks - 1);
  if (chunk < L.T) { int p2 = 1; while (p2 * 2 <= chunk) p2 *= 2; chunk = p2; }
  P.chunk = chunk;
  auto in_windows = [&](const RecKernel* k, int gx, int seq_tile, int units, int quarters) {
    if (!k) return false;
    auto grid_of = [&](int Sw) { return dim3(gx, L.ndir, cdiv(Sw, seq_tile)); };
    auto words_of = [&](const dim3& g) { return ctl_words((size_t)g.y * g.z * quarters); };
    const int nwin = pick_windows(L.S, seq_tile, [&](int Sw) { return words_of(grid_of(Sw)) <= (size_t)kCtlHalf && fits(*k, grid_of(Sw)); });
    if (nwin == 0 || (nwin > 1 && !line_aligned(L.S / nwin, ldG))) return false;
    take(P, *k, grid_of(L.S / nwin), words_of(grid_of(L.S / nwin)), seq_tile, units, nwin);
    return true;
  };
  for (int pass = 0; pass < 2; ++pass) {
    const int stq = (L.bwd_q4_st8 == 2) == (pass == 0) ? 8 : 4;
    if (!L.bwd_q4 || L.drop_mode || L.H % 32 != 0 || L.H > 512 || chunk < L.T) break;
    if (stq == 4 && stile != 8) continue;
    if (stq == 8 && !(L.bwd_q4_st8 && L.S > 8)) continue;
    const int cpw = 2 * ((L.H + 127) / 128);
    const dim3 grid(L.H / 32, L.ndir, cdiv(L.S, stq));
    const size_t words = ctl_words((size_t)grid.y * grid.z);
    const RecKernel& k = *rec_kernel(kBwdQ4, cpw, stq);
    if (fits(k, grid) && words <= (size_t)kCtlHalf) {
      take(P, k, grid, words, stq, 32, 1);
      return P;
    }
  }
  if (bwd_ksplit_shape(L, stile)) {
    const int cpw = L.H / (32 * NW), gx = L.H / 64 * 4;
    const size_t px = (size_t)2 * L.ndir * cdiv(L.S, 16) * (size_t)(L.H / 64) * 4096 * 2;
    if (bwd_planes_shape(L, stile) && in_windows(rec_kernel(kBwdKsplitH, cpw), gx, 16, 64, 4)) {
      P.need_px = px; P.need_dgh = true;
      P.need_ex = (size_t)L.T * L.ndir * cdiv(L.S, 16) * (size_t)(L.H / 16) * 16;
      return P;
    }
    const RecKernel* k = rec_kernel(kBwdKsplit, cpw);
    const int nwin = !k ? 0 : pick_windows(L.S, 16, [&](int Sw) {
      const dim3 grid(gx, L.ndir, cdiv(Sw, 16));
      return ctl_words((size_t)grid.y * grid.z * 4) <= (size_t)kCtlHalf && fits(*k, grid);
    });
    if (nwin == 2 && L.bwd_mux && cpw >= 2 && cpw <= 4) {
      const int nz = cdiv(L.S, 16);
      const dim3 grid(gx, L.ndir, cdiv(nz, 2));
      const size_t words = ctl_words((size_t)L.ndir * nz * 4);
      const RecKernel& km = *rec_kernel(kBwdKsplitMux, cpw);
      if (words <= (size_t)kCtlHalf && fits(km, grid)) {
        take(P, km, grid, words, 32, 64, 1);
        P.need_px = px;
        return P;
      }
    }
    if (nwin > 0 && (nwin == 1 || line_aligned(L.S / nwin, ldG))) {
      const dim3 grid(gx, L.ndir, cdiv(L.S / nwin, 16));
      take(P, *k, grid, ctl_words((size_t)grid.y * grid.z * 4), 16, 64, nwin);
      P.need_px = px;
      return P;
    }
  }
  in_windows(rec_kernel(kBwdGeneric, need <= 1 ? 1 : need <= 2 ? 2 : need <= 4 ? 4 : need <= 8 ? 8 : 16, stile, L.drop_mode != 0), cdiv(L.H, 16), stile, 16, 1);
  return P;
}

void lstm_bwd_launch(hipStream_t st, const RecPlan& P, const LstmLayerDev& L0, const float* dY, int lddy, float* DG, unsigned* cnt,
                     unsigned* err, int spin_limit, unsigned long long* trace) {
  EESEN_REQUIRE(P.kind == kRecBwdQ4 || P.kind == kRecBwdKsplit || P.kind == kRecBwdKsplitMux || P.kind == kRecBwdGeneric, EESEN_ERR_STATE, "not a backward recurrence plan");
  EESEN_REQUIRE(!P.need_px || (L0.PX && L0.px_floats >= P.need_px), EESEN_ERR_STATE, "the backward plan's partial-sum exchange space (RecPlan::need_px) was not handed over");
  EESEN_REQUIRE(!P.need_dgh || (L0.DGH && L0.EX), EESEN_ERR_STATE, "the backward plan's plane and exponent buffers (RecPlan::need_dgh, need_ex) were not handed over");
  const RecRole role{P.grid[0], P.grid[1], P.grid[2], L0.xcd_map};
  const bool whole_batch = P.kind == kRecBwdQ4 || P.kind == kRecBwdKsplitMux;
  unsigned long long* px = reinterpret_cast<unsigned long long*>(L0.PX);
  int chunk = P.chunk;
  for (int w = 0; w < P.windows; ++w) {
    LstmLayerDev L = L0;
    if (whole_batch) { L.s_begin = 0; L.s_count = 0; }
    else { L.s_count = L0.S / P.windows; L.s_begin = w * L.s_count; }
    EESEN_HIP_CHECK(hipMemsetAsync(cnt, 0, sizeof(unsigned) * P.ctl_words, st));
    if (P.need_px) EESEN_HIP_CHECK(hipMemsetAsync(L.PX, 0, sizeof(float) * P.need_px, st));
    if (P.kind == kRecBwdQ4) plan_launch(st, P.fn, P.wgs, L, dY, lddy, DG, cnt, err, spin_limit, trace, role);
    else if (P.kind == kRecBwdKsplitMux) plan_launch(st, P.fn, P.wgs, L, dY, lddy, DG, px, cnt, err, spin_limit, role, chunk);
    else if (P.kind == kRecBwdKsplit) plan_launch(st, P.fn, P.wgs, L, dY, lddy, DG, px, cnt, err, spin_limit, role, chunk, trace);
    else plan_launch(st, P.fn, P.wgs, L, dY, lddy, DG, cnt, err, spin_limit, trace, role, chunk);
  }
}

}
```

eesen_amd/csrc/tuning.h:

```cpp
#pragma once
#include <cstddef>
#include <cstdlib>

namespace eesen {

constexpr size_t kStampDeltaBytes = (size_t)1 << 30;

struct Tuning {
  int persistent = 1;
  int overlap = -1, gate_fwd = -1, side_lds_kb = -1;
  int spin_limit = 400000;
  bool spin_limit_set = false;
  int bwd_q4 = 1, bwd_q4_st8 = 1, fwd_narrow2 = 1, fwd_t16_small = 1, bwd_ksplit = 1, fwd_mux = 1, bwd_mux = 1, xcd_map = 1, fwd_mid = 1, fwd_split = 1, fwd_f16 = 1, bwd_f16 = 1;
  int comm_defer = -1;
  int trace = 0;
  bool print_flight = false;
  const char* poll_ns = nullptr;

  static Tuning from_env() {
    Tuning t;
    auto num = [](const char* name, int dflt) {
      const char* e = getenv(name);
      return e && *e ? atoi(e) : dflt;
    };
    t.persistent = num("EESEN_PERSISTENT", 1);
    t.overlap = num("EESEN_OVERLAP", -1);
    t.gate_fwd = num("EESEN_GATE_FWD", -1);
    t.fwd_mid = num("EESEN_FWD_MID", 1);
    t.side_lds_kb = num("EESEN_SIDE_LDS_KB", -1);
    t.spin_limit_set = getenv("EESEN_SPIN_LIMIT") != nullptr;
    t.spin_limit = num("EESEN_SPIN_LIMIT", 400000);
    t.bwd_q4 = num("EESEN_BWD_Q4", 1);
    t.bwd_q4_st8 = num("EESEN_BWD_Q4_ST8", 1);
    t.fwd_narrow2 = num("EESEN_FWD_NARROW2", 1);
    t.fwd_t16_small = num("EESEN_FWD_T16_SMALL", 1);
    t.bwd_ksplit = num("EESEN_BWD_KSPLIT", 1);
    t.fwd_mux = num("EESEN_FWD_MUX", 1);
    t.bwd_mux = num("EESEN_BWD_MUX", 1);
    t.fwd_split = num("EESEN_FWD_SPLIT", 1);
    t.fwd_f16 = num("EESEN_FWD_F16", 1);
    t.bwd_f16 = num("EESEN_BWD_F16", 1);
    t.xcd_map = num("EESEN_XCD_MAP", 1);
    t.comm_defer = num("EESEN_COMM_DEFER", -1);
    t.trace = num("EESEN_TRACE", 0);
    t.print_flight = getenv("EESEN_PRINT_FLIGHT") != nullptr;
    t.poll_ns = getenv("EESEN_POLL_NS");
    return t;
  }
};

}
```

Baseline: 995,300.

## Overlap late input-GEMM quadrants with guarded forward recurrence of next layer

Adds a guarded variant of the bf16 persistent forward LSTM kernel that runs its time loop in three segments, spinning on device guard words before the steps whose gate-input rows are computed late on the side stream. The host now computes only the gate-input quadrants the recurrence needs first, launches the recurrence, and computes the remaining quadrants concurrently. This removes part of the input-GEMM time from the critical path between layers. In exchange it adds device-side spin waits, a new kernel instantiation, and a recovery path (EESEN_FWD_QUAD=0) for when the guard wait times out.

```diff
diff --git a/eesen_amd/build.py b/eesen_amd/build.py
--- a/eesen_amd/build.py
+++ b/eesen_amd/build.py
@@ -11,7 +11,7 @@
 LIBDIR = os.path.join(_DIR, "lib")
 LIB = os.path.join(LIBDIR, "libeesen_hip.so")
 SOURCES = ["gemm.hip", "lstm.hip", "lstm_persistent.hip", "rec_plan.cpp", "ctc.hip", "ctc_decode.hip", "ce.hip", "optim.hip", "feeder.hip", "net.cpp", "ctc_host.cpp", "ce_host.cpp", "nnet_format.cpp", "lm.cpp", "lex.cpp", "capi.cpp", "comm.cpp"]
-HEADERS = ["common.h", "guard.h", "kernels.h", "rec_kernels.h", "net.h", "lm.h", "lex.h", "handles.h", "tuning.h", os.path.join("..", "..", "include", "eesen_hip.h")]
+HEADERS = ["common.h", "guard.h", "kernels.h", "rec_kernels.h", "net.h", "lm.h", "lex.h", "handles.h", "tuning.h", "lstm_fwd_bf_step.inc", os.path.join("..", "..", "include", "eesen_hip.h")]
 FLAGS = (os.environ.get("EESEN_BUILD_DEFS", "").split()) + ["--offload-arch=gfx950", "-O3", "-std=c++17", "-fPIC", "-fno-gpu-rdc", "-Wall", "-Wno-unused-function"]
 
 
@@ -24,7 +24,7 @@
     h = hashlib.sha1()
     files = []
     for d in (CSRC, os.path.join(CSRC, "tools"), os.path.join(_DIR, "..", "include")):
-        files += [os.path.join(d, f) for f in sorted(os.listdir(d)) if f.endswith((".hip", ".cpp", ".h", ".cc", ".map"))]
+        files += [os.path.join(d, f) for f in sorted(os.listdir(d)) if f.endswith((".hip", ".cpp", ".h", ".cc", ".map", ".inc"))]
     for f in files:
         h.update(os.path.basename(f).encode() + b"\0")
         h.update(open(f, "rb").read())
diff --git a/eesen_amd/csrc/kernels.h b/eesen_amd/csrc/kernels.h
--- a/eesen_amd/csrc/kernels.h
+++ b/eesen_amd/csrc/kernels.h
@@ -56,6 +56,8 @@
   int poll_raw = 0;
   unsigned* milestone = nullptr;
   int milestone_step = 0;
+  const unsigned* guard[2] = {nullptr, nullptr};
+  int guard_step[2] = {-1, -1};
   int xcd_map = 1, fwd_mux = 1, bwd_q4 = 1, bwd_ksplit = 1, bwd_mux = 1;
   int fwd_t16_small = 1;
   int fwd_narrow2 = 1;
@@ -100,6 +102,7 @@
   size_t ctl_words = 0;
   int chunk = 0;
   const void* fn = nullptr;
+  const void* fn_guard = nullptr;
 };
 RecPlan lstm_fwd_plan(const LstmLayerDev& L);
 RecPlan lstm_bwd_plan(const LstmLayerDev& L);
diff --git a/eesen_amd/csrc/lstm_fwd_bf_step.inc b/eesen_amd/csrc/lstm_fwd_bf_step.inc
--- /dev/null
+++ b/eesen_amd/csrc/lstm_fwd_bf_step.inc
@@ -0,0 +1,97 @@
+    const int t = dir == 0 ? step : T - 1 - step;
+    const int tp = dir == 0 ? t - 1 : t + 1;
+    f32x4 acc[NT];
+#pragma unroll
+    for (int n = 0; n < NT; ++n) acc[n] = f32x4{0.f, 0.f, 0.f, 0.f};
+    EESEN_STAMP(0);
+    if (step > 0) {
+      if (wave == EESEN_POLL_WAVE) {
+        const bool go = wait_counters(my_cnt, nblk, (unsigned)step, err, spin_limit, lane, L.poll_delay);
+        if (lane == 0) s_go = go ? 1 : 0;
+      }
+      __syncthreads();
+      if (!s_go) return;
+      EESEN_STAMP(1);
+      if (L.milestone && step == L.milestone_step + 1 && bx == 0 && tid == 0)
+        report_milestone(L.milestone, (unsigned)(R.ndir * R.nz));
+      const unsigned xb = ((unsigned)(tp * L.ndir + dir) * (unsigned)nzall + (unsigned)zt) * xblk;
+      constexpr unsigned kOob = 0x80000000u;
+      const bool rok = s0 + li < s_end;
+      f32x4 a[AP][CPW];
+#pragma unroll
+      for (int pl = 0; pl < AP; ++pl)
+#pragma unroll
+        for (int c = 0; c < CPW; ++c) {
+          const int ch = wave + c * NW;
+          a[pl][c] = __builtin_amdgcn_raw_buffer_load_b128(rX, (rok && ch < nch) ? xb + (unsigned)pl * xpl + (unsigned)(((ch * 4 + kq) * 16 + li) * 16) : kOob, 0, 0);
+        }
+      __builtin_amdgcn_sched_barrier(0);
+#pragma unroll
+      for (int sum = SMAX; sum >= 0; --sum)
+#pragma unroll
+        for (int i = 0; i < AP; ++i) {
+          const int j = sum - i;
+          if (j < 0 || j >= WP) continue;
+#pragma unroll
+          for (int c = 0; c < CPW; ++c)
+#pragma unroll
+            for (int n = 0; n < NT; ++n) {
+              const f32x4& bb = b[j < WP && j >= 0 ? j : 0][n][c];
+              if constexpr (F16) acc[n] = __builtin_amdgcn_mfma_f32_16x16x32_f16(__builtin_bit_cast(f16x8_t, a[i][c]), __builtin_bit_cast(f16x8_t, bb), acc[n], 0, 0, 0);
+              else acc[n] = __builtin_amdgcn_mfma_f32_16x16x32_bf16(__builtin_bit_cast(bf16x8_t, a[i][c]), __builtin_bit_cast(bf16x8_t, bb), acc[n], 0, 0, 0);
+            }
+        }
+    }
+#pragma unroll
+    for (int n = 0; n < NT; ++n)
+#pragma unroll
+      for (int r = 0; r < 4; ++r) red[wave][4 * kq + r][n * 16 + li] = F16 ? acc[n][r] * unscale : acc[n][r];
+    __syncthreads();
+    EESEN_STAMP(2);
+    if (e_act) {
+      float4 pv[NW];
+#pragma unroll
+      for (int w = 0; w < NW; ++w) pv[w] = *reinterpret_cast<const float4*>(&red[w][es][eu * 4]);
+      __builtin_amdgcn_sched_barrier(0);
+      float4 pre = gx;
+#pragma unroll
+      for (int w = 0; w < NW; ++w) { pre.x += pv[w].x; pre.y += pv[w].y; pre.z += pv[w].z; pre.w += pv[w].w; }
+      float g = tanhf_(pre.x);
+      float i = sigmoidf_(pre.y + p_i * cprev);
+      float f = sigmoidf_(pre.z + p_f * cprev);
+      float c = g * i + cprev * f;
+      float h = tanhf_(c);
+      float o = sigmoidf_(pre.w + p_o * c);
+      float m = h * o;
+      if (t >= len || !e_ok) { g = i = f = o = c = m = 0.f; }
+      if (e_ok) {
+        *reinterpret_cast<float4*>(L.G + (size_t)(t * S + s_e) * ldG + gcol) = make_float4(g, i, f, o);
+        const size_t o1 = (size_t)((t + 1) * S + s_e) * ldY + dir * H + u0 + eu;
+        L.C[o1] = c;
+        __hip_atomic_store(L.Y + o1, m, __ATOMIC_RELAXED, __HIP_MEMORY_SCOPE_AGENT);
+        cprev = c;
+      }
+      const int k = u0 + eu;
+      const size_t xo = ((size_t)(t * L.ndir + dir) * nzall + zt) * (size_t)xblk +
+                        (size_t)((((k >> 5) * 4 + ((k & 31) >> 3)) * 16 + es) * 16 + (k & 7) * 2);
+      float rem = F16 ? m * kMScale : m;
+#pragma unroll
+      for (int pl = 0; pl < AP; ++pl) {
+        const unsigned hb = F16 ? rne_f16(rem) : rne_bf16(rem);
+        rem -= F16 ? f16_bits_to_f32(hb) : __uint_as_float(hb << 16);
+        const unsigned pk = hb | (quad_xor1(hb) << 16);
+        const unsigned pk2 = quad_xor2(pk);
+        if (e_ok && (eu & 3) == 0)
+          __hip_atomic_store(reinterpret_cast<unsigned long long*>(xbytes + xo + (size_t)pl * xpl), (unsigned long long)pk | ((unsigned long long)pk2 << 32),
+                             __ATOMIC_RELAXED, __HIP_MEMORY_SCOPE_AGENT);
+      }
+    }
+    EESEN_STAMP(3);
+    {
+      if (e_act) asm volatile("s_waitcnt vmcnt(0)" ::: "memory");
+      __syncthreads();
+      EESEN_STAMP(4);
+      if (tid == 0) __hip_atomic_fetch_add(my_cnt + (bx & (kShards - 1)) * kShardStride, 1u, __ATOMIC_RELAXED, __HIP_MEMORY_SCOPE_AGENT);
+      if (e_ok && step + 1 < T)
+        gx = *reinterpret_cast<const float4*>(L.G + (size_t)((dir == 0 ? t + 1 : t - 1) * S + s_e) * ldG + gcol);
+    }
diff --git a/eesen_amd/csrc/lstm_persistent.hip b/eesen_amd/csrc/lstm_persistent.hip
--- a/eesen_amd/csrc/lstm_persistent.hip
+++ b/eesen_amd/csrc/lstm_persistent.hip
@@ -64,6 +64,16 @@
     __builtin_amdgcn_s_sleep(EESEN_POLL_SLEEP);
   }
   if (lane == 0) __hip_atomic_store(err, 1u, __ATOMIC_RELAXED, __HIP_MEMORY_SCOPE_AGENT);
+  return false;
+}
+
+__device__ __forceinline__ bool wait_guard(const unsigned* word, unsigned* err, int spin_limit, int lane) {
+  for (int spins = 0; spins < spin_limit; ++spins) {
+    if (__hip_atomic_load(word, __ATOMIC_RELAXED, __HIP_MEMORY_SCOPE_AGENT) != 0u) return true;
+    if ((spins & 1023) == 1023 && __hip_atomic_load(err, __ATOMIC_RELAXED, __HIP_MEMORY_SCOPE_AGENT) != 0) return false;
+    __builtin_amdgcn_s_sleep(EESEN_POLL_SLEEP);
+  }
+  if (lane == 0) __hip_atomic_store(err, 3u, __ATOMIC_RELAXED, __HIP_MEMORY_SCOPE_AGENT);
   return false;
 }
 
@@ -279,9 +289,9 @@
 }
 __device__ __forceinline__ unsigned quad_xor1(unsigned v) { return (unsigned)__builtin_amdgcn_mov_dpp((int)v, 0xB1, 0xf, 0xf, true); }
 __device__ __forceinline__ unsigned quad_xor2(unsigned v) { return (unsigned)__builtin_amdgcn_mov_dpp((int)v, 0x4E, 0xf, 0xf, true); }
-template <int CPW, int NT, int AP, int WP, bool F16 = false>
-__global__ __launch_bounds__(NW * 64) void lstm_fwd_persistent_bf_kernel(LstmLayerDev L, unsigned* cnt, unsigned* err,
-                                                                         int spin_limit, unsigned long long* trace, Role R) {
+template <int CPW, int NT, int AP, int WP, bool F16, bool GUARD>
+__device__ __forceinline__ void lstm_fwd_bf_body(const LstmLayerDev& L, unsigned* cnt, unsigned* err, int spin_limit, unsigned long long* trace,
+                                                 const Role& R) {
   constexpr int ST = 16, UB = 4 * NT, RW = 16 * NT + 4, SMAX = (AP > WP ? AP : WP) - 1;
   constexpr float kMScale = 16384.f;
   __shared__ __attribute__((aligned(16))) float red[NW][ST][RW];
@@ -363,105 +373,43 @@
   const int zt = (L.s_begin / ST) + bz;
   const int nzall = (S + ST - 1) / ST;
   unsigned char* const xbytes = reinterpret_cast<unsigned char*>(L.X);
+  if constexpr (!GUARD) {
   for (int step = 0; step < T; ++step) {
-    const int t = dir == 0 ? step : T - 1 - step;
-    const int tp = dir == 0 ? t - 1 : t + 1;
-    f32x4 acc[NT];
-#pragma unroll
-    for (int n = 0; n < NT; ++n) acc[n] = f32x4{0.f, 0.f, 0.f, 0.f};
-    EESEN_STAMP(0);
-    if (step > 0) {
+#include "lstm_fwd_bf_step.inc"
+  }
+  } else {
+  int step0 = 0;
+#pragma unroll 1
+  for (int seg = 0; seg < (GUARD ? 3 : 1); ++seg) {
+  int send = T;
+  if constexpr (GUARD) {
+    if (seg < 2) send = min(max(L.guard_step[seg] - 1, step0), T);
+    if (seg > 0) {
       if (wave == EESEN_POLL_WAVE) {
-        const bool go = wait_counters(my_cnt, nblk, (unsigned)step, err, spin_limit, lane, L.poll_delay);
+        const bool go = wait_guard(L.guard[seg - 1], err, spin_limit, lane);
         if (lane == 0) s_go = go ? 1 : 0;
       }
       __syncthreads();
       if (!s_go) return;
-      EESEN_STAMP(1);
-      if (L.milestone && step == L.milestone_step + 1 && bx == 0 && tid == 0)
-        report_milestone(L.milestone, (unsigned)(R.ndir * R.nz));
-      const unsigned xb = ((unsigned)(tp * L.ndir + dir) * (unsigned)nzall + (unsigned)zt) * xblk;
-      constexpr unsigned kOob = 0x80000000u;
-      const bool rok = s0 + li < s_end;
-      f32x4 a[AP][CPW];
-#pragma unroll
-      for (int pl = 0; pl < AP; ++pl)
-#pragma unroll
-        for (int c = 0; c < CPW; ++c) {
-          const int ch = wave + c * NW;
-          a[pl][c] = __builtin_amdgcn_raw_buffer_load_b128(rX, (rok && ch < nch) ? xb + (unsigned)pl * xpl + (unsigned)(((ch * 4 + kq) * 16 + li) * 16) : kOob, 0, 0);
-        }
-      __builtin_amdgcn_sched_barrier(0);
-#pragma unroll
-      for (int sum = SMAX; sum >= 0; --sum)
-#pragma unroll
-        for (int i = 0; i < AP; ++i) {
-          const int j = sum - i;
-          if (j < 0 || j >= WP) continue;
-#pragma unroll
-          for (int c = 0; c < CPW; ++c)
-#pragma unroll
-            for (int n = 0; n < NT; ++n) {
-              const f32x4& bb = b[j < WP && j >= 0 ? j : 0][n][c];
-              if constexpr (F16) acc[n] = __builtin_amdgcn_mfma_f32_16x16x32_f16(__builtin_bit_cast(f16x8_t, a[i][c]), __builtin_bit_cast(f16x8_t, bb), acc[n], 0, 0, 0);
-              else acc[n] = __builtin_amdgcn_mfma_f32_16x16x32_bf16(__builtin_bit_cast(bf16x8_t, a[i][c]), __builtin_bit_cast(bf16x8_t, bb), acc[n], 0, 0, 0);
-            }
-        }
-    }
-#pragma unroll
-    for (int n = 0; n < NT; ++n)
-#pragma unroll
-      for (int r = 0; r < 4; ++r) red[wave][4 * kq + r][n * 16 + li] = F16 ? acc[n][r] * unscale : acc[n][r];
-    __syncthreads();
-    EESEN_STAMP(2);
-    if (e_act) {
-      float4 pv[NW];
-#pragma unroll
-      for (int w = 0; w < NW; ++w) pv[w] = *reinterpret_cast<const float4*>(&red[w][es][eu * 4]);
-      __builtin_amdgcn_sched_barrier(0);
-      float4 pre = gx;
-#pragma unroll
-      for (int w = 0; w < NW; ++w) { pre.x += pv[w].x; pre.y += pv[w].y; pre.z += pv[w].z; pre.w += pv[w].w; }
-      float g = tanhf_(pre.x);
-      float i = sigmoidf_(pre.y + p_i * cprev);
-      float f = sigmoidf_(pre.z + p_f * cprev);
-      float c = g * i + cprev * f;
-      float h = tanhf_(c);
-      float o = sigmoidf_(pre.w + p_o * c);
-      float m = h * o;
-      if (t >= len || !e_ok) { g = i = f = o = c = m = 0.f; }
-      if (e_ok) {
-        *reinterpret_cast<float4*>(L.G + (size_t)(t * S + s_e) * ldG + gcol) = make_float4(g, i, f, o);
-        const size_t o1 = (size_t)((t + 1) * S + s_e) * ldY + dir * H + u0 + eu;
-        L.C[o1] = c;
-        __hip_atomic_store(L.Y + o1, m, __ATOMIC_RELAXED, __HIP_MEMORY_SCOPE_AGENT);
-        cprev = c;
-      }
-      const int k = u0 + eu;
-      const size_t xo = ((size_t)(t * L.ndir + dir) * nzall + zt) * (size_t)xblk +
-                        (size_t)((((k >> 5) * 4 + ((k & 31) >> 3)) * 16 + es) * 16 + (k & 7) * 2);
-      float rem = F16 ? m * kMScale : m;
-#pragma unroll
-      for (int pl = 0; pl < AP; ++pl) {
-        const unsigned hb = F16 ? rne_f16(rem) : rne_bf16(rem);
-        rem -= F16 ? f16_bits_to_f32(hb) : __uint_as_float(hb << 16);
-        const unsigned pk = hb | (quad_xor1(hb) << 16);
-        const unsigned pk2 = quad_xor2(pk);
-        if (e_ok && (eu & 3) == 0)
-          __hip_atomic_store(reinterpret_cast<unsigned long long*>(xbytes + xo + (size_t)pl * xpl), (unsigned long long)pk | ((unsigned long long)pk2 << 32),
-                             __ATOMIC_RELAXED, __HIP_MEMORY_SCOPE_AGENT);
-      }
-    }
-    EESEN_STAMP(3);
-    {
-      if (e_act) asm volatile("s_waitcnt vmcnt(0)" ::: "memory");
-      __syncthreads();
-      EESEN_STAMP(4);
-      if (tid == 0) __hip_atomic_fetch_add(my_cnt + (bx & (kShards - 1)) * kShardStride, 1u, __ATOMIC_RELAXED, __HIP_MEMORY_SCOPE_AGENT);
-      if (e_ok && step + 1 < T)
-        gx = *reinterpret_cast<const float4*>(L.G + (size_t)((dir == 0 ? t + 1 : t - 1) * S + s_e) * ldG + gcol);
-    }
-  }
+    }
+  }
+  for (int step = step0; step < send; ++step) {
+#include "lstm_fwd_bf_step.inc"
+  }
+  step0 = send;
+  }
+  }
+}
+
+template <int CPW, int NT, int AP, int WP, bool F16 = false>
+__global__ __launch_bounds__(NW * 64) void lstm_fwd_persistent_bf_kernel(LstmLayerDev L, unsigned* cnt, unsigned* err,
+                                                                         int spin_limit, unsigned long long* trace, Role R) {
+  lstm_fwd_bf_body<CPW, NT, AP, WP, F16, false>(L, cnt, err, spin_limit, trace, R);
+}
+template <int CPW, int NT, int AP, int WP, bool F16 = false>
+__global__ __launch_bounds__(NW * 64) void lstm_fwd_persistent_bf_guard_kernel(LstmLayerDev L, unsigned* cnt, unsigned* err,
+                                                                               int spin_limit, unsigned long long* trace, Role R) {
+  lstm_fwd_bf_body<CPW, NT, AP, WP, F16, true>(L, cnt, err, spin_limit, trace, R);
 }
 
 template <int CPW, int NT, bool XCHG>
@@ -1745,6 +1693,10 @@
     EESEN_ROW(kBwdKsplitMux, kRecBwdKsplitMux, lstm_bwd_persistent_ksplit_mux_kernel, 2), EESEN_ROW(kBwdKsplitMux, kRecBwdKsplitMux, lstm_bwd_persistent_ksplit_mux_kernel, 3),
     EESEN_ROW(kBwdKsplitMux, kRecBwdKsplitMux, lstm_bwd_persistent_ksplit_mux_kernel, 4),
 };
+const RecKernel kRecGuardKernels[] = {
+    EESEN_ROW(kFwdBfGuard, kRecFwdBf, lstm_fwd_persistent_bf_guard_kernel, 1,2,2,2,true), EESEN_ROW(kFwdBfGuard, kRecFwdBf, lstm_fwd_persistent_bf_guard_kernel, 2,2,2,2,true),
+    EESEN_ROW(kFwdBfGuard, kRecFwdBf, lstm_fwd_persistent_bf_guard_kernel, 1,2,3,3,false), EESEN_ROW(kFwdBfGuard, kRecFwdBf, lstm_fwd_persistent_bf_guard_kernel, 2,2,3,3,false),
+};
 #undef EESEN_BWD_Q4
 #undef EESEN_BWD_GEN
 #undef EESEN_FWD_BF
@@ -1757,6 +1709,8 @@
   const int want[5] = {a0, a1, a2, a3, a4};
   for (const RecKernel& k : kRecKernels)
     if (k.family == family && std::equal(want, want + 5, k.arg)) return &k;
+  for (const RecKernel& k : kRecGuardKernels)
+    if (k.family == family && std::equal(want, want + 5, k.arg)) return &k;
   return nullptr;
 }
 const void* handoff_pingpong_fn() { return reinterpret_cast<const void*>(&handoff_pingpong_kernel); }
diff --git a/eesen_amd/csrc/net.cpp b/eesen_amd/csrc/net.cpp
--- a/eesen_amd/csrc/net.cpp
+++ b/eesen_amd/csrc/net.cpp
@@ -183,7 +183,9 @@
   EESEN_HIP_CHECK(hipStreamSynchronize(st));
   EESEN_HIP_CHECK(hipMemset(ctl.p + kCtlWords - 1, 0, sizeof(unsigned)));
   const bool only_waiter = e == 2 && tn.fwd_mid;
+  const bool only_guard = e == 3 && tn.fwd_quad;
   if (only_waiter) tn.fwd_mid = 0;
+  else if (only_guard) tn.fwd_quad = 0;
   else { persistent = 0; gate_fwd = false; overlap = false; }
   ++recoveries;
   const int lost = std::max(1, steps_since_clean);
@@ -193,6 +195,10 @@
   if (only_waiter)
     fprintf(stderr, "WARNING (eesen_hip) the side stream's wait for a forward-recurrence milestone gave up (kernels serialised by a tool?): "
                     "%d minibatch(es) in flight %s%s; continuing without the early input GEMM (EESEN_FWD_MID=0)\n", lost, what,
+            rerun ? " and the last forward pass is re-run" : "");
+  else if (only_guard)
+    fprintf(stderr, "WARNING (eesen_hip) a forward recurrence gave up waiting for gate-input rows from the side stream (kernels serialised by a tool?): "
+                    "%d minibatch(es) in flight %s%s; continuing with every gate-input row in front of its recurrence (EESEN_FWD_QUAD=0)\n", lost, what,
             rerun ? " and the last forward pass is re-run" : "");
   else
     fprintf(stderr, "WARNING (eesen_hip) a persistent recurrence kernel gave up waiting for a peer workgroup (GPU shared or preempted?): "
@@ -601,6 +607,37 @@
   forward_pass();
 }
 
+Net::FwdEarly Net::fwd_early(int li, const RecPlan& fp, int T) const {
+  FwdEarly E;
+  const Layer& L = layers[li];
+  const Layer* nxt = li + 1 < (int)layers.size() ? &layers[li + 1] : nullptr;
+  const int nd = L.ndir, ldY = nd * L.H;
+  const long rows = (long)T * S;
+  const bool pers = fp.kind != kRecNone;
+  E.gate = pers && overlap && gate_fwd && !fwd_bf16 && !L.cur_fwd_drop && fp.units <= 8 && nxt && nxt->is_lstm() && T >= 2 && rows >= 128 &&
+           fp.one_window &&
+           (nxt->ndir * 4 * nxt->H) % 128 == 0 && ldY % 16 == 0 && nd * fp.seq_tiles * kShards <= 64;
+  E.mile_step = (3 * T) / 4;
+  E.mid = pers && overlap && tn.fwd_mid && !E.gate && !L.cur_fwd_drop && fp.leaves_room && nd == 2 && nxt && nxt->is_lstm() &&
+          T >= 32 && E.mile_step + 1 < T && fp.one_window;
+  if (E.mid) {
+    E.r0 = ((T - 1 - E.mile_step) * S + 255) / 256 * 256;
+    E.r1 = (E.mile_step + 1) * S / 256 * 256;
+    if (E.r1 <= E.r0) E.r0 = E.r1 = 0;
+  }
+  return E;
+}
+
+bool Net::fwd_quad_rule(int li, const RecPlan& fp, int T, int r0, int r1, int steps[2]) const {
+  steps[0] = steps[1] = -1;
+  if (!tn.fwd_quad || li < 1 || r1 <= r0 || r0 <= 0 || (long)r1 >= (long)T * S) return false;
+  const Layer& L = layers[li];
+  if (L.ndir != 2 || fp.kind != kRecFwdBf || !fp.fn_guard || !fp.one_window || !fp.leaves_room || (4 * L.H) % 256 != 0) return false;
+  steps[0] = std::min(r0 / S, T - 1 - (r1 - 1) / S);
+  steps[1] = std::min(r1 / S, T - 1 - (r0 - 1) / S);
+  return steps[0] >= 2 && steps[1] >= steps[0];
+}
+
 void Net::forward_pass() {
   const float* x = input.p;
   int ldx = pad4(layers[0].din);
@@ -633,7 +670,39 @@
       EESEN_HIP_CHECK(hipMemsetAsync(L.C.p + (size_t)(T + 1) * S * ldY, 0, blk, st));
       EESEN_HIP_CHECK(hipMemsetAsync(L.Y.p + (size_t)(T + 1) * S * ldY, 0, blk, st));
       prepare_dropout(*this, L);
-      if (g_gated) {
+      LstmLayerDev v = lstm_view(*this, L, T);
+      const RecPlan fp = persistent ? lstm_fwd_plan(v) : RecPlan{};
+      const bool pers = fp.kind != kRecNone;
+      int quad_steps[2];
+      const bool quad = !g_gated && fwd_quad_rule(li_, fp, T, mid_r0, mid_r1, quad_steps);
+      if (quad) {
+        unsigned* gw = mile.p + ((li_ - 1) & 1) * kMileRegion + kGuardWord;
+        const int N4 = 4 * H;
+        const float* Wx = params.p + L.p_off + L.off_wx;
+        const float* bias = params.p + L.p_off + L.off_bias;
+        GemmBound w_hi = w_amax;
+        if (w_hi.p && w_hi.per_index) w_hi.p += N4;
+        const int ti_ = timer.begin(st, 0);
+        gemm_f32(st, true, true, mid_r0, N4, L.din, 1.f, x, ldx, Wx, pad4(L.din), 0.f, L.G.p, ldG, bias, nullptr, 0, 0, fwd_bf16, x_amax, w_amax);
+        gemm_f32(st, true, true, rows - mid_r1, N4, L.din, 1.f, x + (size_t)mid_r1 * ldx, ldx, Wx + (size_t)N4 * pad4(L.din), pad4(L.din), 0.f,
+                 L.G.p + (size_t)mid_r1 * ldG + N4, ldG, bias + N4, nullptr, 0, 0, fwd_bf16, x_amax, w_hi);
+        timer.end(st, ti_);
+        EESEN_HIP_CHECK(hipEventRecord(ev_quad_go, st));
+        EESEN_HIP_CHECK(hipMemsetD32Async(reinterpret_cast<hipDeviceptr_t>(gw), 1, 1, st2));
+        EESEN_HIP_CHECK(hipStreamWaitEvent(st2, ev_quad_go, 0));
+        const int late_lds = tn.fwd_quad == 2 ? 64 : (tn.side_lds_kb >= 0 ? tn.side_lds_kb : (gemm_mode() >= 1 ? 48 : 32)) * 1024;
+        const int tj_ = timer.begin(st2, 0);
+        gemm_f32(st2, true, true, rows - mid_r1, N4, L.din, 1.f, x + (size_t)mid_r1 * ldx, ldx, Wx, pad4(L.din), 0.f, L.G.p + (size_t)mid_r1 * ldG, ldG,
+                 bias, nullptr, 0, late_lds, fwd_bf16, x_amax, w_amax);
+        gemm_f32(st2, true, true, mid_r0, N4, L.din, 1.f, x, ldx, Wx + (size_t)N4 * pad4(L.din), pad4(L.din), 0.f, L.G.p + N4, ldG, bias + N4,
+                 nullptr, 0, late_lds, fwd_bf16, x_amax, w_hi);
+        timer.end(st2, tj_);
+        EESEN_HIP_CHECK(hipMemsetD32Async(reinterpret_cast<hipDeviceptr_t>(gw + 1), 1, 1, st2));
+        EESEN_HIP_CHECK(hipEventRecord(ev_quad_done, st2));
+        v.guard[0] = gw; v.guard_step[0] = quad_steps[0];
+        v.guard[1] = gw + 1; v.guard_step[1] = quad_steps[1];
+        mid_r0 = mid_r1 = 0;
+      } else if (g_gated) {
         if (gated_rows < rows) {
           const int ti_ = timer.begin(st, 0);
           gemm_f32(st, true, true, rows - gated_rows, ldG, L.din, 1.f, x + (size_t)gated_rows * ldx, ldx, params.p + L.p_off + L.off_wx,
@@ -659,23 +728,19 @@
         timer.end(st, ti_);
       }
       Layer* nxt = (&L - layers.data()) + 1 < (long)layers.size() ? &layers[(&L - layers.data()) + 1] : nullptr;
-      LstmLayerDev v = lstm_view(*this, L, T);
-      const RecPlan fp = persistent ? lstm_fwd_plan(v) : RecPlan{};
-      const bool pers = fp.kind != kRecNone;
-      const bool plan_gate = pers && overlap && gate_fwd && !fwd_bf16 && !L.cur_fwd_drop && fp.units <= 8 && nxt && nxt->is_lstm() && T >= 2 && rows >= 128 &&
-                             fp.one_window &&
-                             (nxt->ndir * 4 * nxt->H) % 128 == 0 && ldY % 16 == 0 && nd * fp.seq_tiles * kShards <= 64;
-      const int mile_step = (3 * T) / 4;
-      const bool plan_mid = pers && overlap && tn.fwd_mid && !plan_gate && !L.cur_fwd_drop && fp.leaves_room && nd == 2 && nxt && nxt->is_lstm() &&
-                            T >= 32 && mile_step + 1 < T && fp.one_window;
+      const FwdEarly early = fwd_early(li_, fp, T);
+      const bool plan_gate = early.gate;
+      const int mile_step = early.mile_step;
+      const bool plan_mid = early.mid;
       { const int ti_ = timer.begin(st, 1);
       v.poll_delay = delay_fwd;
       v.poll_raw = poll_raw;
       if (plan_mid) {
-        mile.reserve(32);
-        EESEN_HIP_CHECK(hipMemsetAsync(mile.p, 0, 2 * sizeof(unsigned), st));
+        mile.reserve(2 * kMileRegion);
+        unsigned* region = mile.p + (li_ & 1) * kMileRegion;
+        EESEN_HIP_CHECK(hipMemsetAsync(region, 0, kMileRegion * sizeof(unsigned), st));
         EESEN_HIP_CHECK(hipEventRecord(ev_gate_reset, st));
-        v.milestone = mile.p;
+        v.milestone = region;
         v.milestone_step = mile_step;
       }
       if (pers) lstm_fwd_launch(st, fp, v, ctl.p, ctl.p + kCtlWords - 1, spin_limit, trace.p, plan_gate ? ev_gate_reset.get() : nullptr);
@@ -686,6 +751,7 @@
       ++info_lstm_layers;
       check_launch("lstm_fwd");
       timer.end(st, ti_);
+      if (quad) EESEN_HIP_CHECK(hipStreamWaitEvent(st, ev_quad_done, 0));
       if (pers && plan_gate) {
         const int ldG2 = nxt->ndir * 4 * nxt->H;
         nxt->G.reserve((size_t)rows * ldG2);
@@ -700,17 +766,16 @@
         g_gated = true;
       }
       if (plan_mid) {
-        EESEN_HIP_CHECK(hipMemsetD32Async(reinterpret_cast<hipDeviceptr_t>(mile.p + 1), 1, 1, st));
+        EESEN_HIP_CHECK(hipMemsetD32Async(reinterpret_cast<hipDeviceptr_t>(v.milestone + 1), 1, 1, st));
         const int ldG2 = nxt->ndir * 4 * nxt->H;
         nxt->G.reserve((size_t)rows * ldG2);
-        mid_r0 = ((T - 1 - mile_step) * S + 255) / 256 * 256;
-        mid_r1 = (mile_step + 1) * S / 256 * 256;
-        if (mid_r1 <= mid_r0) mid_r0 = mid_r1 = 0;
+        mid_r0 = early.r0;
+        mid_r1 = early.r1;
       }
       if (plan_mid && mid_r1 > mid_r0) {
         const int ldG2 = nxt->ndir * 4 * nxt->H;
         EESEN_HIP_CHECK(hipStreamWaitEvent(st2, ev_gate_reset, 0));
-        wait_for_word(st2, mile.p + 1, 1u, ctl.p + kCtlWords - 1, 2.0 * std::max(1.0, T / 1000.0) * std::max(1.0, spin_limit / 400000.0));
+        wait_for_word(st2, v.milestone + 1, 1u, ctl.p + kCtlWords - 1, 2.0 * std::max(1.0, T / 1000.0) * std::max(1.0, spin_limit / 400000.0));
         const int tj_ = timer.begin(st2, 0);
         gemm_f32(st2, true, true, mid_r1 - mid_r0, ldG2, nxt->din, 1.f, L.Y.p + (size_t)S * ldY + (size_t)mid_r0 * ldY, ldY,
                  params.p + nxt->p_off + nxt->off_wx, pad4(nxt->din), 0.f, nxt->G.p + (size_t)mid_r0 * ldG2, ldG2,
@@ -974,12 +1039,20 @@
   const std::vector<RecPlan> bwd = bwd_plans(T);
   std::string o = "{\"T\": " + std::to_string(T) + ", \"S\": " + std::to_string(S) + ", \"persistent\": " + (persistent ? "true" : "false") + ", \"layers\": [";
   bool first = true;
+  FwdEarly below;
   for (size_t li = 0; li < layers.size(); ++li) {
     const Layer& L = layers[li];
-    if (!L.is_lstm()) continue;
+    if (!L.is_lstm()) { below = FwdEarly{}; continue; }
     const RecPlan fp = persistent && T >= 1 ? lstm_fwd_plan(lstm_view(*this, L, T)) : RecPlan{}, &bp = bwd[li];
+    int qs[2];
+    const char* sched = below.gate ? "gated under the recurrence below"
+                        : below.r1 > below.r0 ? (fwd_quad_rule((int)li, fp, T, below.r0, below.r1, qs) ? "middle under the recurrence below, needed quadrants, recurrence, late quadrants beside it"
+                                                                                                  : "middle under the recurrence below, both ends, recurrence")
+                                              : "whole, recurrence";
+    const bool lstm_below = li > 0 && layers[li - 1].is_lstm();
     o += std::string(first ? "" : ", ") + "{\"layer\": " + std::to_string(li) + ", \"cells\": " + std::to_string(L.H) + ", \"directions\": " + std::to_string(L.ndir) +
-         ", \"forward\": " + one(fp) + ", \"backward\": " + one(bp) + "}";
+         ", \"forward\": " + one(fp) + ", \"backward\": " + one(bp) + (lstm_below ? std::string(", \"input_gemm\": \"") + sched + "\"" : std::string()) + "}";
+    below = T >= 1 ? fwd_early((int)li, fp, T) : FwdEarly{};
     first = false;
   }
   const bool ov = overlap_for_minibatch(bwd);
diff --git a/eesen_amd/csrc/net.h b/eesen_amd/csrc/net.h
--- a/eesen_amd/csrc/net.h
+++ b/eesen_amd/csrc/net.h
@@ -114,6 +114,11 @@
   bool overlap = true;
   DevEvent ev_gate_reset, ev_gate_done;
   DevBuf<unsigned> mile;
+  static constexpr int kMileRegion = 64, kGuardWord = 32;
+  DevEvent ev_quad_go, ev_quad_done;
+  struct FwdEarly { bool gate = false, mid = false; int mile_step = 0, r0 = 0, r1 = 0; };
+  FwdEarly fwd_early(int li, const RecPlan& fp, int T) const;
+  bool fwd_quad_rule(int li, const RecPlan& fp, int T, int r0, int r1, int steps[2]) const;
   bool gate_fwd = true;
   bool fwd_bf16 = false;
   bool fwd_bf16_rec = false;
diff --git a/eesen_amd/csrc/rec_kernels.h b/eesen_amd/csrc/rec_kernels.h
--- a/eesen_amd/csrc/rec_kernels.h
+++ b/eesen_amd/csrc/rec_kernels.h
@@ -6,7 +6,7 @@
 constexpr int kRecWaves = 8;
 struct RecRole { int nblk, ndir, nz, xcd; };
 
-enum RecFamily { kFwdF32, kFwdBf, kFwdMux, kBwdGeneric, kBwdQ4, kBwdKsplit, kBwdKsplitH, kBwdKsplitMux };
+enum RecFamily { kFwdF32, kFwdBf, kFwdBfGuard, kFwdMux, kBwdGeneric, kBwdQ4, kBwdKsplit, kBwdKsplitH, kBwdKsplitMux };
 struct RecKernel {
   int family;
   int kind;
diff --git a/eesen_amd/csrc/rec_plan.cpp b/eesen_amd/csrc/rec_plan.cpp
--- a/eesen_amd/csrc/rec_plan.cpp
+++ b/eesen_amd/csrc/rec_plan.cpp
@@ -239,7 +239,10 @@
   const dim3 grid(L.H / (4 * nt), L.ndir, cdiv(L.S / nwin, 16 * mt));
   const size_t words = ctl_words(grid.y * grid.z);
   if (B.on) {
-    if (words <= (size_t)kCtlHalf) answer(*rec_kernel(kFwdBf, B.cpw, B.nt, B.ap, B.wp, B.f16), grid, words, 16, nwin, nwin == 1);
+    if (words <= (size_t)kCtlHalf) {
+      answer(*rec_kernel(kFwdBf, B.cpw, B.nt, B.ap, B.wp, B.f16), grid, words, 16, nwin, nwin == 1);
+      if (const RecKernel* g = rec_kernel(kFwdBfGuard, B.cpw, B.nt, B.ap, B.wp, B.f16)) P.fn_guard = g->fn;
+    }
     return P;
   }
   const bool xchg = L.X != nullptr && ft.mt == 1 && L.H % 32 == 0 && !drop && small_xchg(L, 2048);
@@ -270,7 +273,11 @@
     EESEN_HIP_CHECK(hipMemsetAsync(cnt, 0, sizeof(unsigned) * P.ctl_words, st));
     if (after_reset && P.one_window) EESEN_HIP_CHECK(hipEventRecord(after_reset, st));
     if (P.kind == kRecFwdMux) plan_launch(st, P.fn, P.wgs, L, cnt, err, spin_limit, role);
-    else plan_launch(st, P.fn, P.wgs, L, cnt, err, spin_limit, trace, role);
+    else {
+      const bool guarded = L.guard[0] != nullptr || L.guard[1] != nullptr;
+      EESEN_REQUIRE(!guarded || P.fn_guard, EESEN_ERR_STATE, "row guards set for a forward plan without a guarded instantiation");
+      plan_launch(st, guarded ? P.fn_guard : P.fn, P.wgs, L, cnt, err, spin_limit, trace, role);
+    }
   }
 }
 
diff --git a/eesen_amd/csrc/tuning.h b/eesen_amd/csrc/tuning.h
--- a/eesen_amd/csrc/tuning.h
+++ b/eesen_amd/csrc/tuning.h
@@ -11,7 +11,7 @@
   int overlap = -1, gate_fwd = -1, side_lds_kb = -1;
   int spin_limit = 400000;
   bool spin_limit_set = false;
-  int bwd_q4 = 1, bwd_q4_st8 = 1, fwd_narrow2 = 1, fwd_t16_small = 1, bwd_ksplit = 1, fwd_mux = 1, bwd_mux = 1, xcd_map = 1, fwd_mid = 1, fwd_split = 1, fwd_f16 = 1, bwd_f16 = 1;
+  int bwd_q4 = 1, bwd_q4_st8 = 1, fwd_narrow2 = 1, fwd_t16_small = 1, bwd_ksplit = 1, fwd_mux = 1, bwd_mux = 1, xcd_map = 1, fwd_mid = 1, fwd_quad = 1, fwd_split = 1, fwd_f16 = 1, bwd_f16 = 1;
   int comm_defer = -1;
   int trace = 0;
   bool print_flight = false;
@@ -27,6 +27,7 @@
     t.overlap = num("EESEN_OVERLAP", -1);
     t.gate_fwd = num("EESEN_GATE_FWD", -1);
     t.fwd_mid = num("EESEN_FWD_MID", 1);
+    t.fwd_quad = num("EESEN_FWD_QUAD", 1);
     t.side_lds_kb = num("EESEN_SIDE_LDS_KB", -1);
     t.spin_limit_set = getenv("EESEN_SPIN_LIMIT") != nullptr;
     t.spin_limit = num("EESEN_SPIN_LIMIT", 400000);
```

Result: faster. 1.009 million, median of 6 (+1.3%).
